# yhn112/DeDLOC

Measured on AMD Instinct MI355X. Metric: samples/sec (whole node) ALBERT-large MLM pretrain at 1/2/4/8 peers, higher is better.
Workload: dtype bf16; 1 GPU; model=albert-large-v2, global_batch=4096, seq_len=512, parallelism=collaborative-dp1, micro_batch=512, grad_accum=1, compression=FLOAT16, optimizer=LAMB, impl=dedloc

## Files before the change

dedloc_amd/_build.py:

```python
from __future__ import annotations

import concurrent.futures as cf
import glob
import os
import subprocess
import sys
import sysconfig

ROOT = os.path.dirname(os.path.abspath(__file__))
CSRC = os.path.join(ROOT, "csrc")
BUILD = os.path.join(os.path.dirname(ROOT), "build", "obj")
ARCH = os.environ.get("DEDLOC_OFFLOAD_ARCH", "gfx950")
SO_PATH = os.path.join(ROOT, "_C.so")
DHT_SO_PATH = os.path.join(ROOT, "_dht.so")
ROCM = os.environ.get("ROCM_PATH", "/opt/rocm")


def _torch_paths():
    import torch
    import torch.utils.cpp_extension as ce

    abi = int(torch.compiled_with_cxx11_abi())
    return ce.include_paths(), ce.library_paths(), abi


def _newer(target: str, deps) -> bool:
    if not os.path.exists(target):
        return True
    t = os.path.getmtime(target)
    return any(os.path.getmtime(d) > t for d in deps)


def _run(cmd, verbose):
    if verbose:
        print(" ".join(cmd), flush=True)
    r = subprocess.run(cmd, stdout=subprocess.PIPE, stderr=subprocess.STDOUT, text=True)
    if r.returncode != 0:
        raise RuntimeError(f"build step failed ({r.returncode}):\n{' '.join(cmd)}\n{r.stdout}")
    return r.stdout


def build(verbose: bool = False, jobs: int | None = None) -> str:
    os.makedirs(BUILD, exist_ok=True)
    headers = glob.glob(os.path.join(CSRC, "include", "*.h"))
    all_headers = sorted(set(headers) | set(glob.glob(os.path.join(CSRC, "**", "*.h"), recursive=True)))
    hip_srcs = sorted(glob.glob(os.path.join(CSRC, "kernels", "*.hip")))
    inc = ["-I", os.path.join(CSRC, "include")]
    hip_flags = ["--offload-arch=" + ARCH, *HIP_FLAGS]
    jobs = jobs or min(8, os.cpu_count() or 4)

    jobs_list = []
    objs = []
    for src in hip_srcs:
        obj = os.path.join(BUILD, os.path.basename(src).replace(".hip", ".o"))
        objs.append(obj)
        if _newer(obj, [src] + headers + [__file__]):
            jobs_list.append(["hipcc", *hip_flags, *FILE_FLAGS.get(os.path.basename(src), []), *inc, "-c", src,
                              "-o", obj])

    tinc, tlib, abi = _torch_paths()
    torch_srcs = [os.path.join(CSRC, "bindings.cpp")] + sorted(glob.glob(os.path.join(CSRC, "comm", "*.cpp")))
    for src in torch_srcs:
        name = os.path.basename(src).replace(".cpp", ".o")
        obj = os.path.join(BUILD, name if src.endswith("bindings.cpp") else "comm_" + name)
        objs.append(obj)
        if _newer(obj, [src] + all_headers):
            cmd = ["g++", "-O2", "-std=c++17", "-fPIC", f"-D_GLIBCXX_USE_CXX11_ABI={abi}", "-D__HIP_PLATFORM_AMD__",
                   "-DUSE_ROCM", "-I", f"{ROCM}/include", *inc]
            for p in tinc:
                cmd += ["-I", p]
            cmd += ["-I", sysconfig.get_paths()["include"], "-c", src, "-o", obj]
            jobs_list.append(cmd)

    for src in sorted(glob.glob(os.path.join(CSRC, "host", "*.cpp"))):
        obj = os.path.join(BUILD, "host_" + os.path.basename(src).replace(".cpp", ".o"))
        objs.append(obj)
        if _newer(obj, [src] + all_headers):
            jobs_list.append(["g++", "-O2", "-std=c++17", "-fPIC", "-Wall", "-D__HIP_PLATFORM_AMD__", "-I",
                              f"{ROCM}/include", *inc, "-c", src, "-o", obj])

    rt_srcs = sorted(glob.glob(os.path.join(CSRC, "runtime", "*.cpp")))
    rt_objs = []
    for src in rt_srcs:
        obj = os.path.join(BUILD, "rt_" + os.path.basename(src).replace(".cpp", ".o"))
        rt_objs.append(obj)
        if _newer(obj, [src] + all_headers):
            jobs_list.append(["g++", "-O2", "-std=c++17", "-fPIC", "-Wall", *inc, "-c", src, "-o", obj])

    with cf.ThreadPoolExecutor(jobs) as ex:
        list(ex.map(lambda c: _run(c, verbose), jobs_list))

    if _newer(SO_PATH, objs):
        _link(objs, SO_PATH, tlib, verbose)
    if rt_objs and _newer(DHT_SO_PATH, rt_objs):
        _run(["g++", "-shared", "-fPIC", *rt_objs, "-o", DHT_SO_PATH, "-lpthread"], verbose)
    _OBJS[:] = objs
    return SO_PATH


_OBJS: list = []
HIP_FLAGS = ["-O3", "-std=c++17", "-fPIC", "-ffp-contract=fast", "-munsafe-fp-atomics"]
FILE_FLAGS: dict = {"comm_q8.hip": ["-ffp-contract=on"]}


def _link(objs, out, tlib, verbose):
    cmd = ["hipcc", "--offload-arch=" + ARCH, "-shared", "-fPIC", *objs, "-o", out]
    for p in tlib:
        cmd += ["-L", p, f"-Wl,-rpath,{p}"]
    cmd += ["-lc10", "-ltorch", "-ltorch_cpu", "-lc10_hip", "-ltorch_hip", "-lamdhip64", "-lrccl", "-L", f"{ROCM}/lib",
            f"-Wl,-rpath,{ROCM}/lib"]
    _run(cmd, verbose)


def build_variant(name: str, rev: str, kernels, verbose: bool = False, flags=None) -> str:
    build(verbose)
    vdir = os.path.join(os.path.dirname(BUILD), "variant_" + name)
    os.makedirs(vdir, exist_ok=True)
    repo = os.path.dirname(ROOT)
    swap = {}
    for k in kernels:
        src = os.path.join(vdir, os.path.basename(k))
        where = "" if k.endswith(".cpp") else "kernels/"
        text = subprocess.run(["git", "-C", repo, "show", f"{rev}:dedloc_amd/csrc/{where}{os.path.basename(k)}"],
                              check=True, capture_output=True, text=True).stdout
        with open(src, "w") as f:
            f.write(text)
        if k.endswith(".cpp"):
            obj = src.replace(".cpp", ".o")
            tinc, _, abi = _torch_paths()
            cmd = ["g++", "-O2", "-std=c++17", "-fPIC", f"-D_GLIBCXX_USE_CXX11_ABI={abi}", "-D__HIP_PLATFORM_AMD__",
                   "-DUSE_ROCM", "-I", f"{ROCM}/include", "-I", os.path.join(CSRC, "include")]
            for ip in tinc:
                cmd += ["-I", ip]
            _run(cmd + list(flags or []) + ["-I", sysconfig.get_paths()["include"], "-c", src, "-o", obj], verbose)
        else:
            obj = src.replace(".hip", ".o")
            extra = FILE_FLAGS.get(os.path.basename(k), []) if flags is None else list(flags)
            _run(["hipcc", "--offload-arch=" + ARCH, *HIP_FLAGS, *extra, "-I", os.path.join(CSRC, "include"), "-c",
                  src, "-o", obj], verbose)
        swap[os.path.basename(obj)] = obj
    out_dir = os.path.join(repo, "ab")
    os.makedirs(out_dir, exist_ok=True)
    out = os.path.join(out_dir, f"_C_{name}.so")
    objs = [swap.get(os.path.basename(o), o) for o in _OBJS]
    _link(objs, out, _torch_paths()[1], verbose)
    return out


if __name__ == "__main__":
    if len(sys.argv) > 3 and sys.argv[1] == "variant":
        fl = [a for a in sys.argv[4:] if a.startswith("--flags=")]
        ks = [a for a in sys.argv[4:] if not a.startswith("--") and a != "-v"]
        print(build_variant(sys.argv[2], sys.argv[3], ks, verbose="-v" in sys.argv,
                            flags=fl[0][len("--flags="):].split() if fl else None))
    else:
        print(build(verbose="-v" in sys.argv))
```

dedloc_amd/csrc/bindings.cpp:

```cpp
#include <torch/extension.h>
#include <torch/library.h>
#include <c10/hip/HIPStream.h>

#include <atomic>
#include <cstring>
#include <map>
#include <mutex>
#include <string>
#include <unordered_map>

#include "dl_kernels.h"

namespace {

inline hipStream_t cur_stream(const at::Tensor& t) {
  return c10::hip::getCurrentHIPStream(t.get_device()).stream();
}

inline bf16_t* bf(const at::Tensor& t) { return reinterpret_cast<bf16_t*>(t.data_ptr()); }
inline const bf16_t* cbf(const at::Tensor& t) { return reinterpret_cast<const bf16_t*>(t.data_ptr()); }
inline float* f32(const at::Tensor& t) { return t.data_ptr<float>(); }

inline void check(int rc, const char* what) { TORCH_CHECK(rc == 0, "dedloc_amd: unsupported shape for ", what); }

// ... 336 lines not shown
                            f32(gamma), f32(beta), bf(y), bf(s), f32(mean), f32(rstd), (int)T, (int)E, (float)eps,
                            cur_stream(ids)),
        "embed_ln_pos_fwd");
  return {y, s, mean, rstd};
}

void embed_pos_bwd(const at::Tensor& ds, const at::Tensor& ids, const c10::optional<at::Tensor>& tt,
                   const at::Tensor& pos, at::Tensor dwemb, at::Tensor dpemb, at::Tensor dtemb) {
  expect(ds, at::kBFloat16, "ds");
  for (auto* t : {&dwemb, &dpemb, &dtemb}) expect(*t, at::kFloat, "embedding grad");
  const int64_t T = ids.numel(), E = ds.size(-1);
  const long* ttp = tt.has_value() ? tt->data_ptr<long>() : nullptr;
  check(dl_embed_pos_bwd(cbf(ds), ids.data_ptr<long>(), ttp, pos_ptr(pos, T), f32(dwemb), f32(dpemb),
                         f32(dtemb), (int)T, (int)E, (int)dtemb.size(0), cur_stream(ds)),
        "embed_pos_bwd");
}

std::tuple<at::Tensor, at::Tensor> xent_fwd_bwd(const at::Tensor& logits, const at::Tensor& labels, bool inplace,
                                                int64_t ignore_index) {
  expect(logits, at::kBFloat16, "logits");
  expect(labels, at::kLong, "labels");
  const int64_t V = logits.size(-1), M = logits.numel() / V;
  auto dl = inplace ? logits : at::empty_like(logits);
  auto ws = at::empty({3}, logits.options().dtype(at::kFloat));
  check(dl_xent_fwd_bwd(cbf(logits), labels.data_ptr<long>(), bf(dl), nullptr, f32(ws), f32(ws) + 1, (int)M, (int)V, V,
                        (int)ignore_index, cur_stream(logits)),
        "xent_fwd_bwd");
  return {ws.narrow(0, 0, 1).squeeze(0), dl};
}

std::tuple<at::Tensor, at::Tensor> xent_eval(const at::Tensor& logits, const at::Tensor& labels,
                                             int64_t ignore_index) {
  TORCH_CHECK(logits.is_cuda() && logits.scalar_type() == at::kBFloat16, "logits must be a bf16 GPU tensor");
  expect(labels, at::kLong, "labels");
  TORCH_CHECK(logits.dim() >= 1 && logits.size(-1) >= 1, "logits must be [..., V] with V >= 1");
  const int64_t V = logits.size(-1), M = logits.numel() / V;
  int64_t ld = V;
  if (logits.dim() == 2 && logits.stride(1) == 1 && logits.stride(0) >= V) ld = logits.stride(0);
  else TORCH_CHECK(logits.is_contiguous(), "logits must be contiguous or a 2-D view with unit column stride");
  TORCH_CHECK(labels.numel() == M, "labels has ", labels.numel(), " elements for ", M, " rows of logits");
  TORCH_CHECK(M <= INT32_MAX && V <= INT32_MAX, "xent_eval: too many rows or columns");
  auto row_loss = at::empty({M}, logits.options().dtype(at::kFloat));
  auto row_rank = at::empty({M}, logits.options().dtype(at::kInt));
  check(dl_xent_eval(cbf(logits), labels.data_ptr<long>(), f32(row_loss), row_rank.data_ptr<int>(), (int)M, (int)V, ld,
                     (int)ignore_index, cur_stream(logits)),
        "xent_eval");
  return {row_loss, row_rank};
}

std::tuple<at::Tensor, at::Tensor> knn_topk(const at::Tensor& q, const at::Tensor& bank, int64_t k, int64_t splits) {
  expect(q, at::kBFloat16, "q");
  expect(bank, at::kBFloat16, "bank");
  TORCH_CHECK(q.dim() == 2 && bank.dim() == 2 && q.size(1) == bank.size(1), "knn_topk: q [Q, D] and bank [N, D]");
  TORCH_CHECK(q.get_device() == bank.get_device(), "knn_topk: q and bank on different devices");
  const int64_t Q = q.size(0), N = bank.size(0), D = q.size(1);
  TORCH_CHECK(D % 16 == 0 && D >= 16 && D <= 4096, "knn_topk: D = ", D, " must be a multiple of 16 in 16 .. 4096");
  TORCH_CHECK(k >= 1 && k <= 256 && k <= N, "knn_topk: k = ", k, " must be in 1 .. min(256, N = ", N, ")");
  TORCH_CHECK(Q <= INT32_MAX && N <= INT32_MAX, "knn_topk: too many rows");
  const int max_splits = dl_knn_max_splits((int)N, (int)k);
  TORCH_CHECK(splits >= 0 && splits <= max_splits, "knn_topk: splits = ", splits, " must be 0 (automatic) or 1 .. ",
              max_splits, " for N = ", N, ", k = ", k);
  auto vals = at::empty({Q, k}, q.options().dtype(at::kFloat));
  auto idx = at::empty({Q, k}, q.options().dtype(at::kInt));
  if (Q == 0) return {vals, idx};
  int cus = 0;
  if (splits == 0)
    TORCH_CHECK(hipDeviceGetAttribute(&cus, hipDeviceAttributeMultiprocessorCount, q.get_device()) == hipSuccess,
                "knn_topk: cannot read the device's CU count");
  const int S = splits > 0 ? (int)splits : dl_knn_splits((int)Q, (int)N, (int)k, cus);
  auto lists = at::empty({dl_knn_list_entries((int)Q, (int)k, S)}, q.options().dtype(at::kLong));
  at::Tensor part;
  if (S > 1) part = at::empty({Q * S * k}, q.options().dtype(at::kLong));
  check(dl_knn_topk(cbf(q), cbf(bank), (int)Q, (int)N, (int)D, (int)k, S,
                    reinterpret_cast<unsigned long long*>(lists.data_ptr<int64_t>()),
                    S > 1 ? reinterpret_cast<unsigned long long*>(part.data_ptr<int64_t>()) : nullptr, f32(vals),
                    idx.data_ptr<int>(), cur_stream(q)),
        "knn_topk");
  return {vals, idx};
}

std::tuple<at::Tensor, at::Tensor> knn_vote(const at::Tensor& vals, const at::Tensor& idx, const at::Tensor& bank_labels,
                                            const at::Tensor& targets, int64_t num_classes, double sigma) {
  expect(vals, at::kFloat, "vals");
  expect(idx, at::kInt, "idx");
  expect(bank_labels, at::kInt, "bank_labels");
  expect(targets, at::kLong, "targets");
  TORCH_CHECK(vals.dim() == 2 && idx.sizes() == vals.sizes(), "knn_vote: vals and idx must both be [Q, k]");
  const int64_t Q = vals.size(0), k = vals.size(1), N = bank_labels.numel();
  TORCH_CHECK(k >= 1 && k <= 256, "knn_vote: k = ", k, " must be in 1 .. 256");
  TORCH_CHECK(targets.numel() == Q, "knn_vote: targets has ", targets.numel(), " elements for ", Q, " rows");
  TORCH_CHECK(N >= 1 && N <= INT32_MAX && Q <= INT32_MAX, "knn_vote: bank_labels must hold 1 .. 2^31 - 1 labels");
  TORCH_CHECK(num_classes >= 1 && num_classes <= 8192, "knn_vote: num_classes = ", num_classes, " must be in 1 .. 8192");
  TORCH_CHECK(sigma > 0, "knn_vote: sigma must be positive");
  auto pred = at::empty({Q}, vals.options().dtype(at::kInt));
  auto rank = at::empty({Q}, vals.options().dtype(at::kInt));
  check(dl_knn_vote(f32(vals), idx.data_ptr<int>(), bank_labels.data_ptr<int>(), targets.data_ptr<long>(),
                    pred.data_ptr<int>(), rank.data_ptr<int>(), (int)Q, (int)k, (int)N, (int)num_classes, (float)sigma,
                    cur_stream(vals)),
        "knn_vote");
  return {pred, rank};
}

inline const int* kvinfo_ptr(const c10::optional<at::Tensor>& kvinfo, int64_t B) {
  if (!kvinfo.has_value()) return nullptr;
  expect(*kvinfo, at::kInt, "kvinfo");
  TORCH_CHECK(kvinfo->numel() == B + 1, "kvinfo must be int32[B + 1] (lengths, prefix flag)");
  return kvinfo->data_ptr<int>();
}

inline void check_head_dim(int64_t D, int64_t ld, int64_t H, const char* what) {
  TORCH_CHECK((D == 64 || D == 128) && ld == 3 * H * D, "dedloc_amd: ", what, ": head_dim ", D, " (row length ", ld,
              ", ", H, " heads) is not supported by the fused attention kernels; supported head sizes are 64 and 128");
}

std::tuple<at::Tensor, at::Tensor> attn_fwd(const at::Tensor& qkv, const c10::optional<at::Tensor>& mbias, int64_t H,
                                            int64_t S, double scale, const c10::optional<at::Tensor>& kvinfo) {
  expect(qkv, at::kBFloat16, "qkv");
  const int64_t ld = qkv.size(-1), T = qkv.numel() / ld, D = ld / (3 * H), B = T / S;
  check_head_dim(D, ld, H, "attn_fwd");
  auto out = at::empty({T, H * D}, qkv.options());
  auto lse = at::empty({B, H, S}, qkv.options().dtype(at::kFloat));
  const float* mb = nullptr;
  if (mbias.has_value()) {
    expect(*mbias, at::kFloat, "mbias");
    mb = f32(*mbias);
  }
  check(dl_attn_fwd(cbf(qkv), ld, mb, kvinfo_ptr(kvinfo, B), bf(out), H * D, f32(lse), (int)B, (int)H, (int)S,
                    (int)D, (float)scale, cur_stream(qkv)),
        "attn_fwd");
  return {out, lse};
}

at::Tensor attn_bwd(const at::Tensor& qkv, const c10::optional<at::Tensor>& mbias, const at::Tensor& out,
                    const at::Tensor& dout, const at::Tensor& lse, int64_t H, int64_t S, double scale,
                    const c10::optional<at::Tensor>& kvinfo, const c10::optional<at::Tensor>& dbias) {
  expect(qkv, at::kBFloat16, "qkv");
  expect(out, at::kBFloat16, "out");
  expect(dout, at::kBFloat16, "dout");
  const int64_t ld = qkv.size(-1), T = qkv.numel() / ld, D = ld / (3 * H), B = T / S;
  check_head_dim(D, ld, H, "attn_bwd");
  auto dqkv = at::empty_like(qkv);
  auto delta = at::empty({B, H, S}, qkv.options().dtype(at::kFloat));
  const float* mb = mbias.has_value() ? f32(*mbias) : nullptr;
  float* dbp = nullptr;
  if (dbias.has_value()) {
    expect(*dbias, at::kFloat, "dbias");
    TORCH_CHECK(dbias->numel() == ld, "dbias must have 3*H*D elements");
    dbp = f32(*dbias);
  }
  check(dl_attn_bwd(cbf(qkv), ld, mb, kvinfo_ptr(kvinfo, B), cbf(out), cbf(dout), H * D, f32(lse), f32(delta),
                    bf(dqkv), dbp, (int)B, (int)H, (int)S, (int)D, (float)scale, cur_stream(qkv)),
        "attn_bwd");
  return dqkv;
}

struct PackedLayout {
  int64_t B, T, max_slot;
  const int* dev;
};
inline PackedLayout packed_layout(const at::Tensor& seqinfo, const at::Tensor& seqinfo_host, int64_t T,
                                  const char* what) {
  expect(seqinfo, at::kInt, "seqinfo");
  TORCH_CHECK(seqinfo_host.device().is_cpu() && seqinfo_host.scalar_type() == at::kInt && seqinfo_host.is_contiguous(),
              what, ": seqinfo_host must be a contiguous int32 CPU tensor");
  const int64_t n = seqinfo_host.numel();
  TORCH_CHECK(n >= 3 && n % 2 == 1 && seqinfo.numel() == n, what,
              ": seqinfo must be int32[2B + 1] (B + 1 row offsets, B lengths) on both sides");
  const int64_t B = (n - 1) / 2;
  const int* p = seqinfo_host.data_ptr<int>();
  TORCH_CHECK(p[0] == 0 && p[B] == T, what, ": row offsets must run from 0 to T = ", T, " (got ", p[0], " .. ", p[B],
              ")");
  int64_t max_slot = 0;
  for (int64_t b = 0; b < B; ++b) {
    const int64_t slot = (int64_t)p[b + 1] - p[b], len = p[B + 1 + b];
    TORCH_CHECK(p[b] % 64 == 0 && p[b + 1] % 64 == 0, what, ": row offset of sequence ", b,
                " is not a multiple of 64 (", p[b], ", ", p[b + 1], ")");
    TORCH_CHECK(slot >= 64, what, ": sequence ", b, " has an empty slot");
    TORCH_CHECK(len >= 1 && len <= slot, what, ": length ", len, " of sequence ", b, " is outside 1 .. its slot of ",
                slot, " rows");
    max_slot = std::max(max_slot, slot);
  }
  return PackedLayout{B, T, max_slot, seqinfo.data_ptr<int>()};
}

std::tuple<at::Tensor, at::Tensor> attn_varlen_fwd(const at::Tensor& qkv, const at::Tensor& seqinfo,
                                                   const at::Tensor& seqinfo_host, int64_t H, double scale) {
  expect(qkv, at::kBFloat16, "qkv");
  const int64_t ld = qkv.size(-1), T = qkv.numel() / ld, D = ld / (3 * H);
  check_head_dim(D, ld, H, "attn_varlen_fwd");
  const PackedLayout L = packed_layout(seqinfo, seqinfo_host, T, "attn_varlen_fwd");
  auto out = at::empty({T, H * D}, qkv.options());
  auto lse = at::empty({H, T}, qkv.options().dtype(at::kFloat));
  check(dl_attn_varlen_fwd(cbf(qkv), ld, L.dev, bf(out), H * D, f32(lse), (int)L.B, (int)T, (int)L.max_slot, (int)H,
                           (int)D, (float)scale, cur_stream(qkv)),
        "attn_varlen_fwd");
  return {out, lse};
}

at::Tensor attn_varlen_bwd(const at::Tensor& qkv, const at::Tensor& seqinfo, const at::Tensor& seqinfo_host,
                           const at::Tensor& out, const at::Tensor& dout, const at::Tensor& lse, int64_t H,
                           double scale, const c10::optional<at::Tensor>& dbias) {
  expect(qkv, at::kBFloat16, "qkv");
  expect(out, at::kBFloat16, "out");
  expect(dout, at::kBFloat16, "dout");
  expect(lse, at::kFloat, "lse");
  const int64_t ld = qkv.size(-1), T = qkv.numel() / ld, D = ld / (3 * H);
  check_head_dim(D, ld, H, "attn_varlen_bwd");
  const PackedLayout L = packed_layout(seqinfo, seqinfo_host, T, "attn_varlen_bwd");
  TORCH_CHECK(out.numel() == T * H * D && dout.numel() == T * H * D && lse.numel() == H * T,
              "attn_varlen_bwd: out / dout must be [T, H*D] and lse [H, T]");
  auto dqkv = at::empty_like(qkv);
  auto delta = at::empty({H, T}, qkv.options().dtype(at::kFloat));
  float* dbp = nullptr;
  if (dbias.has_value()) {
    expect(*dbias, at::kFloat, "dbias");
    TORCH_CHECK(dbias->numel() == ld, "dbias must have 3*H*D elements");
    dbp = f32(*dbias);
  }
  check(dl_attn_varlen_bwd(cbf(qkv), ld, L.dev, cbf(out), cbf(dout), H * D, f32(lse), f32(delta), bf(dqkv), dbp,
                           (int)L.B, (int)T, (int)L.max_slot, (int)H, (int)D, (float)scale, cur_stream(qkv)),
        "attn_varlen_bwd");
  return dqkv;
}

std::tuple<at::Tensor, at::Tensor> attn_softmax_fwd(const at::Tensor& s, const c10::optional<at::Tensor>& mbias,
                                                    int64_t H, double c) {
  expect(s, at::kFloat, "s");
  const int64_t S = s.size(-1), rows = s.numel() / S;
  TORCH_CHECK(rows % (H * S) == 0, "attn_softmax_fwd: scores must be [B*H*S, S]");
  const float* mb = nullptr;
  if (mbias.has_value()) {
    expect(*mbias, at::kFloat, "mbias");
    TORCH_CHECK(mbias->numel() == rows / H, "attn_softmax_fwd: mbias must be [B, S]");
    mb = f32(*mbias);
  }
  auto p = at::empty(s.sizes(), s.options().dtype(at::kBFloat16));
  auto lse = at::empty({rows}, s.options());
  check(dl_attn_softmax_fwd(f32(s), mb, bf(p), f32(lse), rows, (int)H, (int)S, (float)c, cur_stream(s)),
        "attn_softmax_fwd");
  return {p, lse};
}

std::tuple<at::Tensor, at::Tensor> attn_softmax_bwd(const at::Tensor& s, const at::Tensor& dp,
                                                    const c10::optional<at::Tensor>& mbias, const at::Tensor& lse,
                                                    const at::Tensor& delta, int64_t H, double c, double scale) {
  expect(s, at::kFloat, "s");
  expect(dp, at::kFloat, "dp");
  expect(lse, at::kFloat, "lse");
  expect(delta, at::kFloat, "delta");
  const int64_t S = s.size(-1), rows = s.numel() / S;
  TORCH_CHECK(dp.numel() == s.numel() && lse.numel() == rows && delta.numel() == rows && rows % (H * S) == 0,
              "attn_softmax_bwd: shape mismatch");
  const float* mb = nullptr;
  if (mbias.has_value()) {
    expect(*mbias, at::kFloat, "mbias");
    TORCH_CHECK(mbias->numel() == rows / H, "attn_softmax_bwd: mbias must be [B, S]");
    mb = f32(*mbias);
  }
  auto p = at::empty(s.sizes(), s.options().dtype(at::kBFloat16));
  auto ds = at::empty_like(p);
  check(dl_attn_softmax_bwd(f32(s), f32(dp), mb, f32(lse), f32(delta), bf(p), bf(ds), rows, (int)H, (int)S, (float)c,
                            (float)scale, cur_stream(s)),
        "attn_softmax_bwd");
  return {p, ds};
}


enum { kGemmNone = -1, kGemm8 = 0, kGemmTiled = 1, kGemmSmall = 2 };
std::atomic<int64_t> g_gemm_backend[3];

inline int took(int backend, int rc) {
  if (rc == 0) g_gemm_backend[backend].fetch_add(1, std::memory_order_relaxed);
  return rc;
}

std::vector<int64_t> gemm_backend_counts() {
  return {g_gemm_backend[kGemm8].load(), g_gemm_backend[kGemmTiled].load(), g_gemm_backend[kGemmSmall].load()};
}

inline void expect_operands(const at::Tensor& a, const at::Tensor& b) {
  TORCH_CHECK(a.is_cuda() && b.is_cuda(), "gemm operands must be GPU tensors");
  TORCH_CHECK(a.scalar_type() == at::kBFloat16 && b.scalar_type() == at::kBFloat16, "gemm operands must be bf16");
  TORCH_CHECK(a.dim() == 2 && b.dim() == 2 && a.stride(1) == 1 && b.stride(1) == 1,
              "gemm operands must be 2-D with unit inner stride");
}

inline at::Tensor f32_bias(const c10::optional<at::Tensor>& bias, int64_t n) {
  if (!bias.has_value()) return at::Tensor();
  TORCH_CHECK(bias->numel() == n, "gemm bias must hold one value per output column");
  return bias->scalar_type() == at::kFloat ? bias->contiguous() : bias->to(at::kFloat).contiguous();
}

inline DlGemm gemm_desc(const at::Tensor& a, bool trans_a, const at::Tensor& b, bool trans_b, bf16_t* C = nullptr,
                        long ldc = 0) {
  DlGemm g;
  g.A = cbf(a), g.lda = a.stride(0), g.a_kouter = trans_a;
  g.B = cbf(b), g.ldb = b.stride(0), g.b_kouter = !trans_b;
  g.M = (int)a.size(trans_a ? 1 : 0), g.N = (int)b.size(trans_b ? 0 : 1), g.K = (int)a.size(trans_a ? 0 : 1);
  TORCH_CHECK(b.size(trans_b ? 1 : 0) == g.K, "gemm inner dimensions differ");
  g.C = C, g.ldc = ldc;
  return g;
}

enum : unsigned { kUse8 = 1, kUseTiled = 2, kUseSmall = 4 };
int gemm_route(const DlGemm& g, unsigned allow, const at::Tensor& like, hipStream_t st) {
  if ((allow & kUse8) && took(kGemm8, dl_gemm8(g, st)) == 0) return kGemm8;
// ... 900 lines not shown
  TORCH_CHECK(groups >= 1 && N % groups == 0 && mean.numel() == groups * C && rstd.numel() == groups * C &&
                  sums.numel() == 2 * groups * C,
              "conv2d_dgrad_bn: statistics shapes");
  TORCH_CHECK(x.size(2) == H && x.size(3) == W && w.size(1) == C, "conv2d_dgrad_bn: x must be the conv input");
  const long stat_rows = N / groups * H * W;
  const DlBnBwdEpi bn{cbf(x), y.has_value() ? cbf(*y) : nullptr, (long)C, f32(mean), f32(rstd), f32(gamma),
                      f32(beta)};
  const at::Tensor gdy = dy.is_contiguous(at::MemoryFormat::ChannelsLast) ? dy
                                                                           : dy.contiguous(at::MemoryFormat::ChannelsLast);
  const int64_t K = w.size(0), R = w.size(2), S = w.size(3);
  if (is_pointwise(R, S, stride, pad) && gdy.size(2) == H && gdy.size(3) == W && conv_gemm()) {
    expect_nhwc(gdy, "dy");
    if (residual.has_value()) {
      expect_nhwc(*residual, "residual");
      TORCH_CHECK(residual->sizes() == x.sizes(), "conv2d_dgrad_bn: residual must have the input's shape");
    }
    auto dx = at::empty_like(x);
    const at::Tensor wk = krsc_view(w);
    const at::Tensor dyr = rows2d(gdy), wkc = wk.view({K, C});
    DlGemm g = gemm_desc(dyr, false, wkc, false, bf(dx), C);
    g.epi = DL_EPI_BNBWD;
    if (residual.has_value()) g.R = cbf(*residual), g.ldr = C;
    g.stats = f32(sums), g.stat_rows = stat_rows;
    g.bn = &bn;
    if (gemm_route(g, kUse8, dyr, cur_stream(dy)) != kGemmNone) return {dx, true};
  }
  if (!residual.has_value() && K % 64 == 0) {
    expect_nhwc(gdy, "dy");
    auto dx = at::empty_like(x);
    if (conv_dgrad_classes(gdy, krsc_view(w), stride, pad, H, W, dx, wds, f32(sums), groups, &bn)) return {dx, true};
  }
  return {conv2d_dgrad(gdy, w, stride, pad, H, W, residual, wds), false};
}

at::Tensor bn_bwd_prep(at::Tensor g, const at::Tensor& x, const c10::optional<at::Tensor>& y, const at::Tensor& mean,
                       const at::Tensor& rstd, const at::Tensor& gamma, const at::Tensor& beta, at::Tensor sums,
                       int64_t groups) {
  expect_nhwc(g, "g");
  expect_nhwc(x, "x");
  const int64_t C = x.size(1);
  check(dl_bn_bwd_prep(bf(g), y.has_value() ? cbf(*y) : nullptr, cbf(x), f32(mean), f32(rstd), f32(gamma), f32(beta),
                       f32(sums), x.numel() / C / groups, (int)C, (int)groups, cur_stream(g)),
        "bn_bwd_prep");
  return g;
}

void conv2d_wgrad(const at::Tensor& dy_in, const at::Tensor& x, at::Tensor dw, int64_t stride, int64_t pad,
                  const c10::optional<at::Tensor>& cols) {
  const at::Tensor dy = dy_in.is_contiguous(at::MemoryFormat::ChannelsLast)
                            ? dy_in
                            : dy_in.contiguous(at::MemoryFormat::ChannelsLast);
  expect_nhwc(dy, "dy");
  if (!cols.has_value()) expect_nhwc(x, "x");
  TORCH_CHECK(dw.is_cuda() && dw.scalar_type() == at::kFloat && dw.dim() == 4, "dw must be an fp32 4-D GPU tensor");
  const int64_t N = x.size(0), C = x.size(1), H = x.size(2), W = x.size(3);
  const int64_t K = dy.size(1), P = dy.size(2), Q = dy.size(3), R = dw.size(2), S = dw.size(3);
  TORCH_CHECK(dw.size(0) == K && dw.size(1) == C, "conv2d_wgrad: dw shape mismatch");
  TORCH_CHECK(!cols.has_value() || C % 64 != 0, "conv2d_wgrad: cols are the stem's (C not a multiple of 64) only");
  at::Tensor dk = dw.permute({0, 2, 3, 1});
  const bool direct = dk.is_contiguous();
  at::Tensor acc = direct ? dk : at::zeros({K, R, S, C}, dw.options());
  int rc;
  if (is_pointwise(R, S, stride, pad) && conv_gemm() && K % 256 == 0 && C % 256 == 0) {
    gemm_acc_f32(rows2d(dy), rows2d(x), acc.view({K, C}), true, false);
  } else if (C % 8 == 0 && C >= 8 && C % 64 == 0) {
    const DlConvGeom gm = geom(cbf(x), N, H, W, C, P, Q, stride, stride, R, S, -pad, 1, -pad, 1);
    rc = dl_conv_wgrad(gm, cbf(dy), K, (int)K, f32(acc), R * S * C, (int)(R * S * C), cur_stream(dy));
    check(rc, "conv2d_wgrad");
  } else if (stem_s2d_ok(C, R, S, stride, pad, H, W)) {
    at::Tensor xs;
    if (cols.has_value()) {
      TORCH_CHECK(cols->scalar_type() == at::kBFloat16 && cols->is_contiguous() && cols->dim() == 2 &&
                      cols->size(0) == N * P * Q && cols->size(1) == 16,
                  "cols must be the stem's im2col_stem (space-to-depth) matrix for this input");
      xs = *cols;
    } else {
      xs = stem_s2d(x);
    }
    auto slab = at::zeros({K, 256}, dw.options());
    rc = dl_conv_wgrad(geom(cbf(xs), N, H / 2, W / 2, 16, P, Q, 1, 1, 4, 4, -2, 1, -2, 1), cbf(dy), K, (int)K,
                       f32(slab), 256, 256, cur_stream(dy));
    check(rc, "conv2d_wgrad(stem)");
    acc.view({K, R * S * C}).add_(slab.index_select(1, stem_s2d_index(dw.device())));
  } else {
    const StemCols sc = stem_cols(R, S, C, false);
    const int64_t M = N * P * Q;
    const at::Tensor col = stem_cols_checked(cols, x, R, S, stride, pad, P, Q, sc);
    auto slab = at::zeros({K, R, sc.SCp}, dw.options());
    rc = dl_conv_wgrad(geom(cbf(col), M, 1, 1, sc.Kp, 1, 1, 1, 1, 1, 1, 0, 1, 0, 1), cbf(dy), K, (int)K,
                       f32(slab), R * sc.SCp, (int)(R * sc.SCp), cur_stream(dy));
    check(rc, "conv2d_wgrad(stem)");
    acc.view({K, R, S * C}).add_(slab.narrow(2, 0, S * C));
  }
  if (!direct) dk.add_(acc);
}

}

TORCH_LIBRARY_IMPL(dedloc, CUDA, m) {
  m.impl("conv2d_fwd", &conv2d_fwd);
  m.impl("conv2d_bn_act", &conv2d_bn_act);
  m.impl("conv2d_fwd_stats", &conv2d_fwd_stats);
  m.impl("im2col_stem", &im2col_stem);
  m.impl("conv2d_dgrad_bn", &conv2d_dgrad_bn);
  m.impl("conv2d_dgrad_weights", &conv2d_dgrad_weights);
  m.impl("conv2d_dgrad_weights_batched", &conv2d_dgrad_weights_batched);
  m.impl("bn_bwd_prep", &bn_bwd_prep);
  m.impl("conv2d_dgrad", &conv2d_dgrad);
  m.impl("conv2d_wgrad", &conv2d_wgrad);
  m.impl("bn_fwd", &bn_fwd);
  m.impl("bn_apply", &bn_apply);
  m.impl("bn_bwd", &bn_bwd);
  m.impl("sinkhorn", &sinkhorn);
  m.impl("swav_ce", &swav_ce);
  m.impl("swav_ce_multi", &swav_ce_multi);
  m.impl("row_normalize_", &row_normalize_);
  m.impl("maxpool_fwd", &maxpool_fwd);
  m.impl("maxpool_bwd", &maxpool_bwd);
  m.impl("avgpool_fwd", &avgpool_fwd);
  m.impl("avgpool_bwd", &avgpool_bwd);
  m.impl("l2norm_fwd", &l2norm_fwd);
  m.impl("l2norm_bwd", &l2norm_bwd);
  m.impl("multicrop", &multicrop);
  m.impl("multicrop_ragged", &multicrop_ragged);
  m.impl("layernorm_fwd", &layernorm_fwd);
  m.impl("layernorm_bwd", &layernorm_bwd);
  m.impl("gelu_fwd", &gelu_fwd);
  m.impl("gelu_bwd", &gelu_bwd);
  m.impl("tanh_fwd", &tanh_fwd);
  m.impl("tanh_bwd", &tanh_bwd);
  m.impl("bias_grad", &bias_grad);
  m.impl("cast_bf16", &cast_bf16);
  m.impl("lamb_step", &lamb_step);
  m.impl("larc_sgd_step", &larc_sgd_step);
  m.impl("grad_norm_clip", &grad_norm_clip);
  m.impl("axpby", &axpby);
  m.impl("add_slabs_zero_", &add_slabs_zero_);
  m.impl("scale_by_", &scale_by_);
  m.impl("pack", &pack);
  m.impl("reduce_parts", &reduce_parts);
  m.impl("unpack", &unpack);
  m.impl("reduce_delta", &reduce_delta);
  m.impl("pack_q8", &pack_q8);
  m.impl("reduce_delta_q8", &reduce_delta_q8);
  m.impl("unpack_q8", &unpack_q8);
  m.impl("embed_ln_fwd", &embed_ln_fwd);
  m.impl("embed_bwd", &embed_bwd);
  m.impl("xent_fwd_bwd", &xent_fwd_bwd);
  m.impl("xent_eval", &xent_eval);
  m.impl("knn_topk", &knn_topk);
  m.impl("knn_vote", &knn_vote);
  m.impl("attn_fwd", &attn_fwd);
  m.impl("attn_bwd", &attn_bwd);
  m.impl("attn_varlen_fwd", &attn_varlen_fwd);
  m.impl("attn_varlen_bwd", &attn_varlen_bwd);
  m.impl("embed_ln_pos_fwd", &embed_ln_pos_fwd);
  m.impl("embed_pos_bwd", &embed_pos_bwd);
  m.impl("attn_softmax_fwd", &attn_softmax_fwd);
  m.impl("attn_softmax_bwd", &attn_softmax_bwd);
  m.impl("gemm", &gemm);
  m.impl("bmm", &bmm);
  m.impl("gemm_acc_f32", &gemm_acc_f32);
  m.impl("gemm_acc_f32_shared", &gemm_acc_f32_shared);
  m.impl("gemm_gelu", &gemm_gelu);
  m.impl("gemm_dgelu", &gemm_dgelu);
  m.impl("gemm_gelu_d", &gemm_gelu_d);
  m.impl("gemm_dmul", &gemm_dmul);
}

extern "C" int dedloc_amd_native_abi_version() { return 1; }

TORCH_LIBRARY(dedloc_ws, m) {
  m.def("clear_workspaces() -> int", &clear_workspaces);
  m.def("gemm_backend_counts() -> int[]", &gemm_backend_counts);
  m.def("gemm_wgrad_splits(int M, int N, int K) -> int", &gemm_wgrad_splits);
}
```

dedloc_amd/csrc/include/dl_kernels.h:

```cpp
#pragma once
#include <hip/hip_runtime.h>
#include <stddef.h>
#include <stdint.h>

typedef uint16_t bf16_t;

int dl_layernorm_fwd(const bf16_t* x, const bf16_t* r, const float* gamma, const float* beta, bf16_t* y,
                     bf16_t* s_out, float* mean, float* rstd, int rows, int D, float eps, hipStream_t st);
int dl_layernorm_bwd(const bf16_t* dy, const bf16_t* s, const float* gamma, const float* mean, const float* rstd,
                     bf16_t* ds, float* dg_part, float* db_part, float* dsum, int rows, int D, int nparts,
                     hipStream_t st);

int dl_gelu_fwd(const bf16_t* h, bf16_t* y, size_t n, hipStream_t st);
int dl_gelu_bwd(const bf16_t* dy, const bf16_t* h, bf16_t* dh, size_t n, hipStream_t st);
int dl_gelu_bwd_colsum(const bf16_t* dy, const bf16_t* h, bf16_t* dh, float* dbias, int rows, int N, hipStream_t st);
int dl_gelu_fwd_d(const bf16_t* h, bf16_t* y, bf16_t* d, size_t n, hipStream_t st);
int dl_mul_colsum(const bf16_t* dy, const bf16_t* d, bf16_t* dh, float* dbias, int rows, int N, hipStream_t st);
int dl_tanh_fwd(const bf16_t* x, bf16_t* y, size_t n, hipStream_t st);
int dl_tanh_bwd(const bf16_t* dy, const bf16_t* y, bf16_t* dx, size_t n, hipStream_t st);
int dl_colsum_bf16(const bf16_t* x, float* part, int rows, int N, int nparts, hipStream_t st);
int dl_colsum_f32(const float* part, float* out, int nparts, int N, int accumulate, hipStream_t st);
int dl_cast_f32_bf16(const float* x, bf16_t* y, size_t n, hipStream_t st);
int dl_add_bf16_to_f32(const bf16_t* x, float* y, size_t n, float alpha, hipStream_t st);

// ... 14 lines not shown
int dl_add_slabs_zero(float* out, float* slabs, int s, size_t n, hipStream_t st);

int dl_pack(const float* src, void* dst, int dst_dt, size_t n, float weight, hipStream_t st);
int dl_reduce_parts(const void* parts, int part_dt, size_t part_stride, int nparts, void* out, int out_dt, size_t n,
                    float inv_total, hipStream_t st);
int dl_unpack(const void* src, int src_dt, float* dst, const float* snap, int add, size_t n, hipStream_t st);
int dl_reduce_delta(const void* parts, void* deltas, int dt, size_t part_stride, int nparts, const float* weights,
                    size_t n, hipStream_t st);

size_t dl_q8_bytes(size_t n);
int dl_pack_q8(const float* src, void* dst, size_t n, hipStream_t st);
int dl_unpack_q8(const void* src, float* dst, int add, size_t n, hipStream_t st);
int dl_reduce_delta_q8(const void* parts, void* deltas, int nparts, const float* weights, size_t n, hipStream_t st);

int dl_embed_ln_fwd(const long* ids, const long* tt, const float* wemb, const float* pemb, const float* temb,
                    const float* gamma, const float* beta, bf16_t* y, bf16_t* s_out, float* mean, float* rstd, int T,
                    int S, int E, float eps, hipStream_t st);
int dl_embed_bwd(const bf16_t* ds, const long* ids, const long* tt, float* dwemb, float* dpemb, float* dtemb, int B,
                 int S, int E, int ntypes, hipStream_t st);
int dl_embed_ln_pos_fwd(const long* ids, const long* tt, const int* pos, const float* wemb, const float* pemb,
                        const float* temb, const float* gamma, const float* beta, bf16_t* y, bf16_t* s_out, float* mean,
                        float* rstd, int T, int E, float eps, hipStream_t st);
int dl_embed_pos_bwd(const bf16_t* ds, const long* ids, const long* tt, const int* pos, float* dwemb, float* dpemb,
                     float* dtemb, int T, int E, int ntypes, hipStream_t st);

int dl_xent_fwd_bwd(const bf16_t* logits, const long* labels, bf16_t* dlogits, float* row_loss, float* loss_out,
                    float* scale_buf, int M, int V, long ld, int ignore_index, hipStream_t st);

int dl_xent_eval(const bf16_t* logits, const long* labels, float* row_loss, int* row_rank, int M, int V, long ld,
                 int ignore_index, hipStream_t st);

int dl_knn_max_splits(int N, int k);
int dl_knn_splits(int Q, int N, int k, int cus);
long dl_knn_list_entries(int Q, int k, int splits);
int dl_knn_topk(const bf16_t* q, const bf16_t* bank, int Q, int N, int D, int k, int splits, unsigned long long* lists,
                unsigned long long* part, float* vals, int* idx, hipStream_t st);
int dl_knn_vote(const float* vals, const int* idx, const int* labels, const long* targets, int* pred, int* rank, int Q,
                int k, int N, int C, float sigma, hipStream_t st);

struct DlBnBwdEpi {
  const bf16_t* X;
  const bf16_t* Y;
  long ldx;
  const float* mean;
  const float* rstd;
  const float* gamma;
  const float* beta;
};

enum DlGemmEpi {
  DL_EPI_STORE = 0,
  DL_EPI_GELU = 1,
  DL_EPI_DGELU = 2,
  DL_EPI_F32 = 3,
  DL_EPI_STATS = 4,
  DL_EPI_BNBWD = 5,
  DL_EPI_GELUD = 6,
  DL_EPI_DMUL = 7,
};

struct DlGemm {
  const bf16_t* A = nullptr; long lda = 0; int a_kouter = 0;
  const bf16_t* B = nullptr; long ldb = 0; int b_kouter = 0;
  int M = 0, N = 0, K = 0;
  DlGemmEpi epi = DL_EPI_STORE;
  bf16_t* C = nullptr; long ldc = 0;
  float* Cf = nullptr; long ldcf = 0; long slab = 0; int accumulate = 0;
  const float* bias = nullptr;
  const bf16_t* R = nullptr; long ldr = 0;
  bf16_t* H = nullptr; long ldh = 0;
  float* dbias = nullptr;
  int splits = 1;
  float* stats = nullptr; long stat_rows = 0;
  const DlBnBwdEpi* bn = nullptr;
};

int dl_gemm8(const DlGemm& g, hipStream_t st);
int dl_gemm(const DlGemm& g, hipStream_t st);

int dl_sinkhorn_ws(int n, int K);
int dl_sinkhorn(const float* scores, float* Q, float* ws, int n, int K, int bs, float eps, int iters,
                hipStream_t st);
int dl_swav_ce(const void* scores, int scores_bf16, const float* q, float* dscores, float* loss, int rows, int K,
               float temperature, float scale, hipStream_t st);
int dl_swav_ce_multi(const void* scores, int scores_bf16, const float* q, const int* crops, int n_assign,
                     float* dscores, float* loss, int num_crops, int bs, int K, float temperature, float scale,
                     hipStream_t st);
int dl_row_normalize(float* w, int rows, int d, hipStream_t st);
int dl_multicrop(const float* pool, int P, int Hp, int Wp, const float* params, int nb, int S, int rad, const float* mean,
                 const float* stdv, float* ws, bf16_t* out, hipStream_t st);
int dl_multicrop_ragged(const unsigned char* bytes, long nbytes, const long* meta, int n, const float* params, int nb,
                        int S, int rad, const float* mean, const float* stdv, float* ws, bf16_t* out, hipStream_t st);
int dl_bn_fwd(const bf16_t* x, const bf16_t* res, bf16_t* y, const float* gamma, const float* beta, float* sums,
              float* mean, float* rstd, float* run_mean, float* run_var, long R, int C, int G, float eps,
              float momentum, int relu, hipStream_t st, int sums_zeroed = 0, int stats_ready = 0);
int dl_bn_apply(const bf16_t* x, const bf16_t* res, bf16_t* y, const float* gamma, const float* beta,
                const float* mean, const float* rstd, long R, int C, int G, int relu, hipStream_t st);
int dl_bn_stats(const bf16_t* x, float* sums, long R, int C, int G, hipStream_t st);
int dl_bn_bwd(const bf16_t* dy, const bf16_t* y, const bf16_t* x, const float* mean, const float* rstd,
              const float* gamma, float* sums, bf16_t* dx, bf16_t* dres, float* dgamma, float* dbeta, long R, int C,
              int G, int relu, hipStream_t st, int sums_zeroed = 0, int accumulate = 0, const float* beta = nullptr,
              int stats_ready = 0);
int dl_bn_bwd_prep(bf16_t* dy, const bf16_t* y, const bf16_t* x, const float* mean, const float* rstd,
                   const float* gamma, const float* beta, float* sums, long R, int C, int G, hipStream_t st);

struct DlConvGeom {
  const bf16_t* img;
  int Nimg, H, W, C;
  int I, J, sh, sw;
  int TR, TS, dh0, dhs, dw0, dws;
};
int dl_conv_fwd(const DlConvGeom& g, const bf16_t* w, long ldw, int N, bf16_t* out, int OH, int OW, int osh, int osw,
                int oh0, int ow0, long ldo, hipStream_t st, float* stats = nullptr, long stat_rows = 0,
                const DlBnBwdEpi* bn = nullptr);
int dl_conv_fwd_affine(const DlConvGeom& g, const bf16_t* w, long ldw, int N, bf16_t* out, int OH, int OW, long ldo,
                       const float* scale, const float* shift, const bf16_t* res, int relu, hipStream_t st);
struct DlConvFwdJob {
  DlConvGeom g;
  const bf16_t* w;
  long ldw;
  int oh0, ow0;
  long stat_rows;
};
int dl_conv_fwd_multi(const DlConvFwdJob* jobs, int njobs, int N, bf16_t* out, int OH, int OW, int osh, int osw,
                      long ldo, hipStream_t st, float* stats = nullptr, const DlBnBwdEpi* bn = nullptr);
struct DlWtJob {
  const bf16_t* src;
  bf16_t* dst;
  int K, C, R, S;
  int r0, s0, st, TR, TS;
};
int dl_conv_dgrad_weights_batched(const DlWtJob* jobs, int njobs, hipStream_t st);
int dl_conv_wgrad(const DlConvGeom& g, const bf16_t* dy, long ldy, int Cout, float* dw, long lddw, int Ncols,
                  hipStream_t st);
int dl_stem_s2d(const bf16_t* x, int N, int H, int W, bf16_t* xs, hipStream_t st);
int dl_im2col(const bf16_t* x, int N, int H, int W, int C, int R, int S, int stride, int pad, int P, int Q, int SCp,
              int Kp, bf16_t* col, hipStream_t st);

int dl_attn_softmax_fwd(const float* s, const float* mbias, bf16_t* p, float* lse, long rows, int H, int S, float c,
                        hipStream_t st);
int dl_attn_softmax_bwd(const float* s, const float* dp, const float* mbias, const float* lse, const float* delta,
                        bf16_t* p, bf16_t* ds, long rows, int H, int S, float c, float scale, hipStream_t st);

int dl_attn_hd128_fwd(const bf16_t* qkv, long ld, const float* mbias, const int* kvinfo, bf16_t* out, long ldo,
                      float* lse, int B, int H, int S, float scale, hipStream_t st);
int dl_attn_hd128_bwd(const bf16_t* qkv, long ld, const float* mbias, const int* kvinfo, const bf16_t* out,
                      const bf16_t* dout, long ldo, const float* lse, float* delta, bf16_t* dqkv, float* dbias, int B,
                      int H, int S, float scale, hipStream_t st);
int dl_attn_fwd(const bf16_t* qkv, long ld, const float* mbias, const int* kvinfo, bf16_t* out, long ldo, float* lse,
                int B, int H, int S, int D, float scale, hipStream_t st);
int dl_attn_bwd(const bf16_t* qkv, long ld, const float* mbias, const int* kvinfo, const bf16_t* out,
                const bf16_t* dout, long ldo, const float* lse, float* delta, bf16_t* dqkv, float* dbias, int B, int H,
                int S, int D, float scale, hipStream_t st);
int dl_attn_hd128_varlen_fwd(const bf16_t* qkv, long ld, const int* seqinfo, bf16_t* out, long ldo, float* lse, int B,
                             int T, int max_slot, int H, float scale, hipStream_t st);
int dl_attn_hd128_varlen_bwd(const bf16_t* qkv, long ld, const int* seqinfo, const bf16_t* out, const bf16_t* dout,
                             long ldo, const float* lse, float* delta, bf16_t* dqkv, float* dbias, int B, int T,
                             int max_slot, int H, float scale, hipStream_t st);
int dl_attn_varlen_fwd(const bf16_t* qkv, long ld, const int* seqinfo, bf16_t* out, long ldo, float* lse, int B, int T,
                       int max_slot, int H, int D, float scale, hipStream_t st);
int dl_attn_varlen_bwd(const bf16_t* qkv, long ld, const int* seqinfo, const bf16_t* out, const bf16_t* dout, long ldo,
                       const float* lse, float* delta, bf16_t* dqkv, float* dbias, int B, int T, int max_slot, int H,
                       int D, float scale, hipStream_t st);

int dl_maxpool_fwd(const bf16_t* x, bf16_t* y, uint8_t* arg, int N, int H, int W, int C, int P, int Q, hipStream_t st);
int dl_maxpool_bwd(const bf16_t* dy, const uint8_t* arg, bf16_t* dx, int N, int H, int W, int C, int P, int Q,
                   hipStream_t st);
int dl_avgpool_fwd(const bf16_t* x, bf16_t* y, int N, int HW, int C, hipStream_t st);
int dl_avgpool_bwd(const bf16_t* dy, bf16_t* dx, int N, int HW, int C, hipStream_t st);
int dl_l2norm_fwd(const bf16_t* x, bf16_t* y, float* rinv, int rows, int D, float eps, hipStream_t st);
int dl_l2norm_bwd(const bf16_t* dy, const bf16_t* y, const float* rinv, bf16_t* dx, int rows, int D, hipStream_t st);

int dl_gemm_small(const DlGemm& g, float* ws, hipStream_t st);
int dl_gemm_small_splits(int M, int N, int K);
int dl_gemm_small_batched(int epi, const bf16_t* A, long sam, long sak, long sab, const bf16_t* B, long sbn, long sbk,
                          long sbb, int M, int N, int K, bf16_t* C, long ldc, float* Cf, long ldcf, long scb,
                          int batch, hipStream_t st);
```

dedloc_amd/csrc/kernels/attention.hip:

```cpp
#include <cstdlib>
#include <type_traits>

#include "dl_attn_tile.h"
#include "dl_common.h"
#include "dl_kernels.h"

namespace {

constexpr int HD = 64;

struct TileRegs { uint4 a, b; };

__device__ __forceinline__ uint4 tile_ld1(const bf16_t* g, long ld, int row0, int rows_valid, int idx) {
  const int row = min(row0 + (idx >> 3), rows_valid - 1);
  return *reinterpret_cast<const uint4*>(g + (long)row * ld + (idx & 7) * 8);
}

__device__ __forceinline__ void tile_load(TileRegs& t, const bf16_t* g, long ld, int row0, int rows_valid) {
  t.a = tile_ld1(g, ld, row0, rows_valid, threadIdx.x);
  t.b = tile_ld1(g, ld, row0, rows_valid, threadIdx.x + 256);
}

__device__ __forceinline__ void tile_store(const TileRegs& t, uint8_t* tile) {
  const int i0 = threadIdx.x, i1 = threadIdx.x + 256;
// ... 1 lines not shown
  *reinterpret_cast<uint4*>(tile + chunk_off(i1 >> 3, i1 & 7)) = t.b;
}

constexpr int NBUF = 2;
constexpr int STAGE = 2 * TILE_BYTES + 512;


struct FwdCtx {
  const bf16_t* Kg;
  const bf16_t* Vg;
  long ld;
  int S, kv_end;
  const float* mb_g;
  float sl2;
  uint8_t* smem;
  float* mbs;
  int w, lane;
  template <int NW = 4>
  __device__ __forceinline__ void issue(int s) const {
    uint8_t* slot = smem + (s % NBUF) * STAGE;
    dma_tile<NW>(Kg, ld, s * 64, slot, w, lane);
    dma_tile<NW>(Vg, ld, s * 64, slot + TILE_BYTES, w, lane);
    if (mb_g) dma_f32x64(mb_g + s * 64, slot + 2 * TILE_BYTES, lane);
  }
};

__device__ __forceinline__ float key_bias(const FwdCtx& c, int key) {
  return c.mb_g ? c.mb_g[key] : (key < c.kv_end ? 0.f : NEG_BIG);
}

template <bool LEAN, bool RING, int QS, int NW>
__device__ __forceinline__ void fwd_tiles(const FwdCtx& c, int kt0, int kt1, int nt, const bf16x8 (&qf)[QS][4],
                                          floatx16 (&o)[QS][2], float (&m)[QS], float (&l)[QS], int r, int hh,
                                          int lane) {
  TileRegs kr, vr;
  float mbr = 0.f;
  for (int kt = kt0; kt < kt1; ++kt) {
    const uint8_t* Ks;
    const float* mb;
    bool more = false;
    if constexpr (RING) {
      wait_stages<16 / NW>(min(nt - 1 - kt, NBUF - 2), c.mb_g != nullptr);
      __syncthreads();
      if (kt + NBUF - 1 < nt) c.template issue<NW>(kt + NBUF - 1);
      Ks = c.smem + (kt % NBUF) * STAGE;
      mb = reinterpret_cast<const float*>(Ks + 2 * TILE_BYTES);
    } else {
      const int cur = kt & 1;
      Ks = c.smem + cur * 2 * TILE_BYTES;
      mb = c.mbs + cur * 64;
      more = kt + 1 < nt;
      if (more) {
        tile_load(kr, c.Kg, c.ld, (kt + 1) * 64, c.S);
        tile_load(vr, c.Vg, c.ld, (kt + 1) * 64, c.S);
        if (threadIdx.x < 64) mbr = key_bias(c, (kt + 1) * 64 + threadIdx.x);
      }
    }
    const uint8_t* Vs = Ks + TILE_BYTES;
    floatx16 s[QS][2];
#pragma unroll
    for (int u = 0; u < QS; ++u)
#pragma unroll
      for (int j = 0; j < 2; ++j)
#pragma unroll
        for (int i = 0; i < 16; ++i) s[u][j][i] = 0.f;
#pragma unroll
    for (int j = 0; j < 2; ++j)
#pragma unroll
      for (int ks = 0; ks < 4; ++ks) {
        const bf16x8 kfr = lds_row_frag(Ks, 32 * j + r, 2 * ks + hh);
#pragma unroll
        for (int u = 0; u < QS; ++u) s[u][j] = mfma32(kfr, qf[u][ks], s[u][j]);
      }
#pragma unroll
    for (int u = 0; u < QS; ++u) {
      if (!LEAN) {
        if (!RING || c.mb_g) {
#pragma unroll
          for (int j = 0; j < 2; ++j)
#pragma unroll
            for (int i = 0; i < 16; ++i) s[u][j][i] = fmaf(s[u][j][i], c.sl2, mb[32 * j + crow(i, hh)]);
        } else {
#pragma unroll
          for (int j = 0; j < 2; ++j)
#pragma unroll
            for (int i = 0; i < 16; ++i)
              s[u][j][i] = fmaf(s[u][j][i], c.sl2, kt * 64 + 32 * j + crow(i, hh) < c.kv_end ? 0.f : NEG_BIG);
        }
      }
      float mc[4];
#pragma unroll
      for (int q4 = 0; q4 < 4; ++q4) {
        const floatx16& sv = s[u][q4 >> 1];
        const int o8 = (q4 & 1) * 8;
        float v = vmax3(sv[o8], sv[o8 + 1], sv[o8 + 2]);
        v = vmax3(v, sv[o8 + 3], sv[o8 + 4]);
        v = vmax3(v, sv[o8 + 5], sv[o8 + 6]);
        mc[q4] = v;
      }
      float mx = vmax3(vmax3(mc[0], mc[1], s[u][0][7]), vmax3(mc[2], mc[3], s[u][0][15]),
                       vmax3(s[u][1][7], s[u][1][15], mc[0]));
      mx = half_max(mx);
      if (LEAN) mx *= c.sl2;
      const bool grow = mx > m[u] + RESCALE_THR;
      if (__ballot(grow) != 0) {
        const float mn = grow ? mx : m[u];
        const float alpha = __builtin_amdgcn_exp2f(m[u] - mn);
        l[u] *= alpha;
        m[u] = mn;
#pragma unroll
        for (int t = 0; t < 2; ++t)
#pragma unroll
          for (int i = 0; i < 16; ++i) o[u][t][i] *= alpha;
      }
      const float nm = -m[u];
      float rsa[8] = {0.f, 0.f, 0.f, 0.f, 0.f, 0.f, 0.f, 0.f};
#pragma unroll
      for (int j = 0; j < 2; ++j)
#pragma unroll
        for (int i = 0; i < 16; ++i) {
          const float pv = __builtin_amdgcn_exp2f(LEAN ? fmaf(s[u][j][i], c.sl2, nm) : s[u][j][i] + nm);
          s[u][j][i] = pv;
          rsa[i & 7] += pv;
        }
      float rs = ((rsa[0] + rsa[1]) + (rsa[2] + rsa[3])) + ((rsa[4] + rsa[5]) + (rsa[6] + rsa[7]));
      l[u] += half_sum(rs);
    }
#pragma unroll
    for (int j = 0; j < 2; ++j)
#pragma unroll
      for (int ss = 0; ss < 2; ++ss) {
        bf16x8 pb[QS];
#pragma unroll
        for (int u = 0; u < QS; ++u) pb[u] = pack_acc(s[u][j], ss);
#pragma unroll
        for (int t = 0; t < 2; ++t) {
          const bf16x8 vfr = tr_operand(Vs, 32 * j + 16 * ss, hh, t, lane);
#pragma unroll
          for (int u = 0; u < QS; ++u) o[u][t] = mfma32(vfr, pb[u], o[u][t]);
        }
      }
    if constexpr (!RING) {
      if (more) {
        uint8_t* Kn = c.smem + ((kt & 1) ^ 1) * 2 * TILE_BYTES;
        tile_store(kr, Kn);
        tile_store(vr, Kn + TILE_BYTES);
        if (threadIdx.x < 64) c.mbs[((kt & 1) ^ 1) * 64 + threadIdx.x] = mbr;
      }
      __syncthreads();
    }
  }
}

template <bool RING, int QS, int NW = 4, bool VARLEN = false>
__global__ __launch_bounds__(64 * NW, NW == 8 ? 1 : 2) void attn_fwd_kernel(const bf16_t* __restrict__ qkv, long ld,
                                                          const float* __restrict__ mbias,
                                                          const int* __restrict__ kvinfo, bf16_t* __restrict__ out,
                                                          long ldo, float* __restrict__ lse, int B, int H, int S_,
                                                          float sl2, int xcd) {
  __shared__ __attribute__((aligned(16))) uint8_t smem[RING ? NBUF * STAGE : 4 * TILE_BYTES + 2 * 64 * 4];
  const BlockId bid = block_id(xcd);
  const int b = bid.b, h = bid.h;
  const int lane = threadIdx.x & 63, w = threadIdx.x >> 6, r = lane & 31, hh = lane >> 5;
  const int S = seq_rows<VARLEN>(kvinfo, b, S_);
  if constexpr (VARLEN) {
    if (bid.x * (32 * QS * NW) >= S) return;
  }
  const long rb = seq_base<VARLEN>(kvinfo, b, S);
  const bf16_t* Qg = qkv + rb * ld + h * HD;
  bool use_len;
  FwdCtx c;
  c.Kg = qkv + rb * ld + (long)H * HD + h * HD;
  c.Vg = qkv + rb * ld + 2L * H * HD + h * HD;
  c.ld = ld;
  c.S = S;
  c.kv_end = seq_kv_end<VARLEN>(kvinfo, B, b, S, use_len);
  c.mb_g = (!use_len && mbias) ? mbias + rb : nullptr;
  c.sl2 = sl2;
  c.smem = smem;
  c.mbs = reinterpret_cast<float*>(smem + 4 * TILE_BYTES);
  c.w = w;
  c.lane = lane;

  static_assert(NW == 4 || (NW == 8 && RING), "8-wave blocks stage through the ring");
  const int nt = (c.kv_end + 63) / 64;
  if constexpr (RING) {
    for (int s0 = 0; s0 < NBUF - 1 && s0 < nt; ++s0) c.template issue<NW>(s0);
  }
  int q[QS];
  bf16x8 qf[QS][4];
#pragma unroll
  for (int u = 0; u < QS; ++u) {
    q[u] = bid.x * (32 * QS * NW) + w * (32 * QS) + 32 * u + r;
    const int qc = min(q[u], S - 1);
#pragma unroll
    for (int ks = 0; ks < 4; ++ks) qf[u][ks] = gload8(Qg + (long)qc * ld + ks * 16 + 8 * hh);
    if constexpr (RING) {
#pragma unroll
      for (int ks = 0; ks < 4; ++ks) settle(qf[u][ks]);
    }
  }

  floatx16 o[QS][2];
  float m[QS], l[QS];
#pragma unroll
  for (int u = 0; u < QS; ++u) {
    m[u] = NEG_BIG;
    l[u] = 0.f;
#pragma unroll
    for (int t = 0; t < 2; ++t)
#pragma unroll
      for (int i = 0; i < 16; ++i) o[u][t][i] = 0.f;
  }

  if constexpr (RING) {
    wait_vm_all();
  } else {
    TileRegs kr, vr;
    tile_load(kr, c.Kg, ld, 0, S);
    tile_load(vr, c.Vg, ld, 0, S);
    const float mbr = threadIdx.x < 64 ? key_bias(c, threadIdx.x) : 0.f;
    tile_store(kr, smem);
    tile_store(vr, smem + TILE_BYTES);
    if (threadIdx.x < 64) c.mbs[threadIdx.x] = mbr;
    __syncthreads();
  }
  const int nlean = c.mb_g ? 0 : c.kv_end / 64;
  fwd_tiles<true, RING, QS, NW>(c, 0, nlean, nt, qf, o, m, l, r, hh, lane);
  fwd_tiles<false, RING, QS, NW>(c, nlean, nt, nt, qf, o, m, l, r, hh, lane);

#pragma unroll
  for (int u = 0; u < QS; ++u) {
    const bool live = q[u] < S;
    store_row64(out + (rb + q[u]) * ldo + h * HD, o[u], 1.f / l[u], hh, live);
    if (live && hh == 0) lse[seq_stat<VARLEN>(b, h, H, S, S_, rb) + q[u]] = m[u] + log2f(l[u]);
  }
}

template <bool RING, int QS, bool VARLEN = false>
__global__ __launch_bounds__(256, 2) void attn_bwd_dq_kernel(const bf16_t* __restrict__ qkv, long ld,
                                                             const float* __restrict__ mbias,
                                                             const int* __restrict__ kvinfo,
                                                             const bf16_t* __restrict__ out, const bf16_t* __restrict__ dout,
                                                             long ldo, const float* __restrict__ lse,
                                                             float* __restrict__ delta, bf16_t* __restrict__ dqkv,
                                                             float* __restrict__ dbias, int B, int H, int S_, float sl2,
                                                             float scale, int xcd) {
  __shared__ __attribute__((aligned(16))) uint8_t smem[RING ? NBUF * STAGE : 4 * TILE_BYTES + 4 * 64 * 4];
  const BlockId bid = block_id(xcd);
  const int b = bid.b, h = bid.h;
  const int lane = threadIdx.x & 63, w = threadIdx.x >> 6, r = lane & 31, hh = lane >> 5;
  const int S = seq_rows<VARLEN>(kvinfo, b, S_);
  if constexpr (VARLEN) {
    if (bid.x * (128 * QS) >= S) return;
  }
  const long rb = seq_base<VARLEN>(kvinfo, b, S);
  const bf16_t* Qg = qkv + rb * ld + h * HD;
  const bf16_t* Kg = qkv + rb * ld + (long)H * HD + h * HD;
  const bf16_t* Vg = qkv + rb * ld + 2L * H * HD + h * HD;
  bool use_len;
  const int kv_end = seq_kv_end<VARLEN>(kvinfo, B, b, S, use_len);
  const float* mb_g = (!use_len && mbias) ? mbias + rb : nullptr;
  float* mbs = reinterpret_cast<float*>(smem + 4 * TILE_BYTES);
  const int nt = (kv_end + 63) / 64;
  auto issue = [&](int st) {
    uint8_t* slot = smem + (st % NBUF) * STAGE;
    dma_tile(Kg, ld, st * 64, slot, w, lane);
    dma_tile(Vg, ld, st * 64, slot + TILE_BYTES, w, lane);
    if (mb_g) dma_f32x64(mb_g + st * 64, slot + 2 * TILE_BYTES, lane);
  };
  if constexpr (RING) {
    for (int s0 = 0; s0 < NBUF - 1 && s0 < nt; ++s0) issue(s0);
  }

  int q[QS];
  bf16x8 qf[QS][4], df[QS][4];
  float dl[QS], l2[QS];
#pragma unroll
  for (int u = 0; u < QS; ++u) {
    q[u] = bid.x * (128 * QS) + w * (32 * QS) + 32 * u + r;
    const int qc = min(q[u], S - 1);
    dl[u] = 0.f;
#pragma unroll
    for (int ks = 0; ks < 4; ++ks) {
      qf[u][ks] = gload8(Qg + (long)qc * ld + ks * 16 + 8 * hh);
      const long oo = (rb + qc) * ldo + h * HD + ks * 16 + 8 * hh;
      df[u][ks] = gload8(dout + oo);
      const bf16x8 of = gload8(out + oo);
#pragma unroll
      for (int e = 0; e < 8; ++e) dl[u] += (float)df[u][ks][e] * (float)of[e];
    }
    dl[u] += __shfl_xor(dl[u], 32, 64);
    l2[u] = lse[seq_stat<VARLEN>(b, h, H, S, S_, rb) + qc];
    if constexpr (RING) {
      settle(l2[u]);
      settle(dl[u]);
#pragma unroll
      for (int ks = 0; ks < 4; ++ks) {
        settle(qf[u][ks]);
        settle(df[u][ks]);
      }
    }
  }

  floatx16 dq[QS][2];
#pragma unroll
  for (int u = 0; u < QS; ++u)
#pragma unroll
    for (int t = 0; t < 2; ++t)
#pragma unroll
      for (int i = 0; i < 16; ++i) dq[u][t][i] = 0.f;

  TileRegs kr, vr;
  float mbr = 0.f;
  if constexpr (RING) {
    wait_vm_all();
  } else {
    tile_load(kr, Kg, ld, 0, S);
    tile_load(vr, Vg, ld, 0, S);
    if (threadIdx.x < 64) mbr = mb_g ? mb_g[threadIdx.x] : 0.f;
    tile_store(kr, smem);
    tile_store(vr, smem + TILE_BYTES);
    if (threadIdx.x < 64) mbs[threadIdx.x] = mbr;
    __syncthreads();
  }

  auto tiles = [&](auto lean_tag, int kt0, int kt1) {
  constexpr bool LEAN = decltype(lean_tag)::value;
  int tm = threadIdx.x;
  if constexpr (!LEAN) settle(tm);
  const int lm = tm & 63, rm = tm & 31, hm = (tm >> 5) & 1;
  for (int kt = kt0; kt < kt1; ++kt) {
    const uint8_t* Ks;
    const float* mb;
    if constexpr (RING) {
      wait_stages(min(nt - 1 - kt, NBUF - 2), mb_g != nullptr);
      __syncthreads();
      if (kt + NBUF - 1 < nt) issue(kt + NBUF - 1);
      Ks = smem + (kt % NBUF) * STAGE;
      mb = reinterpret_cast<const float*>(Ks + 2 * TILE_BYTES);
    } else {
      Ks = smem + (kt & 1) * 2 * TILE_BYTES;
      mb = mbs + (kt & 1) * 64;
      if (kt + 1 < nt) {
        tile_load(kr, Kg, ld, (kt + 1) * 64, S);
        tile_load(vr, Vg, ld, (kt + 1) * 64, S);
        if (threadIdx.x < 64) mbr = mb_g ? mb_g[(kt + 1) * 64 + threadIdx.x] : 0.f;
      }
    }
    const uint8_t* Vs = Ks + TILE_BYTES;
#pragma unroll
    for (int j = 0; j < 2; ++j) {
      floatx16 st[QS], dp[QS];
#pragma unroll
      for (int u = 0; u < QS; ++u)
#pragma unroll
        for (int i = 0; i < 16; ++i) { st[u][i] = 0.f; dp[u][i] = 0.f; }
#pragma unroll
      for (int ks = 0; ks < 4; ++ks) {
        const bf16x8 kfr = lds_row_frag(Ks, 32 * j + rm, 2 * ks + hm);
        const bf16x8 vfr = lds_row_frag(Vs, 32 * j + rm, 2 * ks + hm);
#pragma unroll
        for (int u = 0; u < QS; ++u) {
          st[u] = mfma32(kfr, qf[u][ks], st[u]);
          dp[u] = mfma32(vfr, df[u][ks], dp[u]);
        }
      }
#pragma unroll
      for (int u = 0; u < QS; ++u) {
        if constexpr (LEAN) {
#pragma unroll
          for (int i = 0; i < 16; ++i) {
            const float p = __builtin_amdgcn_exp2f(fmaf(st[u][i], sl2, -l2[u]));
            st[u][i] = p * (dp[u][i] - dl[u]);
          }
        } else if (mb_g) {
#pragma unroll
          for (int i = 0; i < 16; ++i) {
            const float p = __builtin_amdgcn_exp2f(st[u][i] * sl2 + mb[32 * j + crow(i, hm)] - l2[u]);
            st[u][i] = p * (dp[u][i] - dl[u]);
          }
        } else {
#pragma unroll
          for (int i = 0; i < 16; ++i) {
            const int key = kt * 64 + 32 * j + crow(i, hm);
            const float p = __builtin_amdgcn_exp2f(st[u][i] * sl2 + (key < kv_end ? 0.f : NEG_BIG) - l2[u]);
            st[u][i] = p * (dp[u][i] - dl[u]);
          }
        }
      }
#pragma unroll
      for (int ss = 0; ss < 2; ++ss) {
        bf16x8 pb[QS];
#pragma unroll
        for (int u = 0; u < QS; ++u) pb[u] = pack_acc(st[u], ss);
#pragma unroll
        for (int t = 0; t < 2; ++t) {
          const bf16x8 ktr = tr_operand(Ks, 32 * j + 16 * ss, hm, t, lm);
#pragma unroll
          for (int u = 0; u < QS; ++u) dq[u][t] = mfma32(ktr, pb[u], dq[u][t]);
        }
      }
    }
    if constexpr (!RING) {
      if (kt + 1 < nt) {
        uint8_t* Kn = smem + ((kt & 1) ^ 1) * 2 * TILE_BYTES;
        tile_store(kr, Kn);
        tile_store(vr, Kn + TILE_BYTES);
        if (threadIdx.x < 64) mbs[((kt & 1) ^ 1) * 64 + threadIdx.x] = mbr;
      }
      __syncthreads();
    }
  }
  };
  const int nlean = mb_g ? 0 : kv_end / 64;
  tiles(std::true_type{}, 0, nlean);
  tiles(std::false_type{}, nlean, nt);
  if constexpr (RING) __syncthreads();
  int tid = threadIdx.x;
  settle(tid);
  const int w_ = tid >> 6, r_ = tid & 31, hh_ = (tid >> 5) & 1;
  int qe[QS];
#pragma unroll
  for (int u = 0; u < QS; ++u) qe[u] = bid.x * (128 * QS) + w_ * (32 * QS) + 32 * u + r_;
#pragma unroll
  for (int u = 0; u < QS; ++u) {
    const bool live = qe[u] < S;
    if (live && hh_ == 0) delta[seq_stat<VARLEN>(b, h, H, S, S_, rb) + qe[u]] = dl[u];
    store_row64(dqkv + (rb + qe[u]) * ld + h * HD, dq[u], scale, hh_, live);
  }
  if (dbias) {
    float* part = reinterpret_cast<float*>(smem);
    float cq[2][16], cd[4][8];
#pragma unroll
    for (int t = 0; t < 2; ++t)
#pragma unroll
      for (int i = 0; i < 16; ++i) {
        float v = 0.f;
#pragma unroll
        for (int u = 0; u < QS; ++u) v += qe[u] < S ? round_bf16(dq[u][t][i] * scale) : 0.f;
        cq[t][i] = half_wave_sum(v);
      }
#pragma unroll
    for (int ks = 0; ks < 4; ++ks)
#pragma unroll
      for (int e = 0; e < 8; ++e) {
        float v = 0.f;
#pragma unroll
        for (int u = 0; u < QS; ++u) v += qe[u] < S ? (float)df[u][ks][e] : 0.f;
        cd[ks][e] = half_wave_sum(v);
      }
    if (r_ == 0) {
      float* pw = part + w_ * 128;
#pragma unroll
      for (int t = 0; t < 2; ++t)
#pragma unroll
        for (int v4 = 0; v4 < 4; ++v4)
          *reinterpret_cast<float4*>(pw + 32 * t + 8 * v4 + 4 * hh_) =
              float4{cq[t][4 * v4], cq[t][4 * v4 + 1], cq[t][4 * v4 + 2], cq[t][4 * v4 + 3]};
#pragma unroll
      for (int ks = 0; ks < 4; ++ks)
#pragma unroll
        for (int g = 0; g < 2; ++g)
          *reinterpret_cast<float4*>(pw + 64 + 16 * ks + 8 * hh_ + 4 * g) =
              float4{cd[ks][4 * g], cd[ks][4 * g + 1], cd[ks][4 * g + 2], cd[ks][4 * g + 3]};
    }
    __syncthreads();
    if (threadIdx.x < 128) {
      const int c = threadIdx.x & 63, which = threadIdx.x >> 6;
      const float* pc = part + which * 64 + c;
      atomicAdd(&dbias[(which ? 2L * H * HD : 0L) + h * HD + c], pc[0] + pc[128] + pc[256] + pc[384]);
    }
  }
}

template <bool RING, int KS, bool VARLEN = false>
__global__ __launch_bounds__(256, KS == 2 ? 1 : 2) void attn_bwd_dkdv_kernel(
    const bf16_t* __restrict__ qkv, long ld, const float* __restrict__ mbias, const int* __restrict__ kvinfo,
    const bf16_t* __restrict__ dout, long ldo, const float* __restrict__ lse, const float* __restrict__ delta,
    bf16_t* __restrict__ dqkv, int B, int H, int S_, float sl2, float scale, int xcd) {
  __shared__ __attribute__((aligned(16))) uint8_t smem[RING ? NBUF * STAGE : 4 * TILE_BYTES + 2 * 2 * 64 * 4];
  const BlockId bid = block_id(xcd);
  const int b = bid.b, h = bid.h;
  const int lane = threadIdx.x & 63, w = threadIdx.x >> 6, r = lane & 31, hh = lane >> 5;
  const int S = seq_rows<VARLEN>(kvinfo, b, S_);
  if constexpr (VARLEN) {
    if (bid.x * (128 * KS) >= S) return;
  }
  const long rb = seq_base<VARLEN>(kvinfo, b, S);
  const bf16_t* Qg = qkv + rb * ld + h * HD;
  const bf16_t* Kg = qkv + rb * ld + (long)H * HD + h * HD;
  const bf16_t* Vg = qkv + rb * ld + 2L * H * HD + h * HD;
  const bf16_t* dOg = dout + rb * ldo + h * HD;
  const float* lse_g = lse + seq_stat<VARLEN>(b, h, H, S, S_, rb);
  const float* del_g = delta + seq_stat<VARLEN>(b, h, H, S, S_, rb);
  float* rowv = reinterpret_cast<float*>(smem + 4 * TILE_BYTES);

  int k[KS];
#pragma unroll
  for (int u = 0; u < KS; ++u) k[u] = bid.x * (128 * KS) + w * (32 * KS) + 32 * u + r;
  bool use_len;
  const int kv_end = seq_kv_end<VARLEN>(kvinfo, B, b, S, use_len);
  if (use_len && bid.x * (128 * KS) >= kv_end) {
#pragma unroll
    for (int u = 0; u < KS; ++u) {
      if (k[u] < S) {
        bf16_t* dkp = dqkv + (rb + k[u]) * ld + (long)H * HD + h * HD;
        bf16_t* dvp = dqkv + (rb + k[u]) * ld + 2L * H * HD + h * HD;
#pragma unroll
        for (int v = 0; v < 8; ++v) {
          store4(dkp + 8 * v + 4 * hh, 0.f, 0.f, 0.f, 0.f);
          store4(dvp + 8 * v + 4 * hh, 0.f, 0.f, 0.f, 0.f);
        }
      }
    }
    return;
  }
  const int nt = S / 64;
  auto issue = [&](int st) {
    uint8_t* slot = smem + (st % NBUF) * STAGE;
    dma_tile(Qg, ld, st * 64, slot, w, lane);
    dma_tile(dOg, ldo, st * 64, slot + TILE_BYTES, w, lane);
    dma_f32x64((w < 2 ? lse_g : del_g) + st * 64, slot + 2 * TILE_BYTES + (w < 2 ? 0 : 256), lane);
  };
  if constexpr (RING) {
    for (int s0 = 0; s0 < NBUF - 1 && s0 < nt; ++s0) issue(s0);
  }
  bf16x8 kf[KS][4], vf[KS][4];
  float mbk[KS];
#pragma unroll
  for (int u = 0; u < KS; ++u) {
    const int kc = min(k[u], S - 1);
#pragma unroll
    for (int ks = 0; ks < 4; ++ks) {
      kf[u][ks] = gload8(Kg + (long)kc * ld + ks * 16 + 8 * hh);
      vf[u][ks] = gload8(Vg + (long)kc * ld + ks * 16 + 8 * hh);
    }
    mbk[u] = use_len ? (k[u] < kv_end ? 0.f : NEG_BIG) : (mbias ? mbias[rb + kc] : 0.f);
    if constexpr (RING) {
      settle(mbk[u]);
#pragma unroll
      for (int ks = 0; ks < 4; ++ks) {
        settle(kf[u][ks]);
        settle(vf[u][ks]);
      }
    }
  }

  floatx16 dk[KS][2], dv[KS][2];
#pragma unroll
  for (int u = 0; u < KS; ++u)
#pragma unroll
    for (int t = 0; t < 2; ++t)
#pragma unroll
      for (int i = 0; i < 16; ++i) { dk[u][t][i] = 0.f; dv[u][t][i] = 0.f; }

  TileRegs qr, dr;
  float rv = 0.f;
  if constexpr (RING) {
    wait_vm_all();
  } else {
    tile_load(qr, Qg, ld, 0, S);
    tile_load(dr, dOg, ldo, 0, S);
    if (threadIdx.x < 128) rv = threadIdx.x < 64 ? lse_g[threadIdx.x] : del_g[threadIdx.x - 64];
    tile_store(qr, smem);
    tile_store(dr, smem + TILE_BYTES);
    if (threadIdx.x < 128) rowv[threadIdx.x] = rv;
    __syncthreads();
  }

  auto qloop = [&](auto lean_tag) {
  constexpr bool LEAN = decltype(lean_tag)::value;
  for (int qt = 0; qt < nt; ++qt) {
    const uint8_t* Qs;
    const float* lse_s;
    if constexpr (RING) {
      wait_stages(min(nt - 1 - qt, NBUF - 2), true);
      __syncthreads();
      if (qt + NBUF - 1 < nt) issue(qt + NBUF - 1);
      Qs = smem + (qt % NBUF) * STAGE;
      lse_s = reinterpret_cast<const float*>(Qs + 2 * TILE_BYTES);
    } else {
      Qs = smem + (qt & 1) * 2 * TILE_BYTES;
      lse_s = rowv + (qt & 1) * 128;
      if (qt + 1 < nt) {
        tile_load(qr, Qg, ld, (qt + 1) * 64, S);
        tile_load(dr, dOg, ldo, (qt + 1) * 64, S);
        if (threadIdx.x < 128)
          rv = threadIdx.x < 64 ? lse_g[(qt + 1) * 64 + threadIdx.x] : del_g[(qt + 1) * 64 + threadIdx.x - 64];
      }
    }
    const uint8_t* Ds = Qs + TILE_BYTES;
    const float* del_s = lse_s + 64;
#pragma unroll
    for (int i2 = 0; i2 < 2; ++i2) {
      floatx16 sc[KS], dp[KS];
#pragma unroll
      for (int u = 0; u < KS; ++u)
#pragma unroll
        for (int i = 0; i < 16; ++i) { sc[u][i] = 0.f; dp[u][i] = 0.f; }
#pragma unroll
      for (int ks = 0; ks < 4; ++ks) {
        const bf16x8 qfr = lds_row_frag(Qs, 32 * i2 + r, 2 * ks + hh);
        const bf16x8 dfr = lds_row_frag(Ds, 32 * i2 + r, 2 * ks + hh);
#pragma unroll
        for (int u = 0; u < KS; ++u) {
          sc[u] = mfma32(qfr, kf[u][ks], sc[u]);
          dp[u] = mfma32(dfr, vf[u][ks], dp[u]);
        }
      }
#pragma unroll
      for (int u = 0; u < KS; ++u)
#pragma unroll
        for (int i = 0; i < 16; ++i) {
          const int qq = 32 * i2 + crow(i, hh);
          const float p = __builtin_amdgcn_exp2f(LEAN ? fmaf(sc[u][i], sl2, -lse_s[qq])
                                                      : sc[u][i] * sl2 + mbk[u] - lse_s[qq]);
          sc[u][i] = p;
          dp[u][i] = p * (dp[u][i] - del_s[qq]);
        }
#pragma unroll
      for (int ss = 0; ss < 2; ++ss) {
        bf16x8 pb[KS], db[KS];
#pragma unroll
        for (int u = 0; u < KS; ++u) {
          pb[u] = pack_acc(sc[u], ss);
          db[u] = pack_acc(dp[u], ss);
        }
#pragma unroll
        for (int t = 0; t < 2; ++t) {
          const bf16x8 dtr = tr_operand(Ds, 32 * i2 + 16 * ss, hh, t, lane);
          const bf16x8 qtr = tr_operand(Qs, 32 * i2 + 16 * ss, hh, t, lane);
#pragma unroll
          for (int u = 0; u < KS; ++u) {
            dv[u][t] = mfma32(dtr, pb[u], dv[u][t]);
            dk[u][t] = mfma32(qtr, db[u], dk[u][t]);
          }
        }
      }
    }
    if constexpr (!RING) {
      if (qt + 1 < nt) {
        uint8_t* Qn = smem + ((qt & 1) ^ 1) * 2 * TILE_BYTES;
        tile_store(qr, Qn);
        tile_store(dr, Qn + TILE_BYTES);
        if (threadIdx.x < 128) rowv[((qt & 1) ^ 1) * 128 + threadIdx.x] = rv;
      }
      __syncthreads();
    }
  }
  };
  if (use_len) {
    qloop(std::true_type{});
#pragma unroll
    for (int u = 0; u < KS; ++u)
      if (k[u] >= kv_end)
#pragma unroll
        for (int t = 0; t < 2; ++t)
#pragma unroll
          for (int i = 0; i < 16; ++i) dk[u][t][i] = dv[u][t][i] = 0.f;
  } else {
    qloop(std::false_type{});
  }
#pragma unroll
  for (int u = 0; u < KS; ++u) {
    const bool live = k[u] < S;
    store_row64(dqkv + (rb + k[u]) * ld + (long)H * HD + h * HD, dk[u], scale, hh, live);
    store_row64(dqkv + (rb + k[u]) * ld + 2L * H * HD + h * HD, dv[u], 1.f, hh, live);
  }
}

constexpr int kAttnXcd = 1;

}

int dl_attn_fwd(const bf16_t* qkv, long ld, const float* mbias, const int* kvinfo, bf16_t* out, long ldo, float* lse,
                int B, int H, int S, int D, float scale, hipStream_t st) {
  if (D == 128) return dl_attn_hd128_fwd(qkv, ld, mbias, kvinfo, out, ldo, lse, B, H, S, scale, st);
  if (D != HD || S % 64 != 0 || ld % 8 != 0 || ldo % 8 != 0) return -1;
  const float sl2 = scale * 1.4426950408889634f;
  dim3 grid((S + 255) / 256, H, B);
  attn_fwd_kernel<true, 2><<<grid, 256, 0, st>>>(qkv, ld, mbias, kvinfo, out, ldo, lse, B, H, S, sl2, kAttnXcd);
  return 0;
}

int dl_attn_bwd(const bf16_t* qkv, long ld, const float* mbias, const int* kvinfo, const bf16_t* out,
                const bf16_t* dout, long ldo, const float* lse, float* delta, bf16_t* dqkv, float* dbias, int B, int H,
                int S, int D, float scale, hipStream_t st) {
  if (D == 128)
    return dl_attn_hd128_bwd(qkv, ld, mbias, kvinfo, out, dout, ldo, lse, delta, dqkv, dbias, B, H, S, scale, st);
  if (D != HD || S % 64 != 0 || ld % 8 != 0 || ldo % 8 != 0) return -1;
  const float sl2 = scale * 1.4426950408889634f;
  dim3 grid_dq((S + 255) / 256, H, B);
  attn_bwd_dq_kernel<true, 2><<<grid_dq, 256, 0, st>>>(qkv, ld, mbias, kvinfo, out, dout, ldo, lse, delta, dqkv,
                                                       dbias, B, H, S, sl2, scale, kAttnXcd);
  dim3 grid_kv((S + 127) / 128, H, B);
  attn_bwd_dkdv_kernel<true, 1><<<grid_kv, 256, 0, st>>>(qkv, ld, mbias, kvinfo, dout, ldo, lse, delta, dqkv, B, H,
                                                         S, sl2, scale, kAttnXcd);
  return 0;
}

int dl_attn_varlen_fwd(const bf16_t* qkv, long ld, const int* seqinfo, bf16_t* out, long ldo, float* lse, int B, int T,
                       int max_slot, int H, int D, float scale, hipStream_t st) {
  if (!seqinfo || B < 1 || T % 64 != 0 || max_slot < 64 || max_slot % 64 != 0 || max_slot > T) return -1;
  if (D == 128) return dl_attn_hd128_varlen_fwd(qkv, ld, seqinfo, out, ldo, lse, B, T, max_slot, H, scale, st);
  if (D != HD || ld % 8 != 0 || ldo % 8 != 0) return -1;
  const float sl2 = scale * 1.4426950408889634f;
  dim3 grid((max_slot + 255) / 256, H, B);
  attn_fwd_kernel<true, 2, 4, true><<<grid, 256, 0, st>>>(qkv, ld, nullptr, seqinfo, out, ldo, lse, B, H, T, sl2,
                                                          kAttnXcd);
  return 0;
}

int dl_attn_varlen_bwd(const bf16_t* qkv, long ld, const int* seqinfo, const bf16_t* out, const bf16_t* dout, long ldo,
                       const float* lse, float* delta, bf16_t* dqkv, float* dbias, int B, int T, int max_slot, int H,
                       int D, float scale, hipStream_t st) {
  if (!seqinfo || B < 1 || T % 64 != 0 || max_slot < 64 || max_slot % 64 != 0 || max_slot > T) return -1;
  if (D == 128)
    return dl_attn_hd128_varlen_bwd(qkv, ld, seqinfo, out, dout, ldo, lse, delta, dqkv, dbias, B, T, max_slot, H, scale,
                                    st);
  if (D != HD || ld % 8 != 0 || ldo % 8 != 0) return -1;
  const float sl2 = scale * 1.4426950408889634f;
  dim3 grid_dq((max_slot + 255) / 256, H, B);
  attn_bwd_dq_kernel<true, 2, true><<<grid_dq, 256, 0, st>>>(qkv, ld, nullptr, seqinfo, out, dout, ldo, lse, delta,
                                                             dqkv, dbias, B, H, T, sl2, scale, kAttnXcd);
  dim3 grid_kv((max_slot + 127) / 128, H, B);
  attn_bwd_dkdv_kernel<true, 1, true><<<grid_kv, 256, 0, st>>>(qkv, ld, nullptr, seqinfo, dout, ldo, lse, delta, dqkv,
                                                               B, H, T, sl2, scale, kAttnXcd);
  return 0;
}
```

dedloc_amd/models/albert.py:

```python
from __future__ import annotations

import json
import math
import os
from dataclasses import asdict, dataclass, field, fields
from typing import Dict, List, Optional

import torch
import torch.nn as nn
import torch.nn.functional as F

from .. import ops
from ..data.packing import PackedBatch, pack_batch, unpack_rows
from ..utils.flat import FlatParams

NEG_BIG = -1.0e30


@dataclass
class AlbertConfig:
    vocab_size: int = 30000
    embedding_size: int = 128
    hidden_size: int = 4096
    num_hidden_layers: int = 12
    num_hidden_groups: int = 1
    num_attention_heads: int = 64
    intermediate_size: int = 16384
    inner_group_num: int = 1
    hidden_act: str = "gelu_new"
    hidden_dropout_prob: float = 0.0
    attention_probs_dropout_prob: float = 0.0
    max_position_embeddings: int = 512
    type_vocab_size: int = 2
    initializer_range: float = 0.02
    layer_norm_eps: float = 1e-12
    classifier_dropout_prob: float = 0.1
    num_labels: Optional[int] = None
    pad_token_id: int = 0
    bos_token_id: int = 2
    eos_token_id: int = 3
    model_type: str = "albert"
    architectures: List[str] = field(default_factory=lambda: ["AlbertForPreTraining"])

    @classmethod
    def albert_large_v2(cls, **kw) -> "AlbertConfig":
        base = dict(vocab_size=30000, embedding_size=128, hidden_size=1024, num_hidden_layers=24,
                    num_hidden_groups=1, num_attention_heads=16, intermediate_size=4096, inner_group_num=1)
        base.update(kw)
        return cls(**base)

    @classmethod
    def albert_base_v2(cls, **kw) -> "AlbertConfig":
        base = dict(vocab_size=30000, embedding_size=128, hidden_size=768, num_hidden_layers=12,
                    num_hidden_groups=1, num_attention_heads=12, intermediate_size=3072, inner_group_num=1)
        base.update(kw)
        return cls(**base)

    @classmethod
    def albert_xxlarge_v2(cls, **kw) -> "AlbertConfig":
        base = dict(vocab_size=30000, embedding_size=128, hidden_size=4096, num_hidden_layers=12,
                    num_hidden_groups=1, num_attention_heads=64, intermediate_size=16384, inner_group_num=1)
        base.update(kw)
        return cls(**base)

    @classmethod
    def albert_xlarge_v2(cls, **kw) -> "AlbertConfig":
        base = dict(vocab_size=30000, embedding_size=128, hidden_size=2048, num_hidden_layers=24,
                    num_hidden_groups=1, num_attention_heads=16, intermediate_size=8192, inner_group_num=1)
        base.update(kw)
        return cls(**base)

    BUILTIN = {"albert-large-v2": "albert_large_v2", "albert-base-v2": "albert_base_v2",
               "albert-xlarge-v2": "albert_xlarge_v2", "albert-xxlarge-v2": "albert_xxlarge_v2"}

    @classmethod
    def tiny(cls, **kw) -> "AlbertConfig":
        base = dict(vocab_size=512, embedding_size=64, hidden_size=128, num_hidden_layers=3, num_hidden_groups=1,
                    num_attention_heads=2, intermediate_size=256, max_position_embeddings=128)
        base.update(kw)
        return cls(**base)

    def to_dict(self) -> Dict:
        d = asdict(self)
        if d.get("num_labels") is None:
            d.pop("num_labels", None)
        return d

    @classmethod
    def from_dict(cls, d: Dict) -> "AlbertConfig":
        names = {f.name for f in fields(cls)}
        return cls(**{k: v for k, v in d.items() if k in names})

    @classmethod
    def from_pretrained(cls, path: str) -> "AlbertConfig":
        for name, ctor in cls.BUILTIN.items():
            if path == name or (isinstance(path, str) and path.endswith(f"{name}-config.json")
                                and not os.path.exists(path)):
                return getattr(cls, ctor)()
        if os.path.isdir(path):
            path = os.path.join(path, "config.json")
        with open(path) as f:
            return cls.from_dict(json.load(f))

    def save_pretrained(self, directory: str):
        os.makedirs(directory, exist_ok=True)
        with open(os.path.join(directory, "config.json"), "w") as f:
            json.dump(self.to_dict(), f, indent=2, sort_keys=True)


def _layer_prefix(g: int, i: int) -> str:
    return f"albert.encoder.albert_layer_groups.{g}.albert_layers.{i}."


_RESIDUAL_IN_GEMM = True
_DGRAD_WT = True
_SHARED_WGRAD = True
_GELU_GRAD_IN_FWD = True


class _AlbertLayerFn(torch.autograd.Function):

    @staticmethod
    def forward(ctx, h, mask, lv, H, S, eps):
        O = ops.OPS
        qkv = O.gemm(h, lv["wqkv"], lv["bqkv32"], None, False, True, 0)
        if isinstance(mask, PackedBatch):
            att, lse = ops.attn_varlen_fwd(qkv, mask, H, 1.0 / math.sqrt(qkv.shape[1] // (3 * H)))
        else:
            mbias, kvinfo = mask
            att, lse = ops.attn_fwd(qkv, mbias, H, S, 1.0 / math.sqrt(qkv.shape[1] // (3 * H)), kvinfo)
        if _RESIDUAL_IN_GEMM:
            s1 = O.gemm(att, lv["wo"], lv["bo32"], h, False, True, 0)
            h1, _, m1, r1 = O.layernorm_fwd(s1, None, lv["ln1g"], lv["ln1b"], eps)
            f, g = (O.gemm_gelu_d if _GELU_GRAD_IN_FWD else O.gemm_gelu)(h1, lv["w1"], lv["b132"])
            s2 = O.gemm(g, lv["w2"], lv["b232"], h1, False, True, 0)
            out, _, m2, r2 = O.layernorm_fwd(s2, None, lv["ln2g"], lv["ln2b"], eps)
        else:
            a = O.gemm(att, lv["wo"], lv["bo32"], None, False, True, 0)
            h1, s1, m1, r1 = O.layernorm_fwd(a, h, lv["ln1g"], lv["ln1b"], eps)
            f, g = (O.gemm_gelu_d if _GELU_GRAD_IN_FWD else O.gemm_gelu)(h1, lv["w1"], lv["b132"])
            f2 = O.gemm(g, lv["w2"], lv["b232"], None, False, True, 0)
            out, s2, m2, r2 = O.layernorm_fwd(f2, h1, lv["ln2g"], lv["ln2b"], eps)
        ctx.save_for_backward(h, qkv, att, lse, s1, m1, r1, h1, f, g, s2, m2, r2)
        ctx.lv, ctx.mask, ctx.H, ctx.S = lv, mask, H, S
        ctx.gelu_d = _GELU_GRAD_IN_FWD
        return out

    @staticmethod
    def backward(ctx, dy):
        O = ops.OPS
        h, qkv, att, lse, s1, m1, r1, h1, f, g, s2, m2, r2 = ctx.saved_tensors
        lv = ctx.lv
        dy = dy.contiguous()
        H = ctx.H
        ds2 = O.layernorm_bwd(dy, s2, lv["ln2g"], m2, r2, lv["gln2g"], lv["gln2b"], True, lv["gb2"])
        _wgrad(O, ds2, g, lv, "gw2")
        wt = "w2t" in lv
        dfn = O.gemm_dmul if ctx.gelu_d else O.gemm_dgelu
        df = dfn(ds2, lv["w2t"], f, lv["gb1"], True) if wt else dfn(ds2, lv["w2"], f, lv["gb1"])
        _wgrad(O, df, h1, lv, "gw1")
        dh1 = _dgrad(O, df, lv, "w1", ds2)
        del df
        ds1 = O.layernorm_bwd(dh1, s1, lv["ln1g"], m1, r1, lv["gln1g"], lv["gln1b"], True, lv["gbo"])
        _wgrad(O, ds1, att, lv, "gwo")
        datt = _dgrad(O, ds1, lv, "wo", None)
        if isinstance(ctx.mask, PackedBatch):
            dqkv = ops.attn_varlen_bwd(qkv, ctx.mask, att, datt, lse, H, 1.0 / math.sqrt(qkv.shape[1] // (3 * H)),
                                       lv["gbqkv"])
        else:
            dqkv = ops.attn_bwd(qkv, ctx.mask[0], att, datt, lse, H, ctx.S, 1.0 / math.sqrt(qkv.shape[1] // (3 * H)),
                                ctx.mask[1], lv["gbqkv"])
        _wgrad(O, dqkv, h, lv, "gwqkv")
        dh = _dgrad(O, dqkv, lv, "wqkv", ds1)
        return dh, None, None, None, None, None


def _wgrad(O, dy, x, lv, name):
    if "wg_first" in lv:
        O.gemm_acc_f32_shared(dy, x, lv[name], True, False, lv["wg_first"], lv["wg_last"])
    else:
        O.gemm_acc_f32(dy, x, lv[name], True, False)


def _dgrad(O, dy, lv, name, residual):
    if name + "t" in lv:
        return O.gemm(dy, lv[name + "t"], None, residual, False, True, 0)
    return O.gemm(dy, lv[name], None, residual, False, False, 0)


@torch.no_grad()
def _with_transposed_weights(lv: Dict) -> Dict:
    lv = dict(lv)
    for name in ("wqkv", "wo", "w1", "w2"):
        lv[name + "t"] = lv[name].t().contiguous()
    return lv


class AlbertPreTrainedModel(nn.Module):

    add_pooler = True
    pack_sequences = False

    def __init__(self, config: AlbertConfig):
        super().__init__()
        self.config = c = config
        self._p: Dict[str, nn.Parameter] = {}
        E, H, I, V = c.embedding_size, c.hidden_size, c.intermediate_size, c.vocab_size
        add = self._add
        add("albert.embeddings.word_embeddings.weight", V, E)
        add("albert.embeddings.position_embeddings.weight", c.max_position_embeddings, E)
        add("albert.embeddings.token_type_embeddings.weight", c.type_vocab_size, E)
        with torch.no_grad():
            self._p["albert.embeddings.word_embeddings.weight"][c.pad_token_id].zero_()
        add("albert.embeddings.LayerNorm.weight", E, init="ones")
        add("albert.embeddings.LayerNorm.bias", E, init="zeros")
        add("albert.encoder.embedding_hidden_mapping_in.weight", H, E)
        add("albert.encoder.embedding_hidden_mapping_in.bias", H, init="zeros")
        for g in range(c.num_hidden_groups):
            for i in range(c.inner_group_num):
                pre = _layer_prefix(g, i)
                add(pre + "full_layer_layer_norm.weight", H, init="ones")
                add(pre + "full_layer_layer_norm.bias", H, init="zeros")
                for n in ("query", "key", "value"):
                    add(pre + f"attention.{n}.weight", H, H)
                for n in ("query", "key", "value"):
                    add(pre + f"attention.{n}.bias", H, init="zeros")
                add(pre + "attention.dense.weight", H, H)
                add(pre + "attention.dense.bias", H, init="zeros")
                add(pre + "attention.LayerNorm.weight", H, init="ones")
                add(pre + "attention.LayerNorm.bias", H, init="zeros")
                add(pre + "ffn.weight", I, H)
                add(pre + "ffn.bias", I, init="zeros")
                add(pre + "ffn_output.weight", H, I)
                add(pre + "ffn_output.bias", H, init="zeros")
        if self.add_pooler:
            add("albert.pooler.weight", H, H)
            add("albert.pooler.bias", H, init="zeros")
        self._add_heads()
        self.flat: Optional[FlatParams] = None

    def _add(self, name, *shape, init="normal"):
        t = torch.empty(*shape)
        if init == "normal":
            t.normal_(0.0, self.config.initializer_range)
        elif init == "ones":
            t.fill_(1.0)
        else:
            t.zero_()
        p = nn.Parameter(t)
        self._p[name] = p
        self.register_parameter(name.replace(".", "__"), p)

    def _add_heads(self):
        pass

    def hf_named_parameters(self):
        return list(self._p.items())

    def materialize(self, device=None) -> FlatParams:
        device = torch.device(device) if device is not None else next(iter(self._p.values())).device
        for p in self._p.values():
            p.data = p.data.to(device)
        self.flat = FlatParams(self.hf_named_parameters(), device=device)
        return self.flat

    def hf_state_dict(self) -> Dict[str, torch.Tensor]:
        return {k: v.detach() for k, v in self._p.items()}

    @torch.no_grad()
    def load_hf_state_dict(self, sd: Dict[str, torch.Tensor], strict: bool = True):
        missing = [k for k in self._p if k not in sd]
        if strict and missing:
            raise KeyError(f"missing keys: {missing[:5]}...")
        for k, p in self._p.items():
            if k in sd:
                p.data.copy_(sd[k].to(p.dtype))
        if self.flat is not None:
            self.flat.refresh_bf16()

    def save_pretrained(self, directory: str):
        os.makedirs(directory, exist_ok=True)
        self.config.save_pretrained(directory)
        sd = {k: v.detach().float().cpu().contiguous().clone() for k, v in self.hf_state_dict().items()}
        torch.save(sd, os.path.join(directory, "pytorch_model.bin"))

    @classmethod
    def from_pretrained(cls, directory: str, strict: Optional[bool] = None, **config_overrides):
        cfg = AlbertConfig.from_pretrained(directory)
        for k, v in config_overrides.items():
            setattr(cfg, k, v)
        model = cls(cfg)
        sd_path = os.path.join(directory, "pytorch_model.bin")
        if os.path.exists(sd_path):
            sd = torch.load(sd_path, map_location="cpu", weights_only=True)
        else:
            from safetensors.torch import load_file

            sd = load_file(os.path.join(directory, "model.safetensors"))
        if strict is None:
            strict = all(k in sd for k in model._p if not k.startswith("albert."))
        model.load_hf_state_dict(sd, strict=strict)
        return model

    def resize_token_embeddings(self, n: int):
        c = self.config
        if n == c.vocab_size:
            return
        assert self.flat is None, "resize before materialize()"
        for key in ("albert.embeddings.word_embeddings.weight", "predictions.bias"):
            if key not in self._p:
                continue
            old = self._p[key].data
            new = torch.empty((n,) + tuple(old.shape[1:]))
            if key.endswith("weight"):
                new.normal_(0.0, c.initializer_range)
            else:
                new.zero_()
            k = min(n, old.shape[0])
            new[:k] = old[:k]
            self._p[key].data = new
        c.vocab_size = n

    def no_decay_names(self) -> List[str]:
        return [n for n in self._p if any(nd in n for nd in ("bias", "LayerNorm.weight"))]

    def _layer_views(self, g: int, i: int):
        f = self.flat
        pre = _layer_prefix(g, i)
        H = self.config.hidden_size
        return dict(
            wqkv=f.span(f.bf16, pre + "attention.query.weight", pre + "attention.value.weight", (3 * H, H)),
            gwqkv=f.span(f.grad, pre + "attention.query.weight", pre + "attention.value.weight", (3 * H, H)),
            bqkv=f.span(f.bf16, pre + "attention.query.bias", pre + "attention.value.bias", (3 * H,)),
            bqkv32=f.span(f.fp32, pre + "attention.query.bias", pre + "attention.value.bias", (3 * H,)),
            bo32=f.p(pre + "attention.dense.bias"), b132=f.p(pre + "ffn.bias"), b232=f.p(pre + "ffn_output.bias"),
            gbqkv=f.span(f.grad, pre + "attention.query.bias", pre + "attention.value.bias", (3 * H,)),
            wo=f.w(pre + "attention.dense.weight"), gwo=f.g(pre + "attention.dense.weight"),
            bo=f.w(pre + "attention.dense.bias"), gbo=f.g(pre + "attention.dense.bias"),
            ln1g=f.p(pre + "attention.LayerNorm.weight"), ln1b=f.p(pre + "attention.LayerNorm.bias"),
            gln1g=f.g(pre + "attention.LayerNorm.weight"), gln1b=f.g(pre + "attention.LayerNorm.bias"),
            w1=f.w(pre + "ffn.weight"), gw1=f.g(pre + "ffn.weight"), b1=f.w(pre + "ffn.bias"), gb1=f.g(pre + "ffn.bias"),
            w2=f.w(pre + "ffn_output.weight"), gw2=f.g(pre + "ffn_output.weight"),
            b2=f.w(pre + "ffn_output.bias"), gb2=f.g(pre + "ffn_output.bias"),
            ln2g=f.p(pre + "full_layer_layer_norm.weight"), ln2b=f.p(pre + "full_layer_layer_norm.bias"),
            gln2g=f.g(pre + "full_layer_layer_norm.weight"), gln2b=f.g(pre + "full_layer_layer_norm.bias"),
        )

    def _albert_layer(self, h, lv, mask, S):
        c = self.config
        return _AlbertLayerFn.apply(h, mask, lv, c.num_attention_heads, S, c.layer_norm_eps)

    def _packed(self, pack_sequences, input_ids, attention_mask, token_type_ids, lengths, labels=None):
        if not (self.pack_sequences if pack_sequences is None else pack_sequences):
            return None
        batch = {"input_ids": input_ids, "attention_mask": attention_mask, "token_type_ids": token_type_ids}
        if labels is not None:
            batch["labels"] = labels
        return pack_batch(batch, lengths, self.config.pad_token_id)

    def encode(self, input_ids=None, attention_mask=None, token_type_ids=None, packed: Optional[PackedBatch] = None):
        assert self.flat is not None, "call model.materialize(device) first"
        c, f = self.config, self.flat
        if packed is not None:
            return self._encode_packed(packed), None
        B, S = input_ids.shape
        Sp = (S + 63) // 64 * 64
        if attention_mask is None:
            attention_mask = torch.ones_like(input_ids)
        if Sp != S:
            pad = Sp - S
            input_ids = F.pad(input_ids, (0, pad), value=c.pad_token_id)
            attention_mask = F.pad(attention_mask, (0, pad), value=0)
            if token_type_ids is not None:
                token_type_ids = F.pad(token_type_ids, (0, pad), value=0)
        assert Sp <= c.max_position_embeddings, "sequence longer than max_position_embeddings"
        am = attention_mask.bool()
        mbias = torch.where(am, 0.0, NEG_BIG).to(torch.float32).contiguous()
        lens = am.sum(1, dtype=torch.int32)
        prefix = (am == (torch.arange(Sp, device=am.device) < lens[:, None])).all()
        kvinfo = torch.cat([lens, prefix.to(torch.int32).view(1)]).contiguous()
        mask = (mbias, kvinfo)
        emb = "albert.embeddings."
        x = ops.embed_layernorm(
            input_ids, token_type_ids, f.p(emb + "word_embeddings.weight"), f.p(emb + "position_embeddings.weight"),
            f.p(emb + "token_type_embeddings.weight"), f.p(emb + "LayerNorm.weight"), f.p(emb + "LayerNorm.bias"),
            grads=(f.g(emb + "word_embeddings.weight"), f.g(emb + "position_embeddings.weight"),
                   f.g(emb + "token_type_embeddings.weight"), f.g(emb + "LayerNorm.weight"),
                   f.g(emb + "LayerNorm.bias")),
            eps=c.layer_norm_eps)
        return self._layers(x, mask, Sp), Sp

    def _encode_packed(self, packed: PackedBatch):
        c, f = self.config, self.flat
        assert packed.max_slot <= c.max_position_embeddings, "sequence longer than max_position_embeddings"
        D = c.hidden_size // c.num_attention_heads
        if D not in ops.FUSED_HEAD_DIMS:
            raise RuntimeError(f"dedloc_amd: pack_sequences needs a fused attention head size {ops.FUSED_HEAD_DIMS}, "
                               f"this model has head_dim {D}")
        emb = "albert.embeddings."
        x = ops.embed_layernorm_packed(
            packed.input_ids, packed.token_type_ids, packed.positions, f.p(emb + "word_embeddings.weight"),
            f.p(emb + "position_embeddings.weight"), f.p(emb + "token_type_embeddings.weight"),
            f.p(emb + "LayerNorm.weight"), f.p(emb + "LayerNorm.bias"),
            grads=(f.g(emb + "word_embeddings.weight"), f.g(emb + "position_embeddings.weight"),
                   f.g(emb + "token_type_embeddings.weight"), f.g(emb + "LayerNorm.weight"),
                   f.g(emb + "LayerNorm.bias")),
            eps=c.layer_norm_eps)
        return self._layers(x, packed, 0)

    def _layers(self, x, mask, Sp):
        c, f = self.config, self.flat
        m = "albert.encoder.embedding_hidden_mapping_in."
        h = ops.linear(x, f.w(m + "weight"), f.w(m + "bias"), f.g(m + "weight"), f.g(m + "bias"))
        views = [[self._layer_views(g, i) for i in range(c.inner_group_num)] for g in range(c.num_hidden_groups)]
        if _DGRAD_WT and torch.is_grad_enabled():
            views = [[_with_transposed_weights(lv) for lv in row] for row in views]
        per_group = c.num_hidden_layers // c.num_hidden_groups
        group_of = [int(layer / per_group) for layer in range(c.num_hidden_layers)]
        for layer in range(c.num_hidden_layers):
            g = group_of[layer]
            uses = [x for x in range(c.num_hidden_layers) if group_of[x] == g]
            for i in range(c.inner_group_num):
                lv = views[g][i]
                if _SHARED_WGRAD and torch.is_grad_enabled():
                    lv = dict(lv, wg_first=layer == uses[-1], wg_last=layer == uses[0])
                h = self._albert_layer(h, lv, mask, Sp)
        return h

    def num_parameters(self) -> int:
        return sum(p.numel() for p in self._p.values())


class AlbertForPreTraining(AlbertPreTrainedModel):

    def _add_heads(self):
        c = self.config
        E, H, V = c.embedding_size, c.hidden_size, c.vocab_size
        add = self._add
        add("predictions.bias", V, init="zeros")
        add("predictions.dense.weight", E, H)
        add("predictions.dense.bias", E, init="zeros")
        add("predictions.LayerNorm.weight", E, init="ones")
        add("predictions.LayerNorm.bias", E, init="zeros")
        add("sop_classifier.classifier.weight", 2, H)
        add("sop_classifier.classifier.bias", 2, init="zeros")

    def hf_state_dict(self) -> Dict[str, torch.Tensor]:
        sd = super().hf_state_dict()
        sd["predictions.decoder.weight"] = sd["albert.embeddings.word_embeddings.weight"]
        sd["predictions.decoder.bias"] = sd["predictions.bias"]
        return sd

    def _trunk(self, input_ids, attention_mask, token_type_ids, labels, mlm_positions, pack_sequences, lengths):
        pk = self._packed(pack_sequences, input_ids, attention_mask, token_type_ids, lengths,
                          labels if mlm_positions is None else None)
        if pk is not None:
            h, _ = self.encode(packed=pk)
            return h, None, pk, pk.row_start
        h, Sp = self.encode(input_ids, attention_mask, token_type_ids)
        return h, Sp, None, torch.arange(input_ids.shape[0], device=h.device) * Sp

    @staticmethod
    def _mlm_targets(pk, row0, S, Sp, labels, mlm_positions, mlm_labels):
        if mlm_positions is None and labels is not None:
            if pk is not None:
                flat_lab = pk.extras["labels"]
                rows = torch.nonzero(flat_lab != -100).squeeze(1)
                return rows, flat_lab[rows]
            flat_lab = labels.reshape(-1)
            pos = torch.nonzero(flat_lab != -100).squeeze(1)
            b_idx, s_idx = pos // S, pos % S
            return b_idx * Sp + s_idx, flat_lab[pos]
        if mlm_positions is not None:
            return (row0[:, None] + mlm_positions).reshape(-1), mlm_labels.reshape(-1)
        return None, None

    def _mlm_logits(self, h, rows):
        c, f = self.config, self.flat
        hm = h.index_select(0, rows)
        p = "predictions."
        t = ops.linear(hm, f.w(p + "dense.weight"), f.w(p + "dense.bias"), f.g(p + "dense.weight"),
                       f.g(p + "dense.bias"))
        t = ops.gelu_new(t)
        t = ops.add_layernorm(t, None, f.p(p + "LayerNorm.weight"), f.p(p + "LayerNorm.bias"),
                              f.g(p + "LayerNorm.weight"), f.g(p + "LayerNorm.bias"), c.layer_norm_eps)
        wname = "albert.embeddings.word_embeddings.weight"
        return ops.linear(t, f.w(wname), f.w(p + "bias"), f.g(wname), f.g(p + "bias"))

    def _sop_logits(self, h, B, Sp, pk, row0):
        c, f = self.config, self.flat
        cls = h.index_select(0, row0) if pk is not None else h.view(B, Sp, -1)[:, 0].contiguous()
        pooled = ops.tanh(ops.linear(cls, f.w("albert.pooler.weight"), f.w("albert.pooler.bias"),
                                     f.g("albert.pooler.weight"), f.g("albert.pooler.bias")))
        if self.training and c.classifier_dropout_prob > 0:
            pooled = F.dropout(pooled, c.classifier_dropout_prob, True)
        s = "sop_classifier.classifier."
        return ops.linear(pooled, f.w(s + "weight"), f.w(s + "bias"), f.g(s + "weight"), f.g(s + "bias"))

    def evaluate_batch(self, batch, lengths=None):
        was_training = self.training
        self.eval()
        try:
            with torch.no_grad():
                ids = batch["input_ids"]
                B, S = ids.shape
                labels, pos = batch.get("labels"), batch.get("mlm_positions")
                h, Sp, pk, row0 = self._trunk(ids, batch.get("attention_mask"), batch.get("token_type_ids"), labels,
                                              pos, None, lengths)
                rows, tgt = self._mlm_targets(pk, row0, S, Sp, labels, pos, batch.get("mlm_labels"))
                if rows is None:
                    raise ValueError("evaluate_batch needs MLM targets: labels or mlm_positions/mlm_labels")
                mlm = ops.eval_cross_entropy(self._mlm_logits(h, rows), tgt, topk=(1, 5))
                sop = ops.eval_cross_entropy(self._sop_logits(h, B, Sp, pk, row0), batch["sentence_order_label"],
                                             topk=(1,))
        finally:
            self.train(was_training)
        return {"mlm_loss_sum": mlm["loss_sum"], "mlm_count": mlm["count"], "mlm_top1": mlm["top1"],
                "mlm_top5": mlm["top5"], "sop_loss_sum": sop["loss_sum"], "sop_count": sop["count"],
                "sop_correct": sop["top1"]}

    def forward(self, input_ids, attention_mask=None, token_type_ids=None, labels=None, sentence_order_label=None,
                mlm_positions=None, mlm_labels=None, return_logits=False, pack_sequences=None, lengths=None):
        B, S = input_ids.shape
        h, Sp, pk, row0 = self._trunk(input_ids, attention_mask, token_type_ids, labels, mlm_positions,
                                      pack_sequences, lengths)
        out = {}
        rows, tgt = self._mlm_targets(pk, row0, S, Sp, labels, mlm_positions, mlm_labels)
        loss = None
        if rows is not None:
            logits = self._mlm_logits(h, rows)
            mlm_loss = ops.cross_entropy(logits, tgt)
            out["mlm_loss"] = mlm_loss
            loss = mlm_loss
            if return_logits:
                out["prediction_logits_masked"] = logits
        sop_logits = self._sop_logits(h, B, Sp, pk, row0)
        out["sop_logits"] = sop_logits
        if sentence_order_label is not None:
            sop_loss = ops.cross_entropy(sop_logits, sentence_order_label)
            out["sop_loss"] = sop_loss
            loss = sop_loss if loss is None else loss + sop_loss
        out["loss"] = loss
        return out


class AlbertForSequenceClassification(AlbertPreTrainedModel):

    def __init__(self, config: AlbertConfig, num_labels: Optional[int] = None):
        self.num_labels = int(num_labels or config.num_labels or 2)
        config.num_labels = self.num_labels
        super().__init__(config)

    def _add_heads(self):
        self._add("classifier.weight", self.num_labels, self.config.hidden_size)
        self._add("classifier.bias", self.num_labels, init="zeros")

    def forward(self, input_ids, attention_mask=None, token_type_ids=None, labels=None, pack_sequences=None,
                lengths=None):
        c, f = self.config, self.flat
        B = input_ids.shape[0]
        pk = self._packed(pack_sequences, input_ids, attention_mask, token_type_ids, lengths)
        if pk is not None:
            h, _ = self.encode(packed=pk)
            cls = h.index_select(0, pk.row_start)
        else:
            h, Sp = self.encode(input_ids, attention_mask, token_type_ids)
            cls = h.view(B, Sp, -1)[:, 0].contiguous()
        pooled = ops.tanh(ops.linear(cls, f.w("albert.pooler.weight"), f.w("albert.pooler.bias"),
                                     f.g("albert.pooler.weight"), f.g("albert.pooler.bias")))
        if self.training and c.classifier_dropout_prob > 0:
            pooled = F.dropout(pooled, c.classifier_dropout_prob, True)
        logits = ops.linear(pooled, f.w("classifier.weight"), f.w("classifier.bias"), f.g("classifier.weight"),
                            f.g("classifier.bias"))
        out = {"logits": logits}
        if labels is not None:
            if self.num_labels == 1:
                out["loss"] = F.mse_loss(logits.float().view(-1), labels.float().view(-1))
            else:
                out["loss"] = ops.cross_entropy(logits, labels)
        return out


class AlbertForTokenClassification(AlbertPreTrainedModel):

    add_pooler = False

    def __init__(self, config: AlbertConfig, num_labels: Optional[int] = None):
        self.num_labels = int(num_labels or config.num_labels or 2)
        config.num_labels = self.num_labels
        super().__init__(config)

    def _add_heads(self):
        self._add("classifier.weight", self.num_labels, self.config.hidden_size)
        self._add("classifier.bias", self.num_labels, init="zeros")

    def forward(self, input_ids, attention_mask=None, token_type_ids=None, labels=None, pack_sequences=None,
                lengths=None):
        c, f = self.config, self.flat
        B, S = input_ids.shape
        pk = self._packed(pack_sequences, input_ids, attention_mask, token_type_ids, lengths, labels)
        if pk is not None:
            h, _ = self.encode(packed=pk)
        else:
            h, Sp = self.encode(input_ids, attention_mask, token_type_ids)
        if self.training and c.classifier_dropout_prob > 0:
            h = F.dropout(h, c.classifier_dropout_prob, True)
        logits = ops.linear(h, f.w("classifier.weight"), f.w("classifier.bias"), f.g("classifier.weight"),
                            f.g("classifier.bias"))
        if pk is not None:
            out = {"logits": unpack_rows(logits, pk, S)}
            if labels is not None:
                out["loss"] = ops.cross_entropy(logits, pk.extras["labels"])
            return out
        out = {"logits": logits.view(B, Sp, -1)[:, :S]}
        if labels is not None:
            lab = labels
            if Sp != S:
                lab = F.pad(labels, (0, Sp - S), value=-100)
            out["loss"] = ops.cross_entropy(logits, lab.reshape(-1))
        return out


def flops_per_sample(config: AlbertConfig, seq_len: int, masked_per_seq: int) -> float:
    c = config
    H, I, E = c.hidden_size, c.intermediate_size, c.embedding_size
    per_tok_layer = 2 * (4 * H * H + 2 * H * I)
    attn = 2 * 2 * seq_len * H
    fwd = seq_len * (c.num_hidden_layers * (per_tok_layer + attn) + 2 * E * H)
    fwd += masked_per_seq * (2 * H * E + 2 * E * c.vocab_size)
    return 3.0 * fwd
```

dedloc_amd/ops/__init__.py:

```python
from __future__ import annotations

import math

import torch

from . import _lib
from ._lib import load_native, native_loaded

OPS = torch.ops.dedloc


def _needs_grad(*xs):
    return any(isinstance(x, torch.Tensor) and x.requires_grad for x in xs)


class _Linear(torch.autograd.Function):
    @staticmethod
    def forward(ctx, x, w, b, gw, gb, epilogue):
        ctx.save_for_backward(x, w)
        ctx.gw, ctx.gb = gw, gb
        return OPS.gemm(x, w, b, None, False, True, epilogue)

    @staticmethod
    def backward(ctx, dy):
        x, w = ctx.saved_tensors
        dy = dy.contiguous()
        dx = OPS.gemm(dy, w, None, None, False, False, 0)
        if ctx.gw is not None:
            OPS.gemm_acc_f32(dy, x, ctx.gw, True, False)
        if ctx.gb is not None:
            OPS.bias_grad(dy, ctx.gb, True)
        return dx, None, None, None, None, None


def linear(x, w, b=None, gw=None, gb=None):
    return _Linear.apply(x, w, b, gw, gb, 0)


class _Gelu(torch.autograd.Function):
    @staticmethod
    def forward(ctx, h):
        ctx.save_for_backward(h)
        return OPS.gelu_fwd(h)

    @staticmethod
    def backward(ctx, dy):
        (h,) = ctx.saved_tensors
        return OPS.gelu_bwd(dy.contiguous(), h)


def gelu_new(h):
    return _Gelu.apply(h)


class _Tanh(torch.autograd.Function):
    @staticmethod
    def forward(ctx, x):
        y = OPS.tanh_fwd(x)
        ctx.save_for_backward(y)
        return y

    @staticmethod
    def backward(ctx, dy):
        (y,) = ctx.saved_tensors
        return OPS.tanh_bwd(dy.contiguous(), y)


def tanh(x):
    return _Tanh.apply(x)


class _AddLayerNorm(torch.autograd.Function):
    @staticmethod
    def forward(ctx, x, res, gamma, beta, ggamma, gbeta, eps):
        y, s, mean, rstd = OPS.layernorm_fwd(x, res, gamma, beta, eps)
        ctx.save_for_backward(s, gamma, mean, rstd)
        ctx.ggamma, ctx.gbeta, ctx.has_res = ggamma, gbeta, res is not None
        return y

    @staticmethod
    def backward(ctx, dy):
        s, gamma, mean, rstd = ctx.saved_tensors
        gg, gb = ctx.ggamma, ctx.gbeta
        if gg is None:
            gg = torch.zeros_like(gamma)
            gb = torch.zeros_like(gamma)
        ds = OPS.layernorm_bwd(dy.contiguous(), s, gamma, mean, rstd, gg, gb, True)
        return ds, (ds if ctx.has_res else None), None, None, None, None, None


def add_layernorm(x, res, gamma, beta, ggamma=None, gbeta=None, eps=1e-12):
    return _AddLayerNorm.apply(x, res, gamma, beta, ggamma, gbeta, eps)


_LOG2E = math.log2(math.e)


def _bmm_f32(a, b):
    return OPS.bmm(a, b, True)


def _bmm(a, b):
    return OPS.bmm(a, b, False)


def _attn_split(qkv, H, S):
    T, ld = qkv.shape
    D = ld // (3 * H)
    B = T // S
    x = qkv.view(B, S, 3, H, D).permute(2, 0, 3, 1, 4)
    return (x[0].reshape(B * H, S, D), x[1].reshape(B * H, S, D), x[2].reshape(B * H, S, D)), B, D


def attn_composed_fwd(qkv, mbias, H, S, scale):
    (q, k, v), B, D = _attn_split(qkv, H, S)
    s = _bmm_f32(q, k.transpose(1, 2))
    p, lse = OPS.attn_softmax_fwd(s, mbias, H, scale * _LOG2E)
    del s
    o = _bmm(p, v)
    return o.view(B, H, S, D).transpose(1, 2).reshape(B * S, H * D), lse.view(B, H, S)


def attn_composed_bwd(qkv, mbias, out, dout, lse, H, S, scale, dbias=None):
    (q, k, v), B, D = _attn_split(qkv, H, S)
    do = dout.view(B, S, H, D).transpose(1, 2).reshape(B * H, S, D)
    o = out.view(B, S, H, D).transpose(1, 2).reshape(B * H, S, D)
    s = _bmm_f32(q, k.transpose(1, 2))
    dp = _bmm_f32(do, v.transpose(1, 2))
    delta = (do.float() * o.float()).sum(-1)
    p, ds = OPS.attn_softmax_bwd(s, dp, mbias, lse.reshape(-1).contiguous(), delta.reshape(-1), H,
                                 scale * _LOG2E, scale)
    del s, dp
    dv = _bmm(p.transpose(1, 2), do)
    dq = _bmm(ds, k)
    dk = _bmm(ds.transpose(1, 2), q)
    g = torch.stack([dq, dk, dv], 0).view(3, B, H, S, D).permute(1, 3, 0, 2, 4).reshape(B * S, 3 * H * D)
    if dbias is not None:
        HD = H * D
        dbias[:HD] += g[:, :HD].float().sum(0)
        dbias[2 * HD:] += dout.float().sum(0)
    return g


FUSED_HEAD_DIMS = (64, 128)


def _fused_attention(qkv, H):
    return not qkv.is_cuda or qkv.shape[-1] // (3 * H) in FUSED_HEAD_DIMS


def attn_fwd(qkv, mbias, H, S, scale, kvinfo=None):
    if _fused_attention(qkv, H):
        return OPS.attn_fwd(qkv, mbias, H, S, scale, kvinfo)
    return attn_composed_fwd(qkv, mbias, H, S, scale)


def attn_bwd(qkv, mbias, out, dout, lse, H, S, scale, kvinfo=None, dbias=None):
    if _fused_attention(qkv, H):
        return OPS.attn_bwd(qkv, mbias, out, dout, lse, H, S, scale, kvinfo, dbias)
    return attn_composed_bwd(qkv, mbias, out, dout, lse, H, S, scale, dbias)


def attn_varlen_fwd(qkv, packed, H, scale):
    D = qkv.shape[-1] // (3 * H)
    if D not in FUSED_HEAD_DIMS:
        raise RuntimeError(f"dedloc_amd: packed batches need a fused attention head size {FUSED_HEAD_DIMS}, "
                           f"got head_dim {D}")
    return OPS.attn_varlen_fwd(qkv, packed.seqinfo, packed.seqinfo_host, H, scale)


def attn_varlen_bwd(qkv, packed, out, dout, lse, H, scale, dbias=None):
    return OPS.attn_varlen_bwd(qkv, packed.seqinfo, packed.seqinfo_host, out, dout, lse, H, scale, dbias)


class _Attention(torch.autograd.Function):
    @staticmethod
    def forward(ctx, qkv, mbias, H, S, scale):
        out, lse = attn_fwd(qkv, mbias, H, S, scale)
        ctx.save_for_backward(qkv, out, lse)
        ctx.mbias, ctx.H, ctx.S, ctx.scale = mbias, H, S, scale
        return out

    @staticmethod
    def backward(ctx, dout):
        qkv, out, lse = ctx.saved_tensors
        dqkv = attn_bwd(qkv, ctx.mbias, out, dout.contiguous(), lse, ctx.H, ctx.S, ctx.scale)
        return dqkv, None, None, None, None


def attention(qkv, mbias, num_heads, seq_len, scale=None):
    d = qkv.shape[-1] // (3 * num_heads)
    scale = scale if scale is not None else 1.0 / math.sqrt(d)
    return _Attention.apply(qkv, mbias, num_heads, seq_len, scale)


class _EmbedLN(torch.autograd.Function):
    @staticmethod
    def forward(ctx, anchor, ids, tt, wemb, pemb, temb, gamma, beta, gw, gp, gt, ggamma, gbeta, S, eps):
        y, s, mean, rstd = OPS.embed_ln_fwd(ids, tt, wemb, pemb, temb, gamma, beta, S, eps)
        ctx.save_for_backward(ids, s, gamma, mean, rstd)
        ctx.tt = tt
        ctx.grads = (gw, gp, gt, ggamma, gbeta)
        ctx.S = S
        return y

    @staticmethod
    def backward(ctx, dy):
        ids, s, gamma, mean, rstd = ctx.saved_tensors
        gw, gp, gt, gg, gb = ctx.grads
        if gw is not None:
            ds = OPS.layernorm_bwd(dy.contiguous(), s, gamma, mean, rstd, gg, gb, True)
            OPS.embed_bwd(ds, ids, ctx.tt, gw, gp, gt, ctx.S)
        return (None,) * 15


class _EmbedLNPacked(torch.autograd.Function):
    @staticmethod
    def forward(ctx, anchor, ids, tt, pos, wemb, pemb, temb, gamma, beta, gw, gp, gt, ggamma, gbeta, eps):
        y, s, mean, rstd = OPS.embed_ln_pos_fwd(ids, tt, pos, wemb, pemb, temb, gamma, beta, eps)
        ctx.save_for_backward(ids, pos, s, gamma, mean, rstd)
        ctx.tt = tt
        ctx.grads = (gw, gp, gt, ggamma, gbeta)
        return y

    @staticmethod
    def backward(ctx, dy):
        ids, pos, s, gamma, mean, rstd = ctx.saved_tensors
        gw, gp, gt, gg, gb = ctx.grads
        if gw is not None:
            ds = OPS.layernorm_bwd(dy.contiguous(), s, gamma, mean, rstd, gg, gb, True)
            OPS.embed_pos_bwd(ds, ids, ctx.tt, pos, gw, gp, gt)
        return (None,) * 15


def embed_layernorm_packed(ids, tt, pos, wemb, pemb, temb, gamma, beta, grads=(None,) * 5, eps=1e-12):
    anchor = torch.empty(0, device=ids.device, requires_grad=True)
    return _EmbedLNPacked.apply(anchor, ids.contiguous(), None if tt is None else tt.contiguous(), pos.contiguous(),
                                wemb, pemb, temb, gamma, beta, *grads, eps)


def embed_layernorm(ids, tt, wemb, pemb, temb, gamma, beta, grads=(None,) * 5, eps=1e-12):
    B, S = ids.shape
    anchor = torch.empty(0, device=ids.device, requires_grad=True)
    return _EmbedLN.apply(anchor, ids.reshape(-1).contiguous(), None if tt is None else tt.reshape(-1).contiguous(),
                          wemb, pemb, temb, gamma, beta, *grads, S, eps)


class _CrossEntropy(torch.autograd.Function):
    @staticmethod
    def forward(ctx, logits, labels, ignore_index):
        loss, dlogits = OPS.xent_fwd_bwd(logits, labels, False, ignore_index)
        ctx.save_for_backward(dlogits)
        return loss

    @staticmethod
    def backward(ctx, dloss):
        (dlogits,) = ctx.saved_tensors
        if dlogits.dtype == torch.bfloat16 and dlogits.is_contiguous():
            OPS.scale_by_(dlogits, dloss.reshape(1).float())
            return dlogits, None, None
        return dlogits.mul_(dloss.to(dlogits.dtype)), None, None


def cross_entropy(logits, labels, ignore_index=-100):
    return _CrossEntropy.apply(logits.contiguous(), labels.reshape(-1).contiguous(), ignore_index)


@torch.no_grad()
def eval_cross_entropy(logits, labels, ignore_index=-100, topk=(1, 5)):
    if not (logits.dim() == 2 and logits.stride(1) == 1 and logits.stride(0) >= logits.shape[1]):
        logits = logits.contiguous()
    row_loss, row_rank = OPS.xent_eval(logits, labels.reshape(-1).contiguous(), ignore_index)
    valid = row_rank >= 0
    out = {"loss_sum": row_loss.sum(dtype=torch.float64), "count": valid.sum()}
    for k in topk:
        out[f"top{k}"] = (valid & (row_rank < k)).sum()
    return out


@torch.no_grad()
def knn_topk(q, bank, k, splits=0):
    return OPS.knn_topk(q.to(torch.bfloat16).contiguous(), bank.to(torch.bfloat16).contiguous(), int(k), int(splits))


@torch.no_grad()
def knn_classify(q, bank, bank_labels, targets, num_classes, k=200, sigma=0.1, splits=0):
    k = max(1, min(int(k), bank.shape[0]))
    vals, idx = knn_topk(q, bank, k, splits)
    targets = targets.to(torch.int64).reshape(-1).contiguous()
    pred, rank = OPS.knn_vote(vals, idx, bank_labels.to(torch.int32).contiguous(), targets, int(num_classes),
                              float(sigma))
    count = ((targets >= 0) & (targets < int(num_classes))).sum()
    return {"count": count, "top1": (rank == 0).sum(), "top5": ((rank >= 0) & (rank < 5)).sum(), "pred": pred,
            "rank": rank}


__all__ = [
    "linear", "gelu_new", "tanh", "add_layernorm", "attention", "embed_layernorm", "cross_entropy",
    "eval_cross_entropy", "knn_topk", "knn_classify", "OPS",
    "load_native", "native_loaded",
]

load_native()
```

dedloc_amd/ops/_lib.py:

```python
from __future__ import annotations

import math
import os

import torch
import torch.nn.functional as F

LIB = torch.library.Library("dedloc", "DEF")

_SCHEMAS = [
    "layernorm_fwd(Tensor x, Tensor? res, Tensor gamma, Tensor beta, float eps) -> (Tensor, Tensor, Tensor, Tensor)",
    "layernorm_bwd(Tensor dy, Tensor s, Tensor gamma, Tensor mean, Tensor rstd, Tensor(a!) dgamma, Tensor(b!) dbeta, bool accumulate, Tensor(c!)? dsum=None) -> Tensor",
    "gelu_fwd(Tensor h) -> Tensor",
    "gelu_bwd(Tensor dy, Tensor h, Tensor(a!)? dbias=None) -> Tensor",
    "tanh_fwd(Tensor x) -> Tensor",
    "tanh_bwd(Tensor dy, Tensor y) -> Tensor",
    "bias_grad(Tensor dy, Tensor(a!) dbias, bool accumulate) -> ()",
    "cast_bf16(Tensor x, Tensor(a!) out) -> ()",
    "lamb_step(Tensor(a!) p, Tensor g, Tensor(b!) m, Tensor(c!) v, Tensor chunk_tensor, Tensor chunk_start, Tensor chunk_len, Tensor tensor_wd, Tensor(d!) norms, float beta1, float beta2, float eps, float step_size, float clamp_value, float grad_scale) -> ()",
    "larc_sgd_step(Tensor(a!) p, Tensor g, Tensor(b!) buf, Tensor chunk_tensor, Tensor chunk_start, Tensor chunk_len, Tensor tensor_wd, Tensor(c!) norms, float lr, float momentum, float trust_coef, float eps, bool clip, bool first_step, float grad_scale) -> ()",
    "grad_norm_clip(Tensor(a!) g, float max_norm, Tensor(b!) part, Tensor(c!) out) -> ()",
    "axpby(Tensor(a!) y, Tensor x, float a, float b, Tensor? flag=None, Tensor? bdiv=None) -> ()",
    "add_slabs_zero_(Tensor(a!) out, Tensor(b!) slabs) -> ()",
    "scale_by_(Tensor(a!) x, Tensor s) -> ()",
    "pack(Tensor src, Tensor(a!) dst, float weight) -> ()",
    "reduce_parts(Tensor parts, int nparts, Tensor(a!) out, float inv_total) -> ()",
    "unpack(Tensor src, Tensor(a!) dst, Tensor? snap, bool add=False) -> ()",
    "reduce_delta(Tensor parts, Tensor weights, Tensor(a!) deltas) -> ()",
    "pack_q8(Tensor src, Tensor(a!) dst) -> ()",
    "reduce_delta_q8(Tensor parts, Tensor weights, Tensor(a!) deltas, int n) -> ()",
    "unpack_q8(Tensor src, Tensor(a!) dst, bool add=False) -> ()",
    "embed_ln_fwd(Tensor ids, Tensor? tt, Tensor wemb, Tensor pemb, Tensor temb, Tensor gamma, Tensor beta, int S, float eps) -> (Tensor, Tensor, Tensor, Tensor)",
    "embed_bwd(Tensor ds, Tensor ids, Tensor? tt, Tensor(a!) dwemb, Tensor(b!) dpemb, Tensor(c!) dtemb, int S) -> ()",
    "xent_fwd_bwd(Tensor logits, Tensor labels, bool inplace, int ignore_index) -> (Tensor, Tensor)",
    "xent_eval(Tensor logits, Tensor labels, int ignore_index) -> (Tensor, Tensor)",
    "knn_topk(Tensor q, Tensor bank, int k, int splits=0) -> (Tensor, Tensor)",
    "knn_vote(Tensor vals, Tensor idx, Tensor bank_labels, Tensor targets, int num_classes, float sigma) "
    "-> (Tensor, Tensor)",
    "attn_fwd(Tensor qkv, Tensor? mbias, int H, int S, float scale, Tensor? kvinfo=None) -> (Tensor, Tensor)",
    "attn_bwd(Tensor qkv, Tensor? mbias, Tensor out, Tensor dout, Tensor lse, int H, int S, float scale, "
    "Tensor? kvinfo=None, Tensor(a!)? dbias=None) -> Tensor",
    "attn_varlen_fwd(Tensor qkv, Tensor seqinfo, Tensor seqinfo_host, int H, float scale) -> (Tensor, Tensor)",
    "attn_varlen_bwd(Tensor qkv, Tensor seqinfo, Tensor seqinfo_host, Tensor out, Tensor dout, Tensor lse, int H, "
    "float scale, Tensor(a!)? dbias=None) -> Tensor",
    "embed_ln_pos_fwd(Tensor ids, Tensor? tt, Tensor pos, Tensor wemb, Tensor pemb, Tensor temb, Tensor gamma, Tensor beta, float eps) -> (Tensor, Tensor, Tensor, Tensor)",
    "embed_pos_bwd(Tensor ds, Tensor ids, Tensor? tt, Tensor pos, Tensor(a!) dwemb, Tensor(b!) dpemb, Tensor(c!) dtemb) -> ()",
    "attn_softmax_fwd(Tensor s, Tensor? mbias, int H, float c) -> (Tensor, Tensor)",
    "attn_softmax_bwd(Tensor s, Tensor dp, Tensor? mbias, Tensor lse, Tensor delta, int H, float c, float scale) "
    "-> (Tensor, Tensor)",
    "gemm(Tensor a, Tensor b, Tensor? bias, Tensor? residual, bool trans_a, bool trans_b, int epilogue) -> Tensor",
    "bmm(Tensor a, Tensor b, bool out_f32=False) -> Tensor",
    "gemm_acc_f32(Tensor a, Tensor b, Tensor(a!) c, bool trans_a, bool trans_b) -> ()",
    "gemm_acc_f32_shared(Tensor a, Tensor b, Tensor(a!) c, bool trans_a, bool trans_b, bool first, bool last) -> ()",
    "gemm_gelu(Tensor x, Tensor w, Tensor bias, bool trans_w=False) -> (Tensor, Tensor)",
    "sinkhorn(Tensor scores, int bs, float eps, int iters) -> Tensor",
    "swav_ce(Tensor scores, Tensor q, Tensor(a!) dscores, Tensor(b!) loss, float temperature, float scale) -> ()",
    "swav_ce_multi(Tensor scores, Tensor q, int[] crops, Tensor(a!) dscores, Tensor(b!) loss, float temperature, "
    "float scale) -> ()",
    "row_normalize_(Tensor(a!) w) -> ()",
    "maxpool_fwd(Tensor x) -> (Tensor, Tensor)",
    "maxpool_bwd(Tensor dy, Tensor arg, int H, int W) -> Tensor",
    "avgpool_fwd(Tensor x) -> Tensor",
    "avgpool_bwd(Tensor dy, int H, int W) -> Tensor",
    "l2norm_fwd(Tensor x, float eps) -> (Tensor, Tensor)",
    "l2norm_bwd(Tensor dy, Tensor y, Tensor rinv) -> Tensor",
    "multicrop(Tensor pool, Tensor params, int size, int rad, float[] mean, float[] std) -> Tensor",
    "multicrop_ragged(Tensor bytes, Tensor meta, Tensor params, int size, int rad, float[] mean, float[] std) -> Tensor",
    "bn_fwd(Tensor x, Tensor? res, Tensor gamma, Tensor beta, Tensor(a!)? running_mean, Tensor(b!)? running_var, "
    "float eps, float momentum, bool relu, int groups=1, Tensor(c!)? sums=None, bool stats_ready=False) "
    "-> (Tensor, Tensor, Tensor)",
    "bn_apply(Tensor x, Tensor? res, Tensor gamma, Tensor beta, Tensor mean, Tensor rstd, bool relu, int groups=1) "
    "-> Tensor",
    "bn_bwd(Tensor dy, Tensor y, Tensor x, Tensor mean, Tensor rstd, Tensor gamma, bool relu, bool want_dres, "
    "Tensor(a!)? sums=None, Tensor(b!)? dgamma_acc=None, Tensor(c!)? dbeta_acc=None, Tensor? beta=None, "
    "bool stats_ready=False) -> (Tensor, Tensor, Tensor, Tensor)",
    "conv2d_dgrad_bn(Tensor dy, Tensor w, int stride, int pad, int H, int W, Tensor? residual, Tensor x, Tensor? y, "
    "Tensor mean, Tensor rstd, Tensor gamma, Tensor beta, Tensor(a!) sums, int groups, Tensor[]? wds=None) "
    "-> (Tensor, bool)",
    "bn_bwd_prep(Tensor(a!) g, Tensor x, Tensor? y, Tensor mean, Tensor rstd, Tensor gamma, Tensor beta, "
    "Tensor(b!) sums, int groups) -> Tensor",
    "gemm_dgelu(Tensor dy, Tensor w, Tensor F, Tensor(a!) dbias, bool trans_w=False) -> Tensor",
    "gemm_gelu_d(Tensor x, Tensor w, Tensor bias, bool trans_w=False) -> (Tensor, Tensor)",
    "gemm_dmul(Tensor dy, Tensor w, Tensor D, Tensor(a!) dbias, bool trans_w=False) -> Tensor",
    "conv2d_fwd(Tensor x, Tensor w, int stride, int pad, Tensor? cols=None) -> Tensor",
    "conv2d_fwd_stats(Tensor x, Tensor w, int stride, int pad, Tensor(a!) sums, int groups, Tensor? cols=None) "
    "-> Tensor",
    "conv2d_bn_act(Tensor x, Tensor w, Tensor scale, Tensor shift, Tensor? res, bool relu, int stride, int pad) "
    "-> Tensor",
    "im2col_stem(Tensor x, int R, int S, int stride, int pad) -> Tensor",
    "conv2d_dgrad(Tensor dy, Tensor w, int stride, int pad, int H, int W, Tensor? residual=None, "
    "Tensor[]? wds=None) -> Tensor",
    "conv2d_dgrad_weights(Tensor w, int stride, int pad) -> Tensor[]",
    "conv2d_dgrad_weights_batched(Tensor[] ws, int[] strides, int[] pads) -> Tensor[]",
    "conv2d_wgrad(Tensor dy, Tensor x, Tensor(a!) dw, int stride, int pad, Tensor? cols=None) -> ()",
]
for _s in _SCHEMAS:
    LIB.define(_s)

_NATIVE = {"loaded": False, "path": None, "error": None}


def _impl(name):
    def deco(fn):
        LIB.impl(name, fn, "CPU")
        return fn

    return deco


def load_native(required: bool | None = None) -> bool:
    if _NATIVE["loaded"]:
        return True
    if required is None:
        required = torch.cuda.is_available()
    pkg = os.path.dirname(os.path.dirname(os.path.abspath(__file__)))
    path = os.environ.get("DEDLOC_NATIVE_LIB") or os.path.join(pkg, "_C.so")
    try:
        if not os.path.exists(path):
            raise FileNotFoundError(f"{path} not built (run python -m dedloc_amd._build)")
        torch.ops.load_library(path)
        _NATIVE.update(loaded=True, path=path)
        return True
    except Exception as e:
        _NATIVE["error"] = repr(e)
        if required:
            raise ImportError(
                "dedloc_amd: the gfx950 kernel library could not be loaded on a GPU machine; refusing to run "
                f"without it ({e})"
            ) from e
        return False


def native_loaded() -> bool:
    return _NATIVE["loaded"]


def _bf(x):
    return x.to(torch.bfloat16)


@_impl("layernorm_fwd")
def _ln_fwd_cpu(x, res, gamma, beta, eps):
    s = x.float() if res is None else (x.float() + res.float())
    s_b = _bf(s)
    sf = s_b.float() if res is not None else x.float()
    mean = sf.mean(-1)
    var = ((sf - mean.unsqueeze(-1)) ** 2).mean(-1)
    rstd = torch.rsqrt(var + eps)
    y = (sf - mean.unsqueeze(-1)) * rstd.unsqueeze(-1) * gamma + beta
    D = x.shape[-1]
    return _bf(y), (s_b if res is not None else x), mean.reshape(-1), rstd.reshape(-1)


@_impl("layernorm_bwd")
def _ln_bwd_cpu(dy, s, gamma, mean, rstd, dgamma, dbeta, accumulate, dsum=None):
    D = dy.shape[-1]
    g = dy.float().reshape(-1, D)
    xh = (s.float().reshape(-1, D) - mean.unsqueeze(-1)) * rstd.unsqueeze(-1)
    dg = (g * xh).sum(0)
    db = g.sum(0)
    if accumulate:
        dgamma.add_(dg)
        dbeta.add_(db)
    else:
        dgamma.copy_(dg)
        dbeta.copy_(db)
    gy = g * gamma
    a = gy.mean(-1, keepdim=True)
    b = (gy * xh).mean(-1, keepdim=True)
    ds = _bf(rstd.unsqueeze(-1) * (gy - a - xh * b))
    if dsum is not None:
        dsum.add_(ds.float().sum(0))
    return ds.reshape(dy.shape)


def _gelu_tanh(x):
    return 0.5 * x * (1.0 + torch.tanh(math.sqrt(2.0 / math.pi) * (x + 0.044715 * x.pow(3))))


@_impl("gelu_fwd")
def _gelu_fwd_cpu(h):
    return _bf(_gelu_tanh(h.float()))


@_impl("gelu_bwd")
def _gelu_bwd_cpu(dy, h, dbias=None):
    x = h.float()
    k0, k1 = math.sqrt(2.0 / math.pi), 0.044715
    s = torch.sigmoid(2 * k0 * (x + k1 * x ** 3))
    d = s + 2 * x * (s * (1 - s)) * (k0 * (1 + 3 * k1 * x * x))
    dh = _bf(dy.float() * d)
    if dbias is not None:
        dbias.add_(dh.float().reshape(-1, dh.shape[-1]).sum(0))
    return dh
# ... 259 lines not shown
    s_b = _bf(s)
    sf = s_b.float()
    mean = sf.mean(-1)
    rstd = torch.rsqrt(((sf - mean[:, None]) ** 2).mean(-1) + eps)
    y = (sf - mean[:, None]) * rstd[:, None] * gamma + beta
    return _bf(y), s_b, mean, rstd


@_impl("embed_pos_bwd")
def _embed_pos_bwd_cpu(ds, ids, tt, pos, dwemb, dpemb, dtemb):
    g = ds.float().reshape(-1, ds.shape[-1])
    dwemb.index_add_(0, ids.reshape(-1), g)
    dpemb.index_add_(0, pos.reshape(-1).long(), g)
    tti = tt.reshape(-1) if tt is not None else torch.zeros(g.shape[0], dtype=torch.long)
    dtemb.index_add_(0, tti, g)


@_impl("xent_fwd_bwd")
def _xent_cpu(logits, labels, inplace, ignore_index):
    x = logits.float().reshape(-1, logits.shape[-1])
    lab = labels.reshape(-1)
    valid = lab != ignore_index
    cnt = int(valid.sum())
    lse = torch.logsumexp(x, -1)
    safe = torch.where(valid, lab, torch.zeros_like(lab))
    rows = lse - x.gather(1, safe[:, None]).squeeze(1)
    scale = 1.0 / cnt if cnt > 0 else 0.0
    loss = (rows * valid).sum() * scale
    grad = torch.softmax(x, -1)
    grad[torch.arange(x.shape[0]), safe] -= 1.0
    grad = grad * valid[:, None] * scale
    g = _bf(grad).reshape(logits.shape)
    if inplace:
        logits.copy_(g)
        g = logits
    return loss.float(), g


@_impl("xent_eval")
def _xent_eval_cpu(logits, labels, ignore_index):
    V = logits.shape[-1]
    x = logits.float().reshape(-1, V)
    lab = labels.reshape(-1)
    valid = (lab != ignore_index) & (lab >= 0) & (lab < V)
    safe = torch.where(valid, lab, torch.zeros_like(lab))
    xl = x.gather(1, safe[:, None])
    col = torch.arange(V, device=x.device)[None, :]
    rank = ((x > xl) | ((x == xl) & (col < safe[:, None]))).sum(1)
    loss = torch.logsumexp(x, -1) - xl.squeeze(1)
    loss = torch.where(valid, loss, torch.where(lab == ignore_index, 0.0, float("nan")).float())
    rank = torch.where(valid, rank, torch.full_like(rank, -1))
    return loss.float(), rank.to(torch.int32)


@_impl("knn_topk")
def _knn_topk_cpu(q, bank, k, splits=0):
    if q.dim() != 2 or bank.dim() != 2 or q.shape[1] != bank.shape[1]:
        raise RuntimeError("knn_topk: q [Q, D] and bank [N, D]")
    if q.dtype != torch.bfloat16 or bank.dtype != torch.bfloat16 or not (q.is_contiguous() and bank.is_contiguous()):
        raise RuntimeError("knn_topk: q and bank must be contiguous bf16 tensors")
    Q, N = q.shape[0], bank.shape[0]
    if not 1 <= k <= min(256, N):
        raise RuntimeError(f"knn_topk: k = {k} must be in 1 .. min(256, N = {N})")
    if splits < 0:
        raise RuntimeError(f"knn_topk: splits = {splits} must be 0 (automatic) or positive")
    vals = torch.empty(Q, k, dtype=torch.float32)
    idx = torch.empty(Q, k, dtype=torch.int32)
    bf = bank.float().t()
    for r0 in range(0, Q, 512):
        s = q[r0:r0 + 512].float() @ bf
        v, i = torch.sort(s + 0.0, dim=1, descending=True, stable=True)
        vals[r0:r0 + 512], idx[r0:r0 + 512] = v[:, :k], i[:, :k].to(torch.int32)
    return vals, idx


@_impl("knn_vote")
def _knn_vote_cpu(vals, idx, bank_labels, targets, num_classes, sigma):
    if vals.dim() != 2 or idx.shape != vals.shape or vals.shape[1] < 1:
        raise RuntimeError("knn_vote: vals and idx must both be [Q, k] with k >= 1")
    if not 1 <= num_classes <= 8192 or not sigma > 0:
        raise RuntimeError("knn_vote: num_classes must be in 1 .. 8192 and sigma positive")
    Q, k = vals.shape
    C, N = int(num_classes), bank_labels.numel()
    if targets.numel() != Q or N < 1:
        raise RuntimeError("knn_vote: one target per row and at least one bank label")
    i = idx.long()
    inside = (i >= 0) & (i < N)
    cls = bank_labels.long()[i.clamp(0, N - 1)]
    votes = inside & (cls >= 0) & (cls < C)
    w = torch.exp((vals.float() - vals[:, :1].float()) / torch.tensor(sigma, dtype=torch.float32))
    sums = torch.zeros(Q, C, dtype=torch.float32)
    voted = torch.zeros(Q, C, dtype=torch.bool)
    rows = torch.arange(Q)
    for j in range(k):
        r, c = rows[votes[:, j]], cls[votes[:, j], j]
        sums[r, c] += w[votes[:, j], j]
        voted[r, c] = True
    col = torch.arange(C)[None, :]
    best = sums.max(1, keepdim=True).values
    pred = torch.where(sums == best, col, C).min(1).values
    t = targets.reshape(-1)
    valid = (t >= 0) & (t < C)
    safe = torch.where(valid, t, torch.zeros_like(t))
    pt = sums.gather(1, safe[:, None])
    rank = ((sums > pt) | ((sums == pt) & (col < safe[:, None]))).sum(1)
    valid = valid & voted.gather(1, safe[:, None]).squeeze(1)
    return pred.to(torch.int32), torch.where(valid, rank, torch.full_like(rank, -1)).to(torch.int32)


def _attn_probs(qkv, mbias, H, S, scale):
    T, ld = qkv.shape
    D = ld // (3 * H)
    B = T // S
    x = qkv.float().reshape(B, S, 3, H, D)
    q, k, v = x[:, :, 0].transpose(1, 2), x[:, :, 1].transpose(1, 2), x[:, :, 2].transpose(1, 2)
    s = torch.matmul(q, k.transpose(-1, -2)) * scale
    if mbias is not None:
        s = s + mbias.reshape(B, 1, 1, S) / math.log2(math.e)
    return q, k, v, s


@_impl("attn_fwd")
def _attn_fwd_cpu(qkv, mbias, H, S, scale, kvinfo=None):
    q, k, v, s = _attn_probs(qkv, mbias, H, S, scale)
    B, _, _, D = q.shape
    lse = torch.logsumexp(s, -1)
    p = torch.softmax(s, -1)
    o = torch.matmul(p, v).transpose(1, 2).reshape(B * S, H * D)
    return _bf(o), (lse * math.log2(math.e)).contiguous()


@_impl("attn_bwd")
def _attn_bwd_cpu(qkv, mbias, out, dout, lse, H, S, scale, kvinfo=None, dbias=None):
    q, k, v, s = _attn_probs(qkv, mbias, H, S, scale)
    B, _, _, D = q.shape
    p = torch.softmax(s, -1)
    do = dout.float().reshape(B, S, H, D).transpose(1, 2)
    o = out.float().reshape(B, S, H, D).transpose(1, 2)
    dv = torch.matmul(p.transpose(-1, -2), do)
    dp = torch.matmul(do, v.transpose(-1, -2))
    delta = (do * o).sum(-1, keepdim=True)
    ds = p * (dp - delta)
    dq = torch.matmul(ds, k) * scale
    dk = torch.matmul(ds.transpose(-1, -2), q) * scale
    g = torch.stack([dq, dk, dv], dim=2)
    g = _bf(g.permute(0, 3, 2, 1, 4).reshape(B * S, 3 * H * D))
    if dbias is not None:
        HD = H * D
        dbias[:HD] += g[:, :HD].float().sum(0)
        dbias[2 * HD:] += dout.float().reshape(-1, HD).sum(0)
    return g


def packed_layout(seqinfo_host, T):
    v = [int(x) for x in seqinfo_host.reshape(-1).tolist()]
    if len(v) < 3 or len(v) % 2 == 0:
        raise RuntimeError("seqinfo must be int32[2B + 1] (B + 1 row offsets, B lengths)")
    B = (len(v) - 1) // 2
    rows, lens = v[:B + 1], v[B + 1:]
    if rows[0] != 0 or rows[B] != T:
        raise RuntimeError(f"row offsets must run from 0 to T = {T} (got {rows[0]} .. {rows[B]})")
    for b in range(B):
        slot = rows[b + 1] - rows[b]
        if rows[b] % 64 or rows[b + 1] % 64:
            raise RuntimeError(f"row offset of sequence {b} is not a multiple of 64")
        if slot < 64 or not 1 <= lens[b] <= slot:
            raise RuntimeError(f"length {lens[b]} of sequence {b} is outside 1 .. its slot of {slot} rows")
    return rows, lens


def _slot_mbias(slot, n):
    return torch.where(torch.arange(slot) < n, 0.0, -1.0e30).float().reshape(1, slot)


def _check_packed_head_dim(qkv, H, what):
    D = qkv.shape[-1] // (3 * H)
    if D not in (64, 128) or qkv.shape[-1] != 3 * H * D:
        raise RuntimeError(f"dedloc_amd: {what}: head_dim {D} is not supported by the fused attention kernels; "
                           "supported head sizes are 64 and 128")


@_impl("attn_varlen_fwd")
def _attn_varlen_fwd_cpu(qkv, seqinfo, seqinfo_host, H, scale):
    T = qkv.shape[0]
    _check_packed_head_dim(qkv, H, "attn_varlen_fwd")
    rows, lens = packed_layout(seqinfo_host, T)
    out = torch.empty(T, qkv.shape[1] // 3, dtype=qkv.dtype)
    lse = torch.empty(H, T, dtype=torch.float32)
    for b, n in enumerate(lens):
        r0, r1 = rows[b], rows[b + 1]
        o, l = _attn_fwd_cpu(qkv[r0:r1], _slot_mbias(r1 - r0, n), H, r1 - r0, scale)
        out[r0:r1] = o
        lse[:, r0:r1] = l[0]
    return out, lse


@_impl("attn_varlen_bwd")
def _attn_varlen_bwd_cpu(qkv, seqinfo, seqinfo_host, out, dout, lse, H, scale, dbias=None):
    T = qkv.shape[0]
    _check_packed_head_dim(qkv, H, "attn_varlen_bwd")
    rows, lens = packed_layout(seqinfo_host, T)
    g = torch.empty_like(qkv)
    for b, n in enumerate(lens):
        r0, r1 = rows[b], rows[b + 1]
        g[r0:r1] = _attn_bwd_cpu(qkv[r0:r1], _slot_mbias(r1 - r0, n), out[r0:r1], dout[r0:r1], None, H, r1 - r0,
                                 scale, None, dbias)
    return g


def _softmax_logits(s, mbias, H, c):
    S = s.shape[-1]
    x = s.float().reshape(-1, H, S, S) * c
    if mbias is not None:
        x = x + mbias.reshape(-1, 1, 1, S)
    return x.reshape(s.shape)


@_impl("attn_softmax_fwd")
def _attn_softmax_fwd_cpu(s, mbias, H, c):
    x = _softmax_logits(s, mbias, H, c)
    lse = torch.logsumexp(x / math.log2(math.e), -1) * math.log2(math.e)
    return _bf(torch.exp2(x - lse[..., None])), lse.reshape(-1).contiguous()


@_impl("attn_softmax_bwd")
def _attn_softmax_bwd_cpu(s, dp, mbias, lse, delta, H, c, scale):
    p = torch.exp2(_softmax_logits(s, mbias, H, c) - lse.reshape(s.shape[:-1])[..., None])
    return _bf(p), _bf(p * (dp.float() - delta.reshape(s.shape[:-1])[..., None]) * scale)


@_impl("gemm")
def _gemm_cpu(a, b, bias, residual, trans_a, trans_b, epilogue):
    A = a.float().t() if trans_a else a.float()
    Bm = b.float().t() if trans_b else b.float()
    c = A @ Bm
    if bias is not None:
        c = c + bias.float()
    if residual is not None:
        c = c + residual.float()
    if epilogue == 1:
        c = _gelu_tanh(c)
    return _bf(c)


@_impl("gemm_gelu")
def _gemm_gelu_cpu(x, w, bias, trans_w=False):
    h = _bf(x.float() @ (w.float() if trans_w else w.float().t()) + bias.float())
    return h, _bf(_gelu_tanh(h.float()))


@_impl("gemm_dgelu")
def _gemm_dgelu_cpu(dy, w, F, dbias, trans_w=False):
    dg = _bf(dy.float() @ (w.float().t() if trans_w else w.float()))
    return _gelu_bwd_cpu(dg, F, dbias)


def _gelu_grad_tanh(x):
    k0, k1 = 0.7978845608028654, 0.044715
    t = torch.tanh(k0 * (x + k1 * x ** 3))
    return 0.5 * (1 + t) + 0.5 * x * (1 - t * t) * k0 * (1 + 3 * k1 * x * x)


@_impl("gemm_gelu_d")
def _gemm_gelu_d_cpu(x, w, bias, trans_w=False):
    h = _bf(x.float() @ (w.float() if trans_w else w.float().t()) + bias.float()).float()
    return _bf(_gelu_grad_tanh(h)), _bf(_gelu_tanh(h))


@_impl("gemm_dmul")
def _gemm_dmul_cpu(dy, w, D, dbias, trans_w=False):
    dg = _bf(dy.float() @ (w.float().t() if trans_w else w.float())).float()
    c = _bf(dg * D.float())
    dbias.add_(c.float().sum(0))
    return c


@_impl("gemm_acc_f32")
def _gemm_acc_cpu(a, b, c, trans_a, trans_b):
    A = a.float().t() if trans_a else a.float()
    Bm = b.float().t() if trans_b else b.float()
    c.add_(A @ Bm)


@_impl("gemm_acc_f32_shared")
def _gemm_acc_shared_cpu(a, b, c, trans_a, trans_b, first, last):
    _gemm_acc_cpu(a, b, c, trans_a, trans_b)


@_impl("sinkhorn")
def _sinkhorn_cpu(scores, bs, eps, iters):
    Q = torch.exp((scores.float() - scores.max()) / eps).t()
    Q = Q / Q.sum()
    K, n = Q.shape
    r = torch.ones(K) / K
    c = torch.ones(n) / n
    curr = Q.sum(1)
    for _ in range(iters):
        Q = Q * (r / curr).unsqueeze(1)
        Q = Q * (c / Q.sum(0)).unsqueeze(0)
        curr = Q.sum(1)
    Q = (Q / Q.sum(0, keepdim=True)).t()
    return Q[-bs:].contiguous()


@_impl("swav_ce")
def _swav_ce_cpu(scores, q, dscores, loss, temperature, scale):
# ... 248 lines not shown
```

Before: 1062 samples/s.

## Compute only masked-token query rows in the last ALBERT layer

Adds compact-query attention kernels (forward and backward) that take a separate q tensor holding only selected rows per sequence, with K/V still covering the full sequence. The model trunk uses them in the final layer so that only the rows feeding the MLM loss are computed. This removes attention, FFN and projection work for unlabeled positions in that layer. It adds gather/scatter logic and new kernel template paths, and it only applies when labels or mlm_positions are supplied and head_dim is 64.

```diff
diff --git a/dedloc_amd/_build.py b/dedloc_amd/_build.py
--- a/dedloc_amd/_build.py
+++ b/dedloc_amd/_build.py
@@ -54,7 +54,8 @@
     for src in hip_srcs:
         obj = os.path.join(BUILD, os.path.basename(src).replace(".hip", ".o"))
         objs.append(obj)
-        if _newer(obj, [src] + headers + [__file__]):
+        included = [os.path.join(CSRC, "kernels", f) for f in HIP_INCLUDES.get(os.path.basename(src), [])]
+        if _newer(obj, [src] + included + headers + [__file__]):
             jobs_list.append(["hipcc", *hip_flags, *FILE_FLAGS.get(os.path.basename(src), []), *inc, "-c", src,
                               "-o", obj])
 
@@ -101,6 +102,7 @@
 _OBJS: list = []
 HIP_FLAGS = ["-O3", "-std=c++17", "-fPIC", "-ffp-contract=fast", "-munsafe-fp-atomics"]
 FILE_FLAGS: dict = {"comm_q8.hip": ["-ffp-contract=on"]}
+HIP_INCLUDES: dict = {"attention_compact_q.hip": ["attention.hip"]}
 
 
 def _link(objs, out, tlib, verbose):
diff --git a/dedloc_amd/csrc/bindings.cpp b/dedloc_amd/csrc/bindings.cpp
--- a/dedloc_amd/csrc/bindings.cpp
+++ b/dedloc_amd/csrc/bindings.cpp
@@ -512,6 +512,84 @@
                     bf(dqkv), dbp, (int)B, (int)H, (int)S, (int)D, (float)scale, cur_stream(qkv)),
         "attn_bwd");
   return dqkv;
+}
+
+struct CompactLayout {
+  int64_t B, Sq, D, ld;
+};
+inline CompactLayout compact_layout(const at::Tensor& q, const at::Tensor& kv, const at::Tensor& qcnt, int64_t H,
+                                    int64_t S, const char* what) {
+  expect(q, at::kBFloat16, "q");
+  expect(qcnt, at::kInt, "qcnt");
+  TORCH_CHECK(kv.is_cuda() && kv.scalar_type() == at::kBFloat16 && kv.dim() == 2 && kv.stride(1) == 1, what,
+              ": kv must be a 2-D bf16 GPU tensor with unit column stride");
+  TORCH_CHECK(H >= 1 && S >= 64 && S % 64 == 0, what, ": S = ", S, " must be a positive multiple of 64");
+  const int64_t T = kv.size(0), B = T / S, D = kv.size(1) / (2 * H), ld = kv.stride(0);
+  TORCH_CHECK(D == 64 && kv.size(1) == 2 * H * D, "dedloc_amd: ", what, ": compact queries exist for head_dim 64 only (kv has ",
+              kv.size(1), " columns for ", H, " heads)");
+  TORCH_CHECK(B >= 1 && B * S == T, what, ": kv must have B*S rows");
+  TORCH_CHECK(ld >= 2 * H * D && ld % 8 == 0 && reinterpret_cast<uintptr_t>(kv.data_ptr()) % 16 == 0, what,
+              ": kv rows must be 16-byte aligned");
+  TORCH_CHECK(q.dim() == 2 && q.size(1) == H * D && q.size(0) % B == 0, what, ": q must be [B*Sq, H*D]");
+  const int64_t Sq = q.size(0) / B;
+  TORCH_CHECK(Sq >= 64 && Sq % 64 == 0 && Sq <= S, what, ": the query slot Sq = ", Sq,
+              " must be a multiple of 64 in 64 .. S = ", S);
+  TORCH_CHECK(qcnt.numel() == B, what, ": qcnt must be int32[B]");
+  return CompactLayout{B, Sq, D, ld};
+}
+
+std::tuple<at::Tensor, at::Tensor> attn_fwd_q(const at::Tensor& q, const at::Tensor& kv, const at::Tensor& qcnt,
+                                              const c10::optional<at::Tensor>& mbias, int64_t H, int64_t S,
+                                              double scale, const c10::optional<at::Tensor>& kvinfo) {
+  const CompactLayout L = compact_layout(q, kv, qcnt, H, S, "attn_fwd_q");
+  auto out = at::empty({L.B * L.Sq, H * L.D}, q.options());
+  auto lse = at::empty({L.B, H, L.Sq}, q.options().dtype(at::kFloat));
+  const float* mb = nullptr;
+  if (mbias.has_value()) {
+    expect(*mbias, at::kFloat, "mbias");
+    TORCH_CHECK(mbias->numel() == L.B * S, "attn_fwd_q: mbias must be [B, S]");
+    mb = f32(*mbias);
+  }
+  check(dl_attn_fwd_q(cbf(q), reinterpret_cast<const bf16_t*>(kv.data_ptr()), L.ld, mb, kvinfo_ptr(kvinfo, L.B),
+                      qcnt.data_ptr<int>(), bf(out), H * L.D, f32(lse), (int)L.B, (int)H, (int)S, (int)L.Sq, (int)L.D,
+                      (float)scale, cur_stream(q)),
+        "attn_fwd_q");
+  return {out, lse};
+}
+
+std::tuple<at::Tensor, at::Tensor, at::Tensor> attn_bwd_q(const at::Tensor& q, const at::Tensor& kv,
+                                                          const at::Tensor& qcnt,
+                                                          const c10::optional<at::Tensor>& mbias,
+                                                          const at::Tensor& out, const at::Tensor& dout,
+                                                          const at::Tensor& lse, int64_t H, int64_t S, double scale,
+                                                          const c10::optional<at::Tensor>& kvinfo,
+                                                          const c10::optional<at::Tensor>& dbias) {
+  const CompactLayout L = compact_layout(q, kv, qcnt, H, S, "attn_bwd_q");
+  expect(out, at::kBFloat16, "out");
+  expect(dout, at::kBFloat16, "dout");
+  expect(lse, at::kFloat, "lse");
+  TORCH_CHECK(out.numel() == q.numel() && dout.numel() == q.numel() && lse.numel() == L.B * H * L.Sq,
+              "attn_bwd_q: out / dout must be [B*Sq, H*D] and lse [B, H, Sq]");
+  auto dq = at::empty_like(q);
+  auto dkv = at::empty({L.B * S, 2 * H * L.D}, q.options());
+  auto delta = at::empty({L.B, H, L.Sq}, q.options().dtype(at::kFloat));
+  const float* mb = nullptr;
+  if (mbias.has_value()) {
+    expect(*mbias, at::kFloat, "mbias");
+    TORCH_CHECK(mbias->numel() == L.B * S, "attn_bwd_q: mbias must be [B, S]");
+    mb = f32(*mbias);
+  }
+  float* dbp = nullptr;
+  if (dbias.has_value()) {
+    expect(*dbias, at::kFloat, "dbias");
+    TORCH_CHECK(dbias->numel() == 3 * H * L.D, "dbias must have 3*H*D elements");
+    dbp = f32(*dbias);
+  }
+  check(dl_attn_bwd_q(cbf(q), reinterpret_cast<const bf16_t*>(kv.data_ptr()), L.ld, mb, kvinfo_ptr(kvinfo, L.B),
+                      qcnt.data_ptr<int>(), cbf(out), cbf(dout), H * L.D, f32(lse), f32(delta), bf(dq), bf(dkv), dbp,
+                      (int)L.B, (int)H, (int)S, (int)L.Sq, (int)L.D, (float)scale, cur_stream(q)),
+        "attn_bwd_q");
+  return {dq, dkv, delta};
 }
 
 struct PackedLayout {
@@ -1718,6 +1796,8 @@
   m.impl("knn_vote", &knn_vote);
   m.impl("attn_fwd", &attn_fwd);
   m.impl("attn_bwd", &attn_bwd);
+  m.impl("attn_fwd_q", &attn_fwd_q);
+  m.impl("attn_bwd_q", &attn_bwd_q);
   m.impl("attn_varlen_fwd", &attn_varlen_fwd);
   m.impl("attn_varlen_bwd", &attn_varlen_bwd);
   m.impl("embed_ln_pos_fwd", &embed_ln_pos_fwd);
diff --git a/dedloc_amd/csrc/include/dl_kernels.h b/dedloc_amd/csrc/include/dl_kernels.h
--- a/dedloc_amd/csrc/include/dl_kernels.h
+++ b/dedloc_amd/csrc/include/dl_kernels.h
@@ -190,6 +190,11 @@
 int dl_attn_bwd(const bf16_t* qkv, long ld, const float* mbias, const int* kvinfo, const bf16_t* out,
                 const bf16_t* dout, long ldo, const float* lse, float* delta, bf16_t* dqkv, float* dbias, int B, int H,
                 int S, int D, float scale, hipStream_t st);
+int dl_attn_fwd_q(const bf16_t* q, const bf16_t* kv, long ld, const float* mbias, const int* kvinfo, const int* qcnt,
+                  bf16_t* out, long ldo, float* lse, int B, int H, int S, int Sq, int D, float scale, hipStream_t st);
+int dl_attn_bwd_q(const bf16_t* q, const bf16_t* kv, long ld, const float* mbias, const int* kvinfo, const int* qcnt,
+                  const bf16_t* out, const bf16_t* dout, long ldo, const float* lse, float* delta, bf16_t* dq,
+                  bf16_t* dkv, float* dbias, int B, int H, int S, int Sq, int D, float scale, hipStream_t st);
 int dl_attn_hd128_varlen_fwd(const bf16_t* qkv, long ld, const int* seqinfo, bf16_t* out, long ldo, float* lse, int B,
                              int T, int max_slot, int H, float scale, hipStream_t st);
 int dl_attn_hd128_varlen_bwd(const bf16_t* qkv, long ld, const int* seqinfo, const bf16_t* out, const bf16_t* dout,
diff --git a/dedloc_amd/csrc/kernels/attention.hip b/dedloc_amd/csrc/kernels/attention.hip
--- a/dedloc_amd/csrc/kernels/attention.hip
+++ b/dedloc_amd/csrc/kernels/attention.hip
@@ -177,26 +177,84 @@
   }
 }
 
-template <bool RING, int QS, int NW = 4, bool VARLEN = false>
+struct CompactQ {
+  const bf16_t* q;
+  bf16_t* dq;
+  bf16_t* dkv;
+  long lddkv;
+  const int* cnt;
+  int Sq;
+};
+struct NoCompactQ {};
+template <bool CQ>
+using CompactArg = std::conditional_t<CQ, CompactQ, NoCompactQ>;
+__device__ __forceinline__ NoCompactQ compact_arg() { return {}; }
+__device__ __forceinline__ const CompactQ& compact_arg(const CompactQ& cq) { return cq; }
+template <bool VARLEN, bool CQ>
+__device__ __forceinline__ long q_stat(const CompactArg<CQ>& cq, int b, int h, int H, int S, int T, long rb) {
+  if constexpr (CQ) return ((long)b * H + h) * cq.Sq;
+  else return seq_stat<VARLEN>(b, h, H, S, T, rb);
+}
+template <bool CQ>
+__device__ __forceinline__ long q_first(const CompactArg<CQ>& cq, int b, long rb) {
+  if constexpr (CQ) return (long)b * cq.Sq;
+  else return rb;
+}
+template <bool CQ>
+__device__ __forceinline__ int q_slot(const CompactArg<CQ>& cq, int S) {
+  if constexpr (CQ) return cq.Sq;
+  else return S;
+}
+template <bool CQ>
+__device__ __forceinline__ const bf16_t* q_head(const CompactArg<CQ>& cq, const bf16_t* qkv, long ld, long ldo, long rb,
+                                                 long qb, int h) {
+  if constexpr (CQ) return cq.q + qb * ldo + h * 64;
+  else return qkv + rb * ld + h * 64;
+}
+__device__ __forceinline__ void zero_rows64(bf16_t* g, long ld, int rows) {
+  if ((int)threadIdx.x < rows) {
+    uint4* p = reinterpret_cast<uint4*>(g + (long)threadIdx.x * ld);
+#pragma unroll
+    for (int i = 0; i < 8; ++i) p[i] = make_uint4(0u, 0u, 0u, 0u);
+  }
+}
+template <bool CQ>
+__device__ __forceinline__ int q_rows(const CompactArg<CQ>& cq, int b, int S) {
+  if constexpr (CQ) return max(1, min(cq.cnt[b], cq.Sq));
+  else return S;
+}
+
+template <bool RING, int QS, int NW = 4, bool VARLEN = false, typename... CQA>
 __global__ __launch_bounds__(64 * NW, NW == 8 ? 1 : 2) void attn_fwd_kernel(const bf16_t* __restrict__ qkv, long ld,
                                                           const float* __restrict__ mbias,
                                                           const int* __restrict__ kvinfo, bf16_t* __restrict__ out,
                                                           long ldo, float* __restrict__ lse, int B, int H, int S_,
-                                                          float sl2, int xcd) {
+                                                          float sl2, int xcd, CQA... cqa) {
+  constexpr bool CQ = sizeof...(CQA) == 1;
+  const CompactArg<CQ> cq = compact_arg(cqa...);
   __shared__ __attribute__((aligned(16))) uint8_t smem[RING ? NBUF * STAGE : 4 * TILE_BYTES + 2 * 64 * 4];
   const BlockId bid = block_id(xcd);
   const int b = bid.b, h = bid.h;
   const int lane = threadIdx.x & 63, w = threadIdx.x >> 6, r = lane & 31, hh = lane >> 5;
   const int S = seq_rows<VARLEN>(kvinfo, b, S_);
-  if constexpr (VARLEN) {
-    if (bid.x * (32 * QS * NW) >= S) return;
+  const int nq = q_rows<CQ>(cq, b, S);
+  if constexpr (VARLEN || CQ) {
+    if (bid.x * (32 * QS * NW) >= nq) {
+      if constexpr (CQ) {
+        const int q0 = bid.x * (32 * QS * NW);
+        zero_rows64(out + ((long)b * cq.Sq + q0) * ldo + h * HD, ldo, cq.Sq - q0);
+      }
+      return;
+    }
   }
   const long rb = seq_base<VARLEN>(kvinfo, b, S);
-  const bf16_t* Qg = qkv + rb * ld + h * HD;
+  const long qb = q_first<CQ>(cq, b, rb);
+  const long ldq = CQ ? ldo : ld;
+  const bf16_t* Qg = q_head<CQ>(cq, qkv, ld, ldo, rb, qb, h);
   bool use_len;
   FwdCtx c;
-  c.Kg = qkv + rb * ld + (long)H * HD + h * HD;
-  c.Vg = qkv + rb * ld + 2L * H * HD + h * HD;
+  c.Kg = qkv + rb * ld + (CQ ? 0L : (long)H * HD) + h * HD;
+  c.Vg = qkv + rb * ld + (CQ ? (long)H * HD : 2L * H * HD) + h * HD;
   c.ld = ld;
   c.S = S;
   c.kv_end = seq_kv_end<VARLEN>(kvinfo, B, b, S, use_len);
@@ -217,9 +275,9 @@
 #pragma unroll
   for (int u = 0; u < QS; ++u) {
     q[u] = bid.x * (32 * QS * NW) + w * (32 * QS) + 32 * u + r;
-    const int qc = min(q[u], S - 1);
-#pragma unroll
-    for (int ks = 0; ks < 4; ++ks) qf[u][ks] = gload8(Qg + (long)qc * ld + ks * 16 + 8 * hh);
+    const int qc = min(q[u], nq - 1);
+#pragma unroll
+    for (int ks = 0; ks < 4; ++ks) qf[u][ks] = gload8(Qg + (long)qc * ldq + ks * 16 + 8 * hh);
     if constexpr (RING) {
 #pragma unroll
       for (int ks = 0; ks < 4; ++ks) settle(qf[u][ks]);
@@ -256,13 +314,16 @@
 
 #pragma unroll
   for (int u = 0; u < QS; ++u) {
-    const bool live = q[u] < S;
-    store_row64(out + (rb + q[u]) * ldo + h * HD, o[u], 1.f / l[u], hh, live);
-    if (live && hh == 0) lse[seq_stat<VARLEN>(b, h, H, S, S_, rb) + q[u]] = m[u] + log2f(l[u]);
-  }
-}
-
-template <bool RING, int QS, bool VARLEN = false>
+    const bool live = q[u] < nq;
+    if constexpr (CQ)
+      store_row64(out + (qb + q[u]) * ldo + h * HD, o[u], live ? 1.f / l[u] : 0.f, hh, q[u] < cq.Sq);
+    else
+      store_row64(out + (qb + q[u]) * ldo + h * HD, o[u], 1.f / l[u], hh, live);
+    if (live && hh == 0) lse[q_stat<VARLEN, CQ>(cq, b, h, H, S, S_, rb) + q[u]] = m[u] + log2f(l[u]);
+  }
+}
+
+template <bool RING, int QS, bool VARLEN = false, typename... CQA>
 __global__ __launch_bounds__(256, 2) void attn_bwd_dq_kernel(const bf16_t* __restrict__ qkv, long ld,
                                                              const float* __restrict__ mbias,
                                                              const int* __restrict__ kvinfo,
@@ -270,19 +331,30 @@
                                                              long ldo, const float* __restrict__ lse,
                                                              float* __restrict__ delta, bf16_t* __restrict__ dqkv,
                                                              float* __restrict__ dbias, int B, int H, int S_, float sl2,
-                                                             float scale, int xcd) {
+                                                             float scale, int xcd, CQA... cqa) {
+  constexpr bool CQ = sizeof...(CQA) == 1;
+  const CompactArg<CQ> cq = compact_arg(cqa...);
   __shared__ __attribute__((aligned(16))) uint8_t smem[RING ? NBUF * STAGE : 4 * TILE_BYTES + 4 * 64 * 4];
   const BlockId bid = block_id(xcd);
   const int b = bid.b, h = bid.h;
   const int lane = threadIdx.x & 63, w = threadIdx.x >> 6, r = lane & 31, hh = lane >> 5;
   const int S = seq_rows<VARLEN>(kvinfo, b, S_);
-  if constexpr (VARLEN) {
-    if (bid.x * (128 * QS) >= S) return;
+  const int nq = q_rows<CQ>(cq, b, S);
+  if constexpr (VARLEN || CQ) {
+    if (bid.x * (128 * QS) >= nq) {
+      if constexpr (CQ) {
+        const int q0 = bid.x * (128 * QS);
+        zero_rows64(cq.dq + ((long)b * cq.Sq + q0) * ldo + h * HD, ldo, cq.Sq - q0);
+      }
+      return;
+    }
   }
   const long rb = seq_base<VARLEN>(kvinfo, b, S);
-  const bf16_t* Qg = qkv + rb * ld + h * HD;
-  const bf16_t* Kg = qkv + rb * ld + (long)H * HD + h * HD;
-  const bf16_t* Vg = qkv + rb * ld + 2L * H * HD + h * HD;
+  const long qb = q_first<CQ>(cq, b, rb);
+  const long ldq = CQ ? ldo : ld;
+  const bf16_t* Qg = q_head<CQ>(cq, qkv, ld, ldo, rb, qb, h);
+  const bf16_t* Kg = qkv + rb * ld + (CQ ? 0L : (long)H * HD) + h * HD;
+  const bf16_t* Vg = qkv + rb * ld + (CQ ? (long)H * HD : 2L * H * HD) + h * HD;
   bool use_len;
   const int kv_end = seq_kv_end<VARLEN>(kvinfo, B, b, S, use_len);
   const float* mb_g = (!use_len && mbias) ? mbias + rb : nullptr;
@@ -304,19 +376,19 @@
 #pragma unroll
   for (int u = 0; u < QS; ++u) {
     q[u] = bid.x * (128 * QS) + w * (32 * QS) + 32 * u + r;
-    const int qc = min(q[u], S - 1);
+    const int qc = min(q[u], nq - 1);
     dl[u] = 0.f;
 #pragma unroll
     for (int ks = 0; ks < 4; ++ks) {
-      qf[u][ks] = gload8(Qg + (long)qc * ld + ks * 16 + 8 * hh);
-      const long oo = (rb + qc) * ldo + h * HD + ks * 16 + 8 * hh;
+      qf[u][ks] = gload8(Qg + (long)qc * ldq + ks * 16 + 8 * hh);
+      const long oo = (qb + qc) * ldo + h * HD + ks * 16 + 8 * hh;
       df[u][ks] = gload8(dout + oo);
       const bf16x8 of = gload8(out + oo);
 #pragma unroll
       for (int e = 0; e < 8; ++e) dl[u] += (float)df[u][ks][e] * (float)of[e];
     }
     dl[u] += __shfl_xor(dl[u], 32, 64);
-    l2[u] = lse[seq_stat<VARLEN>(b, h, H, S, S_, rb) + qc];
+    l2[u] = lse[q_stat<VARLEN, CQ>(cq, b, h, H, S, S_, rb) + qc];
     if constexpr (RING) {
       settle(l2[u]);
       settle(dl[u]);
@@ -450,9 +522,12 @@
   for (int u = 0; u < QS; ++u) qe[u] = bid.x * (128 * QS) + w_ * (32 * QS) + 32 * u + r_;
 #pragma unroll
   for (int u = 0; u < QS; ++u) {
-    const bool live = qe[u] < S;
-    if (live && hh_ == 0) delta[seq_stat<VARLEN>(b, h, H, S, S_, rb) + qe[u]] = dl[u];
-    store_row64(dqkv + (rb + qe[u]) * ld + h * HD, dq[u], scale, hh_, live);
+    const bool live = qe[u] < nq;
+    if (live && hh_ == 0) delta[q_stat<VARLEN, CQ>(cq, b, h, H, S, S_, rb) + qe[u]] = dl[u];
+    if constexpr (CQ)
+      store_row64(cq.dq + (qb + qe[u]) * ldo + h * HD, dq[u], live ? scale : 0.f, hh_, qe[u] < cq.Sq);
+    else
+      store_row64(dqkv + (rb + qe[u]) * ld + h * HD, dq[u], scale, hh_, live);
   }
   if (dbias) {
     float* part = reinterpret_cast<float*>(smem);
@@ -463,7 +538,7 @@
       for (int i = 0; i < 16; ++i) {
         float v = 0.f;
 #pragma unroll
-        for (int u = 0; u < QS; ++u) v += qe[u] < S ? round_bf16(dq[u][t][i] * scale) : 0.f;
+        for (int u = 0; u < QS; ++u) v += qe[u] < nq ? round_bf16(dq[u][t][i] * scale) : 0.f;
         cq[t][i] = half_wave_sum(v);
       }
 #pragma unroll
@@ -472,7 +547,7 @@
       for (int e = 0; e < 8; ++e) {
         float v = 0.f;
 #pragma unroll
-        for (int u = 0; u < QS; ++u) v += qe[u] < S ? (float)df[u][ks][e] : 0.f;
+        for (int u = 0; u < QS; ++u) v += qe[u] < nq ? (float)df[u][ks][e] : 0.f;
         cd[ks][e] = half_wave_sum(v);
       }
     if (r_ == 0) {
@@ -499,11 +574,13 @@
   }
 }
 
-template <bool RING, int KS, bool VARLEN = false>
+template <bool RING, int KS, bool VARLEN = false, typename... CQA>
 __global__ __launch_bounds__(256, KS == 2 ? 1 : 2) void attn_bwd_dkdv_kernel(
     const bf16_t* __restrict__ qkv, long ld, const float* __restrict__ mbias, const int* __restrict__ kvinfo,
     const bf16_t* __restrict__ dout, long ldo, const float* __restrict__ lse, const float* __restrict__ delta,
-    bf16_t* __restrict__ dqkv, int B, int H, int S_, float sl2, float scale, int xcd) {
+    bf16_t* __restrict__ dqkv, int B, int H, int S_, float sl2, float scale, int xcd, CQA... cqa) {
+  constexpr bool CQ = sizeof...(CQA) == 1;
+  const CompactArg<CQ> cq = compact_arg(cqa...);
   __shared__ __attribute__((aligned(16))) uint8_t smem[RING ? NBUF * STAGE : 4 * TILE_BYTES + 2 * 2 * 64 * 4];
   const BlockId bid = block_id(xcd);
   const int b = bid.b, h = bid.h;
@@ -513,12 +590,24 @@
     if (bid.x * (128 * KS) >= S) return;
   }
   const long rb = seq_base<VARLEN>(kvinfo, b, S);
-  const bf16_t* Qg = qkv + rb * ld + h * HD;
-  const bf16_t* Kg = qkv + rb * ld + (long)H * HD + h * HD;
-  const bf16_t* Vg = qkv + rb * ld + 2L * H * HD + h * HD;
-  const bf16_t* dOg = dout + rb * ldo + h * HD;
-  const float* lse_g = lse + seq_stat<VARLEN>(b, h, H, S, S_, rb);
-  const float* del_g = delta + seq_stat<VARLEN>(b, h, H, S, S_, rb);
+  const int nq = q_rows<CQ>(cq, b, S);
+  const long qb = q_first<CQ>(cq, b, rb);
+  const long ldq = CQ ? ldo : ld;
+  const bf16_t* Qg = q_head<CQ>(cq, qkv, ld, ldo, rb, qb, h);
+  const bf16_t* Kg = qkv + rb * ld + (CQ ? 0L : (long)H * HD) + h * HD;
+  const bf16_t* Vg = qkv + rb * ld + (CQ ? (long)H * HD : 2L * H * HD) + h * HD;
+  const bf16_t* dOg = dout + qb * ldo + h * HD;
+  const float* lse_g = lse + q_stat<VARLEN, CQ>(cq, b, h, H, S, S_, rb);
+  const float* del_g = delta + q_stat<VARLEN, CQ>(cq, b, h, H, S, S_, rb);
+  bf16_t* dkv_g;
+  long ldd;
+  if constexpr (CQ) {
+    dkv_g = cq.dkv - (long)H * HD;
+    ldd = cq.lddkv;
+  } else {
+    dkv_g = dqkv;
+    ldd = ld;
+  }
   float* rowv = reinterpret_cast<float*>(smem + 4 * TILE_BYTES);
 
   int k[KS];
@@ -530,8 +619,8 @@
 #pragma unroll
     for (int u = 0; u < KS; ++u) {
       if (k[u] < S) {
-        bf16_t* dkp = dqkv + (rb + k[u]) * ld + (long)H * HD + h * HD;
-        bf16_t* dvp = dqkv + (rb + k[u]) * ld + 2L * H * HD + h * HD;
+        bf16_t* dkp = dkv_g + (rb + k[u]) * ldd + (long)H * HD + h * HD;
+        bf16_t* dvp = dkv_g + (rb + k[u]) * ldd + 2L * H * HD + h * HD;
 #pragma unroll
         for (int v = 0; v < 8; ++v) {
           store4(dkp + 8 * v + 4 * hh, 0.f, 0.f, 0.f, 0.f);
@@ -541,10 +630,10 @@
     }
     return;
   }
-  const int nt = S / 64;
+  const int nt = CQ ? (nq + 63) / 64 : S / 64;
   auto issue = [&](int st) {
     uint8_t* slot = smem + (st % NBUF) * STAGE;
-    dma_tile(Qg, ld, st * 64, slot, w, lane);
+    dma_tile(Qg, ldq, st * 64, slot, w, lane);
     dma_tile(dOg, ldo, st * 64, slot + TILE_BYTES, w, lane);
     dma_f32x64((w < 2 ? lse_g : del_g) + st * 64, slot + 2 * TILE_BYTES + (w < 2 ? 0 : 256), lane);
   };
@@ -585,8 +674,8 @@
   if constexpr (RING) {
     wait_vm_all();
   } else {
-    tile_load(qr, Qg, ld, 0, S);
-    tile_load(dr, dOg, ldo, 0, S);
+    tile_load(qr, Qg, ldq, 0, q_slot<CQ>(cq, S));
+    tile_load(dr, dOg, ldo, 0, q_slot<CQ>(cq, S));
     if (threadIdx.x < 128) rv = threadIdx.x < 64 ? lse_g[threadIdx.x] : del_g[threadIdx.x - 64];
     tile_store(qr, smem);
     tile_store(dr, smem + TILE_BYTES);
@@ -609,14 +698,23 @@
       Qs = smem + (qt & 1) * 2 * TILE_BYTES;
       lse_s = rowv + (qt & 1) * 128;
       if (qt + 1 < nt) {
-        tile_load(qr, Qg, ld, (qt + 1) * 64, S);
-        tile_load(dr, dOg, ldo, (qt + 1) * 64, S);
+        tile_load(qr, Qg, ldq, (qt + 1) * 64, q_slot<CQ>(cq, S));
+        tile_load(dr, dOg, ldo, (qt + 1) * 64, q_slot<CQ>(cq, S));
         if (threadIdx.x < 128)
           rv = threadIdx.x < 64 ? lse_g[(qt + 1) * 64 + threadIdx.x] : del_g[(qt + 1) * 64 + threadIdx.x - 64];
       }
     }
     const uint8_t* Ds = Qs + TILE_BYTES;
     const float* del_s = lse_s + 64;
+    if constexpr (CQ) {
+      if (qt == nt - 1 && (nq & 63) != 0) {
+        if (threadIdx.x < 64 && qt * 64 + (int)threadIdx.x >= nq) {
+          const_cast<float*>(lse_s)[threadIdx.x] = -NEG_BIG;
+          const_cast<float*>(del_s)[threadIdx.x] = 0.f;
+        }
+        __syncthreads();
+      }
+    }
 #pragma unroll
     for (int i2 = 0; i2 < 2; ++i2) {
       floatx16 sc[KS], dp[KS];
@@ -690,14 +788,16 @@
 #pragma unroll
   for (int u = 0; u < KS; ++u) {
     const bool live = k[u] < S;
-    store_row64(dqkv + (rb + k[u]) * ld + (long)H * HD + h * HD, dk[u], scale, hh, live);
-    store_row64(dqkv + (rb + k[u]) * ld + 2L * H * HD + h * HD, dv[u], 1.f, hh, live);
+    store_row64(dkv_g + (rb + k[u]) * ldd + (long)H * HD + h * HD, dk[u], scale, hh, live);
+    store_row64(dkv_g + (rb + k[u]) * ldd + 2L * H * HD + h * HD, dv[u], 1.f, hh, live);
   }
 }
 
 constexpr int kAttnXcd = 1;
 
 }
+
+#ifndef DL_ATTN_COMPACT_Q_UNIT
 
 int dl_attn_fwd(const bf16_t* qkv, long ld, const float* mbias, const int* kvinfo, bf16_t* out, long ldo, float* lse,
                 int B, int H, int S, int D, float scale, hipStream_t st) {
@@ -754,3 +854,39 @@
                                                                B, H, T, sl2, scale, kAttnXcd);
   return 0;
 }
+
+#else
+
+static bool compact_q_ok(const void* q, const void* kv, const int* qcnt, int B, int H, int S, int Sq, int D, long ld,
+                         long ldo) {
+  return q && kv && qcnt && B >= 1 && H >= 1 && D == HD && S % 64 == 0 && Sq % 64 == 0 && Sq >= 64 && Sq <= S &&
+         ld % 8 == 0 && ld >= 2L * H * HD && ldo % 8 == 0 && ldo >= (long)H * HD;
+}
+
+int dl_attn_fwd_q(const bf16_t* q, const bf16_t* kv, long ld, const float* mbias, const int* kvinfo, const int* qcnt,
+                  bf16_t* out, long ldo, float* lse, int B, int H, int S, int Sq, int D, float scale, hipStream_t st) {
+  if (!compact_q_ok(q, kv, qcnt, B, H, S, Sq, D, ld, ldo)) return -1;
+  const float sl2 = scale * 1.4426950408889634f;
+  const CompactQ cq{q, nullptr, nullptr, 0, qcnt, Sq};
+  dim3 grid((Sq + 255) / 256, H, B);
+  attn_fwd_kernel<true, 2, 4, false, CompactQ><<<grid, 256, 0, st>>>(kv, ld, mbias, kvinfo, out, ldo, lse, B, H, S, sl2,
+                                                                 kAttnXcd, cq);
+  return 0;
+}
+
+int dl_attn_bwd_q(const bf16_t* q, const bf16_t* kv, long ld, const float* mbias, const int* kvinfo, const int* qcnt,
+                  const bf16_t* out, const bf16_t* dout, long ldo, const float* lse, float* delta, bf16_t* dq,
+                  bf16_t* dkv, float* dbias, int B, int H, int S, int Sq, int D, float scale, hipStream_t st) {
+  if (!compact_q_ok(q, kv, qcnt, B, H, S, Sq, D, ld, ldo) || !dq || !dkv) return -1;
+  const float sl2 = scale * 1.4426950408889634f;
+  const CompactQ cq{q, dq, dkv, 2L * H * HD, qcnt, Sq};
+  dim3 grid_dq((Sq + 255) / 256, H, B);
+  attn_bwd_dq_kernel<true, 2, false, CompactQ><<<grid_dq, 256, 0, st>>>(kv, ld, mbias, kvinfo, out, dout, ldo, lse, delta,
+                                                                    nullptr, dbias, B, H, S, sl2, scale, kAttnXcd, cq);
+  dim3 grid_kv((S + 127) / 128, H, B);
+  attn_bwd_dkdv_kernel<true, 1, false, CompactQ><<<grid_kv, 256, 0, st>>>(kv, ld, mbias, kvinfo, dout, ldo, lse, delta,
+                                                                      nullptr, B, H, S, sl2, scale, kAttnXcd, cq);
+  return 0;
+}
+
+#endif
diff --git a/dedloc_amd/csrc/kernels/attention_compact_q.hip b/dedloc_amd/csrc/kernels/attention_compact_q.hip
--- /dev/null
+++ b/dedloc_amd/csrc/kernels/attention_compact_q.hip
@@ -0,0 +1,2 @@
+#define DL_ATTN_COMPACT_Q_UNIT
+#include "attention.hip"
diff --git a/dedloc_amd/models/albert.py b/dedloc_amd/models/albert.py
--- a/dedloc_amd/models/albert.py
+++ b/dedloc_amd/models/albert.py
@@ -116,6 +116,7 @@
 _DGRAD_WT = True
 _SHARED_WGRAD = True
 _GELU_GRAD_IN_FWD = True
+_LAST_LAYER_ROWS = True
 
 
 class _AlbertLayerFn(torch.autograd.Function):
@@ -173,6 +174,115 @@
         _wgrad(O, dqkv, h, lv, "gwqkv")
         dh = _dgrad(O, dqkv, lv, "wqkv", ds1)
         return dh, None, None, None, None, None
+
+
+class LastLayerRows:
+
+    def __init__(self, rows, qcnt, Sq, head_rows, targets, owner):
+        self.rows, self.qcnt, self.Sq, self.head_rows, self.targets = rows, qcnt, Sq, head_rows, targets
+        self.owner = owner
+
+    @staticmethod
+    def _build(b_idx, s_pos, targets, B, Sp, Sq):
+        dev = b_idx.device
+        cls = s_pos == 0
+        odd = (s_pos // 32) % 2
+        even = (1 - odd) * (~cls).to(odd.dtype)
+        zeros = torch.zeros(B, dtype=torch.long, device=dev)
+        n_odd, n_even = zeros.scatter_add(0, b_idx, odd), zeros.scatter_add(0, b_idx, even)
+        r_odd = torch.cumsum(odd, 0) - 1 - (torch.cumsum(n_odd, 0) - n_odd)[b_idx]
+        r_even = torch.cumsum(even, 0) - (torch.cumsum(n_even, 0) - n_even)[b_idx]
+        rank = torch.where(odd == 1, r_odd, r_even)
+        cap = Sq // 2
+        fits = rank < cap
+        others = torch.where(odd == 1, (n_even + 1)[b_idx], n_odd[b_idx])
+        half = torch.where(fits, odd, even)
+        rank = torch.where(fits, rank, others + rank - cap)
+        place = torch.where(cls, torch.zeros_like(rank), 64 * (rank // 32) + 32 * half + rank % 32)
+        head_rows = b_idx * Sq + place
+        rows = (torch.arange(B, device=dev)[:, None] * Sp).expand(B, Sq).reshape(-1).clone()
+        rows[head_rows] = b_idx * Sp + s_pos
+        qcnt = torch.ones(B, dtype=torch.long, device=dev).scatter_reduce(0, b_idx, place + 1, "amax")
+        places = torch.arange(B * Sq, device=dev)
+        first = torch.full((B * Sp,), B * Sq, dtype=torch.long, device=dev).scatter_reduce(0, rows, places, "amin")
+        return LastLayerRows(rows, qcnt.to(torch.int32), Sq, head_rows, targets, first[rows])
+
+    @staticmethod
+    def from_positions(mlm_positions, mlm_labels, Sp):
+        B, P = mlm_positions.shape
+        Sq = (1 + P + 63) // 64 * 64
+        if P == 0 or Sq >= Sp:
+            return None
+        b_idx = torch.arange(B, device=mlm_positions.device).repeat_interleave(P)
+        return LastLayerRows._build(b_idx, mlm_positions.reshape(-1), mlm_labels.reshape(-1), B, Sp, Sq)
+
+    @staticmethod
+    def from_labels(labels, Sp):
+        B, S = labels.shape
+        sel = labels != -100
+        host = sel.sum(1).tolist()
+        M, Sq = sum(host), (1 + max(host) + 63) // 64 * 64
+        if M == 0 or Sq >= Sp:
+            return None
+        pos = torch.nonzero_static(sel.reshape(-1), size=M).squeeze(1)
+        return LastLayerRows._build(pos // S, pos % S, labels.reshape(-1)[pos], B, Sp, Sq)
+
+
+class _AlbertLastLayerFn(torch.autograd.Function):
+
+    @staticmethod
+    def forward(ctx, h, mask, lv, H, S, eps, sel):
+        O = ops.OPS
+        Hd = h.shape[1]
+        mbias, kvinfo = mask
+        scale = 1.0 / math.sqrt(Hd // H)
+        kv = O.gemm(h, lv["wqkv"][Hd:], lv["bqkv32"][Hd:], None, False, True, 0)
+        hq = h.index_select(0, sel.rows)
+        q = O.gemm(hq, lv["wqkv"][:Hd], lv["bqkv32"][:Hd], None, False, True, 0)
+        att, lse = ops.attn_fwd_q(q, kv, sel.qcnt, mbias, H, S, scale, kvinfo)
+        s1 = O.gemm(att, lv["wo"], lv["bo32"], hq, False, True, 0)
+        h1, _, m1, r1 = O.layernorm_fwd(s1, None, lv["ln1g"], lv["ln1b"], eps)
+        f, g = (O.gemm_gelu_d if _GELU_GRAD_IN_FWD else O.gemm_gelu)(h1, lv["w1"], lv["b132"])
+        s2 = O.gemm(g, lv["w2"], lv["b232"], h1, False, True, 0)
+        out, _, m2, r2 = O.layernorm_fwd(s2, None, lv["ln2g"], lv["ln2b"], eps)
+        ctx.save_for_backward(h, hq, q, kv, att, lse, s1, m1, r1, h1, f, g, s2, m2, r2)
+        ctx.lv, ctx.mask, ctx.H, ctx.S, ctx.sel, ctx.scale = lv, mask, H, S, sel, scale
+        ctx.gelu_d = _GELU_GRAD_IN_FWD
+        return out
+
+    @staticmethod
+    def backward(ctx, dy):
+        O = ops.OPS
+        h, hq, q, kv, att, lse, s1, m1, r1, h1, f, g, s2, m2, r2 = ctx.saved_tensors
+        lv, sel = ctx.lv, ctx.sel
+        Hd = h.shape[1]
+        dy = dy.contiguous()
+        ds2 = O.layernorm_bwd(dy, s2, lv["ln2g"], m2, r2, lv["gln2g"], lv["gln2b"], True, lv["gb2"])
+        O.gemm_acc_f32(ds2, g, lv["gw2"], True, False)
+        wt = "w2t" in lv
+        dfn = O.gemm_dmul if ctx.gelu_d else O.gemm_dgelu
+        df = dfn(ds2, lv["w2t"], f, lv["gb1"], True) if wt else dfn(ds2, lv["w2"], f, lv["gb1"])
+        O.gemm_acc_f32(df, h1, lv["gw1"], True, False)
+        dh1 = _dgrad(O, df, lv, "w1", ds2)
+        del df
+        ds1 = O.layernorm_bwd(dh1, s1, lv["ln1g"], m1, r1, lv["gln1g"], lv["gln1b"], True, lv["gbo"])
+        O.gemm_acc_f32(ds1, att, lv["gwo"], True, False)
+        datt = _dgrad(O, ds1, lv, "wo", None)
+        dq, dkv, _ = ops.attn_bwd_q(q, kv, sel.qcnt, ctx.mask[0], att, datt, lse, ctx.H, ctx.S, ctx.scale, ctx.mask[1],
+                                    lv["gbqkv"])
+        O.gemm_acc_f32(dq, hq, lv["gwqkv"][:Hd], True, False)
+        O.gemm_acc_f32(dkv, h, lv["gwqkv"][Hd:], True, False)
+        dqo = torch.zeros_like(dq).index_add_(0, sel.owner, dq)
+        ds1o = torch.zeros_like(ds1).index_add_(0, sel.owner, ds1)
+        dcat = torch.cat([dqo, dkv.index_select(0, sel.rows)], 1)
+        if "wqkvt" in lv:
+            dhq = O.gemm(dcat, lv["wqkvt"], None, ds1o, False, True, 0)
+            dh = O.gemm(dkv, lv["wqkvt"][:, Hd:], None, None, False, True, 0)
+        else:
+            dhq = O.gemm(dcat, lv["wqkv"], None, ds1o, False, False, 0)
+            dh = O.gemm(dkv, lv["wqkv"][Hd:], None, None, False, False, 0)
+        dh.index_copy_(0, sel.rows, dhq.index_select(0, sel.owner))
+        return dh, None, None, None, None, None, None
 
 
 def _wgrad(O, dy, x, lv, name):
@@ -346,9 +456,16 @@
             gln2g=f.g(pre + "full_layer_layer_norm.weight"), gln2b=f.g(pre + "full_layer_layer_norm.bias"),
         )
 
-    def _albert_layer(self, h, lv, mask, S):
+    def _albert_layer(self, h, lv, mask, S, last_rows=None):
         c = self.config
+        if last_rows is not None:
+            return _AlbertLastLayerFn.apply(h, mask, lv, c.num_attention_heads, S, c.layer_norm_eps, last_rows)
         return _AlbertLayerFn.apply(h, mask, lv, c.num_attention_heads, S, c.layer_norm_eps)
+
+    def last_layer_rows_supported(self) -> bool:
+        c = self.config
+        return (_LAST_LAYER_ROWS and _RESIDUAL_IN_GEMM and c.inner_group_num == 1
+                and c.hidden_size == 64 * c.num_attention_heads)
 
     def _packed(self, pack_sequences, input_ids, attention_mask, token_type_ids, lengths, labels=None):
         if not (self.pack_sequences if pack_sequences is None else pack_sequences):
@@ -358,7 +475,8 @@
             batch["labels"] = labels
         return pack_batch(batch, lengths, self.config.pad_token_id)
 
-    def encode(self, input_ids=None, attention_mask=None, token_type_ids=None, packed: Optional[PackedBatch] = None):
+    def encode(self, input_ids=None, attention_mask=None, token_type_ids=None, packed: Optional[PackedBatch] = None,
+               last_rows=None):
         assert self.flat is not None, "call model.materialize(device) first"
         c, f = self.config, self.flat
         if packed is not None:
@@ -388,7 +506,7 @@
                    f.g(emb + "token_type_embeddings.weight"), f.g(emb + "LayerNorm.weight"),
                    f.g(emb + "LayerNorm.bias")),
             eps=c.layer_norm_eps)
-        return self._layers(x, mask, Sp), Sp
+        return self._layers(x, mask, Sp, last_rows), Sp
 
     def _encode_packed(self, packed: PackedBatch):
         c, f = self.config, self.flat
@@ -408,7 +526,7 @@
             eps=c.layer_norm_eps)
         return self._layers(x, packed, 0)
 
-    def _layers(self, x, mask, Sp):
+    def _layers(self, x, mask, Sp, last_rows=None):
         c, f = self.config, self.flat
         m = "albert.encoder.embedding_hidden_mapping_in."
         h = ops.linear(x, f.w(m + "weight"), f.w(m + "bias"), f.g(m + "weight"), f.g(m + "bias"))
@@ -422,9 +540,12 @@
             uses = [x for x in range(c.num_hidden_layers) if group_of[x] == g]
             for i in range(c.inner_group_num):
                 lv = views[g][i]
-                if _SHARED_WGRAD and torch.is_grad_enabled():
+                pruned = last_rows is not None and layer == c.num_hidden_layers - 1
+                if last_rows is not None and uses[-1] == c.num_hidden_layers - 1:
+                    uses = uses[:-1]
+                if not pruned and _SHARED_WGRAD and torch.is_grad_enabled():
                     lv = dict(lv, wg_first=layer == uses[-1], wg_last=layer == uses[0])
-                h = self._albert_layer(h, lv, mask, Sp)
+                h = self._albert_layer(h, lv, mask, Sp, last_rows if pruned else None)
         return h
 
     def num_parameters(self) -> int:
@@ -451,17 +572,34 @@
         sd["predictions.decoder.bias"] = sd["predictions.bias"]
         return sd
 
-    def _trunk(self, input_ids, attention_mask, token_type_ids, labels, mlm_positions, pack_sequences, lengths):
+    def _trunk(self, input_ids, attention_mask, token_type_ids, labels, mlm_positions, mlm_labels, pack_sequences,
+               lengths):
         pk = self._packed(pack_sequences, input_ids, attention_mask, token_type_ids, lengths,
                           labels if mlm_positions is None else None)
         if pk is not None:
             h, _ = self.encode(packed=pk)
-            return h, None, pk, pk.row_start
+            return h, None, pk, pk.row_start, None
+        sel = self._last_rows(input_ids, labels, mlm_positions, mlm_labels)
+        if sel is not None:
+            h, _ = self.encode(input_ids, attention_mask, token_type_ids, last_rows=sel)
+            return h, sel.Sq, None, torch.arange(input_ids.shape[0], device=h.device) * sel.Sq, sel
         h, Sp = self.encode(input_ids, attention_mask, token_type_ids)
-        return h, Sp, None, torch.arange(input_ids.shape[0], device=h.device) * Sp
+        return h, Sp, None, torch.arange(input_ids.shape[0], device=h.device) * Sp, None
+
+    def _last_rows(self, input_ids, labels, mlm_positions, mlm_labels):
+        if not self.last_layer_rows_supported():
+            return None
+        Sp = (input_ids.shape[1] + 63) // 64 * 64
+        if mlm_positions is not None:
+            return LastLayerRows.from_positions(mlm_positions, mlm_labels, Sp)
+        if labels is not None:
+            return LastLayerRows.from_labels(labels, Sp)
+        return None
 
     @staticmethod
-    def _mlm_targets(pk, row0, S, Sp, labels, mlm_positions, mlm_labels):
+    def _mlm_targets(pk, row0, S, Sp, labels, mlm_positions, mlm_labels, sel=None):
+        if sel is not None:
+            return sel.head_rows, sel.targets
         if mlm_positions is None and labels is not None:
             if pk is not None:
                 flat_lab = pk.extras["labels"]
@@ -505,9 +643,9 @@
                 ids = batch["input_ids"]
                 B, S = ids.shape
                 labels, pos = batch.get("labels"), batch.get("mlm_positions")
-                h, Sp, pk, row0 = self._trunk(ids, batch.get("attention_mask"), batch.get("token_type_ids"), labels,
-                                              pos, None, lengths)
-                rows, tgt = self._mlm_targets(pk, row0, S, Sp, labels, pos, batch.get("mlm_labels"))
+                h, Sp, pk, row0, sel = self._trunk(ids, batch.get("attention_mask"), batch.get("token_type_ids"),
+                                                   labels, pos, batch.get("mlm_labels"), None, lengths)
+                rows, tgt = self._mlm_targets(pk, row0, S, Sp, labels, pos, batch.get("mlm_labels"), sel)
                 if rows is None:
                     raise ValueError("evaluate_batch needs MLM targets: labels or mlm_positions/mlm_labels")
                 mlm = ops.eval_cross_entropy(self._mlm_logits(h, rows), tgt, topk=(1, 5))
@@ -522,10 +660,10 @@
     def forward(self, input_ids, attention_mask=None, token_type_ids=None, labels=None, sentence_order_label=None,
                 mlm_positions=None, mlm_labels=None, return_logits=False, pack_sequences=None, lengths=None):
         B, S = input_ids.shape
-        h, Sp, pk, row0 = self._trunk(input_ids, attention_mask, token_type_ids, labels, mlm_positions,
-                                      pack_sequences, lengths)
+        h, Sp, pk, row0, sel = self._trunk(input_ids, attention_mask, token_type_ids, labels, mlm_positions, mlm_labels,
+                                           pack_sequences, lengths)
         out = {}
-        rows, tgt = self._mlm_targets(pk, row0, S, Sp, labels, mlm_positions, mlm_labels)
+        rows, tgt = self._mlm_targets(pk, row0, S, Sp, labels, mlm_positions, mlm_labels, sel)
         loss = None
         if rows is not None:
             logits = self._mlm_logits(h, rows)
diff --git a/dedloc_amd/ops/__init__.py b/dedloc_amd/ops/__init__.py
--- a/dedloc_amd/ops/__init__.py
+++ b/dedloc_amd/ops/__init__.py
@@ -161,6 +161,14 @@
     return attn_composed_bwd(qkv, mbias, out, dout, lse, H, S, scale, dbias)
 
 
+def attn_fwd_q(q, kv, qcnt, mbias, H, S, scale, kvinfo=None):
+    return OPS.attn_fwd_q(q, kv, qcnt, mbias, H, S, scale, kvinfo)
+
+
+def attn_bwd_q(q, kv, qcnt, mbias, out, dout, lse, H, S, scale, kvinfo=None, dbias=None):
+    return OPS.attn_bwd_q(q, kv, qcnt, mbias, out, dout, lse, H, S, scale, kvinfo, dbias)
+
+
 def attn_varlen_fwd(qkv, packed, H, scale):
     D = qkv.shape[-1] // (3 * H)
     if D not in FUSED_HEAD_DIMS:
diff --git a/dedloc_amd/ops/_lib.py b/dedloc_amd/ops/_lib.py
--- a/dedloc_amd/ops/_lib.py
+++ b/dedloc_amd/ops/_lib.py
@@ -40,6 +40,10 @@
     "attn_fwd(Tensor qkv, Tensor? mbias, int H, int S, float scale, Tensor? kvinfo=None) -> (Tensor, Tensor)",
     "attn_bwd(Tensor qkv, Tensor? mbias, Tensor out, Tensor dout, Tensor lse, int H, int S, float scale, "
     "Tensor? kvinfo=None, Tensor(a!)? dbias=None) -> Tensor",
+    "attn_fwd_q(Tensor q, Tensor kv, Tensor qcnt, Tensor? mbias, int H, int S, float scale, Tensor? kvinfo=None) "
+    "-> (Tensor, Tensor)",
+    "attn_bwd_q(Tensor q, Tensor kv, Tensor qcnt, Tensor? mbias, Tensor out, Tensor dout, Tensor lse, int H, int S, "
+    "float scale, Tensor? kvinfo=None, Tensor(a!)? dbias=None) -> (Tensor, Tensor, Tensor)",
     "attn_varlen_fwd(Tensor qkv, Tensor seqinfo, Tensor seqinfo_host, int H, float scale) -> (Tensor, Tensor)",
     "attn_varlen_bwd(Tensor qkv, Tensor seqinfo, Tensor seqinfo_host, Tensor out, Tensor dout, Tensor lse, int H, "
     "float scale, Tensor(a!)? dbias=None) -> Tensor",
@@ -605,6 +609,55 @@
     return g
 
 
+def _compact_q_probs(q, kv, qcnt, mbias, H, S, scale):
+    T, D = kv.shape[0], kv.shape[1] // (2 * H)
+    B = T // S
+    Sq = q.shape[0] // B
+    if D != 64 or kv.shape[1] != 2 * H * D or q.shape[1] != H * D or Sq % 64 or not 64 <= Sq <= S:
+        raise RuntimeError("dedloc_amd: compact queries need head_dim 64, kv [B*S, 2*H*64] and q [B*Sq, H*64] "
+                           "with Sq a multiple of 64 in 64 .. S")
+    x = kv.float().reshape(B, S, 2, H, D)
+    k, v = x[:, :, 0].transpose(1, 2), x[:, :, 1].transpose(1, 2)
+    qq = q.float().reshape(B, Sq, H, D).transpose(1, 2)
+    s = torch.matmul(qq, k.transpose(-1, -2)) * scale
+    if mbias is not None:
+        s = s + mbias.reshape(B, 1, 1, S) / math.log2(math.e)
+    live = torch.arange(Sq)[None, :] < qcnt.clamp(1, Sq)[:, None].to(torch.long)
+    return qq, k, v, s, live
+
+
+@_impl("attn_fwd_q")
+def _attn_fwd_q_cpu(q, kv, qcnt, mbias, H, S, scale, kvinfo=None):
+    qq, k, v, s, live = _compact_q_probs(q, kv, qcnt, mbias, H, S, scale)
+    B, _, Sq, D = qq.shape
+    lse = torch.logsumexp(s, -1) * math.log2(math.e)
+    o = torch.matmul(torch.softmax(s, -1), v).transpose(1, 2).reshape(B * Sq, H * D)
+    o = torch.where(live.reshape(-1, 1), o, torch.zeros_like(o))
+    return _bf(o), torch.where(live[:, None, :], lse, torch.zeros_like(lse)).contiguous()
+
+
+@_impl("attn_bwd_q")
+def _attn_bwd_q_cpu(q, kv, qcnt, mbias, out, dout, lse, H, S, scale, kvinfo=None, dbias=None):
+    qq, k, v, s, live = _compact_q_probs(q, kv, qcnt, mbias, H, S, scale)
+    B, _, Sq, D = qq.shape
+    lv = live[:, None, :, None].float()
+    p = torch.softmax(s, -1) * lv
+    do = dout.float().reshape(B, Sq, H, D).transpose(1, 2) * lv
+    o = out.float().reshape(B, Sq, H, D).transpose(1, 2) * lv
+    dv = torch.matmul(p.transpose(-1, -2), do)
+    dp = torch.matmul(do, v.transpose(-1, -2))
+    delta = (do * o).sum(-1, keepdim=True)
+    ds = p * (dp - delta)
+    dq = _bf((torch.matmul(ds, k) * scale).transpose(1, 2).reshape(B * Sq, H * D))
+    dk = torch.matmul(ds.transpose(-1, -2), qq) * scale
+    dkv = _bf(torch.stack([dk, dv], dim=2).permute(0, 3, 2, 1, 4).reshape(B * S, 2 * H * D))
+    if dbias is not None:
+        HD = H * D
+        dbias[:HD] += dq.float().sum(0)
+        dbias[2 * HD:] += do.transpose(1, 2).reshape(-1, HD).sum(0)
+    return dq, dkv, delta.squeeze(-1).contiguous()
+
+
 def packed_layout(seqinfo_host, T):
     v = [int(x) for x in seqinfo_host.reshape(-1).tolist()]
     if len(v) < 3 or len(v) % 2 == 0:
```

Measured after the change: 1083 samples/s (median of 6 runs). +2.0%, better.
